# OpenDriveLab/ST-P3

Hardware: AMD Instinct MI355X
Metric: BEV samples/sec (6-cam x 3-frame fwd+bwd) (higher is better)
Workload: dtype bf16 convs / f32 voxel pool; 1 GPU; BASELINE configs[2]: batch=4/GPU, 6-cam 224x480, T=3, full STP3 fwd+bwd with segmentation + pedestrian + hdmap + depth CE + instance centerness/offset + flow losses, grad-clip 5, Adam; EfficientNet-B4, D=48, C=64, BEV 200x200; global_batch=4, parallelism=dp1, launch=hipgraph

## Files before the change

### include/stp3_hip.h

```cpp
#ifndef STP3_HIP_H
#define STP3_HIP_H

#include <stddef.h>
#include <stdint.h>

#ifdef __cplusplus
extern "C" {
#endif

#define STP3_OK          0
#define STP3_EINVAL   (-10001)
#define STP3_EUNSUP   (-10002)
#define STP3_ENOSPACE (-10003)

#define STP3_DTYPE_F32  0
#define STP3_DTYPE_BF16 1

typedef struct stp3_lift_dims {
    int32_t B, T, N;
    int32_t D, fH, fW;
    int32_t C;
    int32_t X, Y, Z;
} stp3_lift_dims;

// ... 135 lines not shown
                    void* stream);
int stp3_linear_bwd(int32_t M, int32_t K, int32_t N, const float* dy, const float* x, const float* w, int32_t ldw, float* dx,
                    float* dw, int32_t lddw, float* db, void* stream);

typedef struct stp3_conv_dims {
    int32_t N, H, W, Cin;
    int32_t Ho, Wo, Cout;
    int32_t KH, KW, stride;
    int32_t pad_h, pad_w, dil_h, dil_w;
    int32_t ldx, ldy;
    int32_t out_dtype, has_bias;
} stp3_conv_dims;

int stp3_conv2d_fwd_workspace(const stp3_conv_dims* dims, size_t* bytes);
int stp3_conv2d_fwd(const stp3_conv_dims* dims, const void* x, const void* w, const float* bias, void* y,
                    float* sums, void* workspace, size_t workspace_bytes, void* stream);

int stp3_conv2d_fwd_stats(const stp3_conv_dims* dims, const void* x, const void* w, float* sums, void* workspace,
                          size_t workspace_bytes, void* stream);
int stp3_conv2d_fwd_bnact(const stp3_conv_dims* dims, const void* x, const void* w, const float* coef, int32_t act, void* y,
                          void* stream);
int stp3_conv2d_bn_bwd_reduce(const stp3_conv_dims* dims, const void* x, const void* w, const void* dz, int32_t ldz,
                              const float* coef, int32_t act, float* sums, void* workspace, size_t workspace_bytes,
                              void* stream);
int stp3_conv2d_bn_bwd_apply(const stp3_conv_dims* dims, const void* x, const void* w, const void* dz, int32_t ldz,
                             const float* coef, int32_t act, const float* gsums, double count, void* dy, void* stream);
int stp3_conv2d_bn_bwd_apply_dx(const stp3_conv_dims* dims, const void* x, const void* w, const void* dz, int32_t ldz,
                                const float* coef, int32_t act, const float* gsums, double count, void* dy, void* dx,
                                int32_t lddx, const void* add, int32_t ldadd, void* stream);

int stp3_conv2d_fwd_add(const stp3_conv_dims* dims, const void* x, const void* w, const float* bias, const void* add,
                        int32_t ldadd, void* y, void* stream);

int stp3_conv2d_wgrad_workspace(const stp3_conv_dims* dims, size_t* bytes);
int stp3_conv2d_wgrad(const stp3_conv_dims* dims, const void* dy, const void* x, float* dw, void* workspace,
                      size_t workspace_bytes, void* stream);

#define STP3_WGRAD_BATCH_MAX 96
typedef struct stp3_wgrad_job {
    const void* partials;
    float* dw;
    int64_t numel;
    int32_t splits;
    int32_t reserved;
} stp3_wgrad_job;
int stp3_conv2d_wgrad_partials(const stp3_conv_dims* dims, const void* dy, const void* x, const float* pre_coef,
                               int32_t pre_act, void* partials, size_t partials_bytes, int32_t* splits, void* stream);
int stp3_conv2d_wgrad_reduce_batch(int32_t n, const stp3_wgrad_job* jobs, void* stream);

int stp3_conv2d_fwd_pre(const stp3_conv_dims* dims, const void* x, const void* w, const float* bias, const float* pre_coef,
                        int32_t pre_act, void* y, void* stream);
int stp3_conv2d_wgrad_pre(const stp3_conv_dims* dims, const void* dy, const void* x, const float* pre_coef, int32_t pre_act,
                          float* dw, void* workspace, size_t workspace_bytes, void* stream);

typedef struct stp3_se_dims {
    int32_t N, rows, C, ld;
    int32_t dtype;
} stp3_se_dims;

int stp3_se_workspace_bytes(const stp3_se_dims* dims, size_t* bytes);
int stp3_se_pool(const stp3_se_dims* dims, const void* x, const void* dy, void* workspace, size_t workspace_bytes,
                 float* out, void* stream);
int stp3_se_scale(const stp3_se_dims* dims, const void* x, const float* gate, const float* add, void* y, void* stream);

typedef struct stp3_se_mlp_dims {
    int32_t N, C, S;
    float inv_rows;
} stp3_se_mlp_dims;

int stp3_se_mlp_fwd(const stp3_se_mlp_dims* dims, const float* pooled_sum, const float* w1, const float* b1,
                    const float* w2, const float* b2, float* z1, float* gate, void* stream);
int stp3_se_mlp_bwd(const stp3_se_mlp_dims* dims, const float* dgate, const float* gate, const float* pooled_sum,
                    const float* z1, const float* w1, const float* w2, float* dz2, float* dz1, float* dpooled,
                    float* dw1, float* db1, float* dw2, float* db2, void* stream);

int stp3_dwconv2d_fwd_stats_workspace(const stp3_dwconv_dims* dims, size_t* bytes);
int stp3_dwconv2d_fwd_stats(const stp3_dwconv_dims* dims, const void* x, const float* w, void* y, float* sums,
                            void* workspace, size_t workspace_bytes, void* stream);
int stp3_bn_finalize(const float* sums, int32_t C, double count, const float* gamma, const float* beta, float eps,
                     float momentum, float* running_mean, float* running_var, float* coef, void* stream);
int stp3_mbconv_workspace_bytes(const stp3_se_dims* dims, size_t* bytes);
int stp3_se_pool_act(const stp3_se_dims* dims, const void* x, const float* scale, const float* shift, int32_t act,
                     void* workspace, size_t workspace_bytes, float* out, void* stream);
int stp3_mbconv_scale_act(const stp3_se_dims* dims, int32_t ldy, const void* x, const float* scale, const float* shift,
                          int32_t act, const float* gate, void* y, void* stream);
int stp3_mbconv_bwd_reduce(const stp3_se_dims* dims, int32_t ldg, const void* da, const void* x, const float* coef,
                           int32_t act, void* workspace, size_t workspace_bytes, float* sums5, void* stream);
int stp3_mbconv_bwd_coef(int32_t N, int32_t C, const float* sums5, const float* gate, const float* dpooled,
                         float* gsums, void* stream);
int stp3_mbconv_bwd_apply(const stp3_se_dims* dims, int32_t ldg, const void* da, const void* x, const float* coef,
                          int32_t act, const float* gate, const float* dpooled, const float* gsums, double count,
                          void* dx, void* stream);

int stp3_dwconv2d_fwd_stats_bn(const stp3_dwconv_dims* dims, const void* x, const float* w, void* y, float* sums, double count,
                               const float* gamma, const float* beta, float eps, float momentum, float* running_mean,
                               float* running_var, float* coef, void* workspace, size_t workspace_bytes, void* stream);

typedef struct stp3_ce_dims {
    int32_t rows, P, C, k;
    int32_t ignore_index, dtype;
    int64_t stride_row, stride_c, stride_p;
} stp3_ce_dims;

int stp3_ce_topk_workspace_bytes(const stp3_ce_dims* dims, size_t* bytes);
int stp3_ce_topk_fwd(const stp3_ce_dims* dims, const void* logits, const int64_t* labels, const float* class_weights,
                     const float* row_scale, float* loss_px, float* sel, double out_scale, int32_t accumulate, float* out,
// ... 332 lines not shown
```

### st-p3_amd/csrc/stp3_bnact.hip

```cpp
#include <hip/hip_runtime.h>
#include <stdint.h>
#include <stdlib.h>

#include <initializer_list>

#include "stp3_cdna.h"
#include "stp3_hip.h"

namespace {

struct BnDims {
    int N, rows, C, ldx, ldy, ldr;
    int act, res_mode, has_sbias, has_oscale;
    int CL;
};

constexpr int kThreads = 256;
constexpr int kUnroll = 4;

__device__ __forceinline__ float bf2f(uint16_t b) { return __uint_as_float((uint32_t)b << 16); }

template <typename T, int VEC> struct Io;
template <> struct Io<float, 4> {
    typedef float4 Raw;
    static __device__ Raw load_raw(const float* p) { return *reinterpret_cast<const float4*>(p); }
    static __device__ void unpack(const Raw& v, float* f) { f[0] = v.x; f[1] = v.y; f[2] = v.z; f[3] = v.w; }
    static __device__ void load(const float* p, float* f) {
        const float4 v = *reinterpret_cast<const float4*>(p);
        f[0] = v.x; f[1] = v.y; f[2] = v.z; f[3] = v.w;
    }
    static __device__ void store(float* p, const float* f) {
        *reinterpret_cast<float4*>(p) = make_float4(f[0], f[1], f[2], f[3]);
    }
};
template <> struct Io<float, 1> {
    typedef float Raw;
    static __device__ Raw load_raw(const float* p) { return p[0]; }
    static __device__ void unpack(const Raw& v, float* f) { f[0] = v; }
    static __device__ void load(const float* p, float* f) { f[0] = p[0]; }
    static __device__ void store(float* p, const float* f) { p[0] = f[0]; }
};
template <> struct Io<uint16_t, 8> {
    typedef uint4 Raw;
    static __device__ Raw load_raw(const uint16_t* p) { return *reinterpret_cast<const uint4*>(p); }
    static __device__ void unpack(const Raw& v, float* f) {
        const uint32_t w[4] = {v.x, v.y, v.z, v.w};
#pragma unroll
        for (int i = 0; i < 4; ++i) {
            f[2 * i] = __uint_as_float(w[i] << 16);
            f[2 * i + 1] = __uint_as_float(w[i] & 0xffff0000u);
        }
    }
    static __device__ void load(const uint16_t* p, float* f) {
        const uint4 v = *reinterpret_cast<const uint4*>(p);
        const uint32_t w[4] = {v.x, v.y, v.z, v.w};
#pragma unroll
        for (int i = 0; i < 4; ++i) {
            f[2 * i] = __uint_as_float(w[i] << 16);
            f[2 * i + 1] = __uint_as_float(w[i] & 0xffff0000u);
        }
// ... 345 lines not shown
#pragma unroll
                for (int u = 0; u < U; ++u) {
                    if (r + u * step < d.rows) {
                        float v[VEC], g[VEC], rv[VEC];
                        Io<T, VEC>::unpack(xr[u], v);
                        Io<T, VEC>::unpack(gr[u], g);
                        mask_tail<VEC, TAIL>(m, v);
                        mask_tail<VEC, TAIL>(m, g);
                        if (PRE_RES) {
                            Io<T, VEC>::unpack(rr[u], rv);
                            mask_tail<VEC, TAIL>(m, rv);
                        }
#pragma unroll
                        for (int j = 0; j < VEC; ++j) {
                            const float xh = (v[j] - mu[j]) * is[j];
                            float gg = g[j] * os;
                            if (ACT != STP3_ACT_NONE) {
                                float pre = fmaf(v[j], cs[j], ct[j]);
                                if (PRE_RES) pre += rv[j];
                                gg *= act_grad_c<ACT>(pre);
                            }
                            acc[0][j] += gg;
                            acc[1][j] = fmaf(gg, xh, acc[1][j]);
                            acc[2][j] += xh;
                        }
                    }
                }
            }
        });
    }
    block_reduce_store<VEC, 3, FULL>(d, m, acc, red, partial);
}

template <typename T, int VEC, bool TRAIN, bool FULL, bool TAIL>
__global__ __launch_bounds__(kThreads) void bn_apply_bwd_kernel(
    BnDims d, const T* __restrict__ dy, const T* __restrict__ x, const float* __restrict__ sbias,
    const T* __restrict__ res, const float* __restrict__ oscale, const float* __restrict__ mean_,
    const float* __restrict__ invstd_, const float* __restrict__ gamma, const float* __restrict__ beta,
    const float* __restrict__ gsums, float inv_count, T* __restrict__ dx, T* __restrict__ dres) {
    const Map m = make_map<VEC, FULL>(d);
    if (!m.live) return;
    const int n = blockIdx.y;
    const int c0 = m.cv * VEC;
    float cs[VEC], ct[VEC], a2[VEC], a3[VEC];
#pragma unroll
    for (int j = 0; j < VEC; ++j) {
        const int c = c0 + j;
        const bool ok = c < d.C;
        const float sb = (ok && d.has_sbias) ? sbias[(size_t)n * d.C + c] : 0.f;
        const float mu = ok ? mean_[c] - sb : 0.f;
        const float is = ok ? invstd_[c] : 0.f;
        const float ga = ok ? (gamma ? gamma[c] : 1.f) : 0.f;
        const float be = ok ? (beta ? beta[c] : 0.f) : 0.f;
        const float k0 = (TRAIN && ok) ? gsums[c] * inv_count : 0.f;
        const float k1 = (TRAIN && ok) ? gsums[d.C + c] * inv_count : 0.f;
        cs[j] = ga * is;
        ct[j] = be - mu * cs[j];
        a2[j] = -(cs[j] * is) * k1;
        a3[j] = -cs[j] * k0 - a2[j] * mu;
    }
    const float os = d.has_oscale ? oscale[n] : 1.f;
    const T* xs = x + (size_t)n * d.rows * d.ldx + c0;
    const T* gs = dy + (size_t)n * d.rows * d.ldy + c0;
    const bool pre_res = d.res_mode == STP3_RES_BEFORE_ACT;
    const T* rs = pre_res ? res + (size_t)n * d.rows * d.ldr + c0 : nullptr;
    T* dxs = dx + (size_t)n * d.rows * d.ldx + c0;
    T* drs = (pre_res && dres) ? dres + (size_t)n * d.rows * d.ldr + c0 : nullptr;
    const int step = gridDim.x * m.RL;
    constexpr int U = 4;
    typedef typename Io<T, VEC>::Raw Raw;
    dispatch_act_res(d.act, rs ? STP3_RES_BEFORE_ACT : STP3_RES_NONE, [&](auto act_c, auto res_c) {
        constexpr int ACT = decltype(act_c)::value;
        constexpr bool PRE_RES = decltype(res_c)::value == STP3_RES_BEFORE_ACT;
        for (int r = blockIdx.x * m.RL + m.rl; r < d.rows; r += U * step) {
            Raw xr[U], gr[U], rr[U];
#pragma unroll
            for (int u = 0; u < U; ++u) {
                if (r + u * step < d.rows) {
                    xr[u] = Io<T, VEC>::load_raw(xs + (size_t)(r + u * step) * d.ldx);
                    gr[u] = Io<T, VEC>::load_raw(gs + (size_t)(r + u * step) * d.ldy);
                    if (PRE_RES) rr[u] = Io<T, VEC>::load_raw(rs + (size_t)(r + u * step) * d.ldr);
                }
            }
#pragma unroll
            for (int u = 0; u < U; ++u) {
                if (r + u * step < d.rows) {
                    float v[VEC], g[VEC], rv[VEC];
                    Io<T, VEC>::unpack(xr[u], v);
                    Io<T, VEC>::unpack(gr[u], g);
                    mask_tail<VEC, TAIL>(m, v);
                    mask_tail<VEC, TAIL>(m, g);
                    if (PRE_RES) {
                        Io<T, VEC>::unpack(rr[u], rv);
                        mask_tail<VEC, TAIL>(m, rv);
                    }
#pragma unroll
                    for (int j = 0; j < VEC; ++j) {
                        float gg = g[j] * os;
                        if (ACT != STP3_ACT_NONE) {
                            float pre = fmaf(v[j], cs[j], ct[j]);
                            if (PRE_RES) pre += rv[j];
                            gg *= act_grad_c<ACT>(pre);
                        }
                        g[j] = gg;
                        v[j] = fmaf(cs[j], gg, fmaf(a2[j], v[j], a3[j]));
                    }
                    Io<T, VEC>::store(dxs + (size_t)(r + u * step) * d.ldx, v);
                    if (drs) Io<T, VEC>::store(drs + (size_t)(r + u * step) * d.ldr, g);
                }
            }
        }
    });
}

__global__ __launch_bounds__(kThreads) void bn_dsbias_kernel(int N, int C, float rows, const float* __restrict__ sample_sums,
                                                             const float* __restrict__ gsums, float inv_count,
                                                             const float* __restrict__ gamma,
                                                             const float* __restrict__ invstd, float* __restrict__ out) {
    const int i = blockIdx.x * kThreads + threadIdx.x;
    if (i >= N * C) return;
    const int n = i / C, c = i - n * C;
    const float* s = sample_sums + (size_t)n * 3 * C;
    const float gi = (gamma ? gamma[c] : 1.f) * invstd[c];
    float v = s[c];
    if (gsums) {
        const float k0 = gsums[c] * inv_count, k1 = gsums[C + c] * inv_count;
        v = (v - rows * k0) - s[2 * C + c] * k1;
    }
    out[i] = gi * v;
}

struct SumPtrs {
    const void* p[8];
};
template <typename T, int VEC>
__global__ __launch_bounds__(kThreads) void sum_n_kernel(int n, size_t nvec, SumPtrs src, T* __restrict__ y,
                                                         const T* __restrict__ plane, unsigned vps, unsigned cvs) {
    typedef typename Io<T, VEC>::Raw Raw;
    const size_t stride = (size_t)gridDim.x * kThreads;
    for (size_t i = (size_t)blockIdx.x * kThreads + threadIdx.x; i < nvec; i += 2 * stride) {
        const bool two = i + stride < nvec;
        Raw a[8], b[8];
#pragma unroll
        for (int k = 0; k < 8; ++k) {
            if (k < n) {
                a[k] = Io<T, VEC>::load_raw((const T*)src.p[k] + i * VEC);
                if (two) b[k] = Io<T, VEC>::load_raw((const T*)src.p[k] + (i + stride) * VEC);
            }
        }
        float acc[VEC], acc2[VEC], v[VEC];
#pragma unroll
        for (int j = 0; j < VEC; ++j) acc[j] = acc2[j] = 0.f;
#pragma unroll
        for (int k = 0; k < 8; ++k) {
            if (k < n) {
                Io<T, VEC>::unpack(a[k], v);
#pragma unroll
                for (int j = 0; j < VEC; ++j) acc[j] += v[j];
// ... 322 lines not shown
```

### st-p3_amd/csrc/stp3_conv.hip

```cpp
#include <hip/hip_runtime.h>
#include <stdint.h>
#include <stdlib.h>
#include <string.h>

#include "stp3_cdna.h"
#include "stp3_hip.h"

namespace {

typedef __attribute__((ext_vector_type(8))) __bf16 bf16x8;
typedef __attribute__((ext_vector_type(4))) float f32x4;
typedef __attribute__((ext_vector_type(16))) float f32x16;

struct ConvDims {
    int N, H, W, Cin, Ho, Wo, Cout;
    int KH, KW, stride, pad_h, pad_w, dil_h, dil_w;
    int ldx, ldy;
    int out_f32, has_bias;
    int M;
    int kchunks;
    int Ktot;
};

union Frag {
    uint4 u;
    bf16x8 v;
};

__device__ __forceinline__ float bf2f(uint32_t b) { return __uint_as_float(b << 16); }

constexpr int kBM = 128;
constexpr int kBK = 64;

__device__ __attribute__((aligned(16))) uint4 g_zero16 = {0u, 0u, 0u, 0u};
typedef stp3_u32x4 u32x4;

__device__ __forceinline__ uint4 keep(uint4 v, bool ok) {
    return make_uint4(ok ? v.x : 0u, ok ? v.y : 0u, ok ? v.z : 0u, ok ? v.w : 0u);
}

__device__ __forceinline__ int xcd_order(int bid, int nwg) {
    const int q = nwg >> 3, r = nwg & 7, xcd = bid & 7;
    return (xcd < r ? xcd * (q + 1) : r * (q + 1) + (xcd - r) * q) + (bid >> 3);
}

__device__ __forceinline__ int lds_piece(int r, int j) { return (r * 8 + (j ^ ((r >> 1) & 7))) * 16; }

enum { kModePlain = 0, kModeStats = 1, kModeBnAct = 2, kModeBwdReduce = 3, kModeBwdApply = 4, kModeAffine = 5 };
constexpr bool mode_bwd(int m) { return m == kModeBwdReduce || m == kModeBwdApply; }

struct EpiArgs {
    const uint16_t* add;
    int ldadd;
    uint16_t* dx;
    int lddx;
    const float* coef;
    const uint16_t* dz;
    const float* gsums;
    float inv_count;
    int ldz, act;
    const uint16_t* res;
    int ldres, res_mode;
    int cvalid;
    const float* sbias;
    int hw;
    const float* pre;
    int pre_off;
};

enum { kPreNone = 0, kPreAffine = 1, kPreRelu = 2 };
template <int PRE>
__device__ __forceinline__ uint32_t pre_pair(uint32_t wd, stp3_f32x2 cs, stp3_f32x2 ct) {
    const stp3_f32x2 e0 = {__uint_as_float(wd << 16), __uint_as_float(wd & 0xffff0000u)};
    stp3_f32x2 out = pk_fma(e0, cs, ct);
    if (PRE == kPreRelu) out = stp3_f32x2{fmaxf(out.x, 0.f), fmaxf(out.y, 0.f)};
    return pack_bf16(out.x, out.y);
}
template <int PRE>
__device__ __forceinline__ u32x4 pre_piece(u32x4 v, const stp3_f32x2 (&cs)[4], const stp3_f32x2 (&ct)[4], uint32_t mask) {
    u32x4 o;
#pragma unroll
    for (int r = 0; r < 4; ++r) o[r] = pre_pair<PRE>(v[r], cs[r], ct[r]) & mask;
    return o;
}

template <int ACT>
__device__ __forceinline__ float epi_act(float v) {
    if (ACT == STP3_ACT_RELU) return fmaxf(v, 0.f);
    if (ACT == STP3_ACT_SWISH) return v * fast_sigmoid(v);
    return v;
}
template <int ACT>
__device__ __forceinline__ float epi_act_grad(float pre) {
    if (ACT == STP3_ACT_RELU) return pre > 0.f ? 1.f : 0.f;
    if (ACT == STP3_ACT_SWISH) {
        const float sg = fast_sigmoid(pre);
        return sg * (1.f + pre * (1.f - sg));
    }
    return 1.f;
}

template <int BN, int MODE = kModePlain, int ACT = STP3_ACT_NONE, bool BUF = false, int PRE = kPreNone>
__global__ __launch_bounds__(256) void conv2d_igemm_kernel(ConvDims d, int tiles_co, const uint16_t* __restrict__ x,
                                                           const uint16_t* __restrict__ w,
                                                           const float* __restrict__ bias, void* __restrict__ y,
                                                           float* __restrict__ stat_partial, EpiArgs ep = EpiArgs()) {
    constexpr int TP = BN == 128 ? 2 : 1;
    constexpr int TC = 2;
    constexpr int kStage = (kBM + BN) * kBK * 2;
    extern __shared__ __attribute__((aligned(16))) uint8_t smem[];
    const int tid = threadIdx.x;
    const int lane = tid & 63;
    const int wave = __builtin_amdgcn_readfirstlane(tid >> 6);
    const int wm = BN == 128 ? (wave >> 1) : wave;
    const int wn = BN == 128 ? (wave & 1) : 0;
    const int v = xcd_order(blockIdx.x, gridDim.x);
    const int tile_m = v / tiles_co, tile_co = v - tile_m * tiles_co;
    const int m0 = tile_m * kBM;
    const int co0 = tile_co * BN;

    const int j = tid & 7, rr = tid >> 3;
    const uint16_t* const zero = reinterpret_cast<const uint16_t*>(&g_zero16);
    const uint16_t* prow[4];
    uint32_t poff[4];
    int phi[4], pwi[4];
    uint32_t rmask[4];
#pragma unroll
    for (int i = 0; i < 4; ++i) {
        const int m = m0 + rr + 32 * i;
        if (PRE) rmask[i] = m < d.M ? 0xffffffffu : 0u;
        if (m < d.M) {
            const int wo = m % d.Wo;
            const int t = m / d.Wo;
            const int ho = t % d.Ho;
            const int n = t / d.Ho;
            phi[i] = ho * d.stride - d.pad_h;
            pwi[i] = wo * d.stride - d.pad_w;
            if (BUF) poff[i] = (uint32_t)(((n * d.H + phi[i]) * d.W + pwi[i]) * d.ldx) * 2u;
            else prow[i] = x + (ptrdiff_t)((n * d.H + phi[i]) * d.W + pwi[i]) * d.ldx;
        } else {
            phi[i] = -(1 << 28);
            pwi[i] = 0;
            if (BUF) poff[i] = kBufOob; else prow[i] = zero;
        }
    }
    const uint16_t* wrow[BN / 32];
    uint32_t woff[BN / 32];
#pragma unroll
    for (int i = 0; i < BN / 32; ++i) {
        const int co = co0 + rr + 32 * i;
        if (BUF) woff[i] = co < d.Cout ? (uint32_t)(co * d.Ktot) * 2u : kBufOob;
        else wrow[i] = co < d.Cout ? w + (size_t)co * d.Ktot : zero;
    }
    const stp3_buffer xbuf = make_buffer(x, BUF ? (uint32_t)((size_t)d.N * d.H * d.W * d.ldx * 2) : 0u);
    const stp3_buffer wbuf = make_buffer(w, BUF ? (uint32_t)((size_t)d.Cout * d.Ktot * 2) : 0u);
    int tap = 0, ci = j * 8;
    while (ci >= d.Cin) { ci -= d.Cin; ++tap; }
    int kh = tap / d.KW, kw = tap - kh * d.KW;
    const int taps = d.KH * d.KW;
    const bool pointwise = taps == 1 && d.pad_h == 0 && d.pad_w == 0 && (d.Ho - 1) * d.stride < d.H &&
                           (d.Wo - 1) * d.stride < d.W;

    const int steps = (d.Ktot + kBK - 1) / kBK;
    float* const ptab = reinterpret_cast<float*>(smem + ep.pre_off);
    const int kpad = steps * kBK;
    int prek = 0;
    if (PRE) {
        for (int e = tid; e < 2 * kpad; e += 256) {
            const int h = e >= kpad, c = e - h * kpad;
            ptab[e] = c < d.Cin ? ep.pre[h * d.Cin + c] : 0.f;
        }
        __syncthreads();
    }

    u32x4 ra[4], rb[BN / 32];
    auto load_step = [&]() {
        const bool kvalid = tap < taps;
        const int dh = kh * d.dil_h, dw = kw * d.dil_w;
        const int toff = (dh * d.W + dw) * d.ldx + ci;
#pragma unroll
        for (int i = 0; i < 4; ++i) {
            if (BUF) {
                bool ok = kvalid & (poff[i] != kBufOob);
                if (!pointwise) {
                    const int hi = phi[i] + dh, wi = pwi[i] + dw;
                    ok = ok & ((unsigned)hi < (unsigned)d.H) & ((unsigned)wi < (unsigned)d.W);
                }
                ra[i] = buffer_load16(xbuf, ok ? poff[i] + (uint32_t)toff * 2u : kBufOob);
            } else {
                bool ok = kvalid && prow[i] != zero;
                if (!pointwise) {
                    const int hi = phi[i] + dh, wi = pwi[i] + dw;
                    ok = ok && (unsigned)hi < (unsigned)d.H && (unsigned)wi < (unsigned)d.W;
                }
                ra[i] = *reinterpret_cast<const u32x4*>(ok ? prow[i] + toff : zero);
            }
        }
        const int kk = tap * d.Cin + ci;
        if (PRE) prek = kk;
#pragma unroll
        for (int i = 0; i < BN / 32; ++i) {
            if (BUF) rb[i] = buffer_load16(wbuf, (kvalid & (woff[i] != kBufOob)) ? woff[i] + (uint32_t)kk * 2u : kBufOob);
            else rb[i] = *reinterpret_cast<const u32x4*>((kvalid && wrow[i] != zero) ? wrow[i] + kk : zero);
        }
        ci += kBK;
        while (ci >= d.Cin && tap < taps) {
            ci -= d.Cin;
            ++tap;
            if (++kw == d.KW) { kw = 0; ++kh; }
        }
    };
    auto store_step = [&](uint8_t* buf) {
        if (PRE) {
            const f32x4 s0 = *reinterpret_cast<const f32x4*>(ptab + prek), s1 = *reinterpret_cast<const f32x4*>(ptab + prek + 4);
            const f32x4 t0 = *reinterpret_cast<const f32x4*>(ptab + kpad + prek);
            const f32x4 t1 = *reinterpret_cast<const f32x4*>(ptab + kpad + prek + 4);
            const stp3_f32x2 cs[4] = {{s0[0], s0[1]}, {s0[2], s0[3]}, {s1[0], s1[1]}, {s1[2], s1[3]}};
            const stp3_f32x2 ct[4] = {{t0[0], t0[1]}, {t0[2], t0[3]}, {t1[0], t1[1]}, {t1[2], t1[3]}};
#pragma unroll
            for (int i = 0; i < 4; ++i) ra[i] = pre_piece<PRE>(ra[i], cs, ct, rmask[i]);
        }
#pragma unroll
        for (int i = 0; i < 4; ++i) *reinterpret_cast<u32x4*>(buf + lds_piece(rr + 32 * i, j)) = ra[i];
#pragma unroll
        for (int i = 0; i < BN / 32; ++i) *reinterpret_cast<u32x4*>(buf + kBM * kBK * 2 + lds_piece(rr + 32 * i, j)) = rb[i];
    };

    f32x16 acc[TC][TP];
#pragma unroll
    for (int a = 0; a < TC; ++a)
#pragma unroll
        for (int b = 0; b < TP; ++b)
#pragma unroll
            for (int r = 0; r < 16; ++r) acc[a][b][r] = 0.f;

    load_step();
    store_step(smem);
    __syncthreads();
    const int frow = lane & 31, fk = lane >> 5;
    for (int s = 0; s < steps; ++s) {
        uint8_t* cur = smem + (s & 1) * kStage;
        if (s + 1 < steps) load_step();
#pragma unroll
        for (int ks = 0; ks < kBK / 16; ++ks) {
            Frag fa[TC], fb[TP];
#pragma unroll
            for (int a = 0; a < TC; ++a)
                fa[a].u = *reinterpret_cast<const uint4*>(cur + kBM * kBK * 2 + lds_piece(wn * 64 + a * 32 + frow, ks * 2 + fk));
#pragma unroll
            for (int b = 0; b < TP; ++b)
                fb[b].u = *reinterpret_cast<const uint4*>(cur + lds_piece(wm * (32 * TP) + b * 32 + frow, ks * 2 + fk));
#pragma unroll
            for (int a = 0; a < TC; ++a)
#pragma unroll
                for (int b = 0; b < TP; ++b)
                    acc[a][b] = __builtin_amdgcn_mfma_f32_32x32x16_bf16(fa[a].v, fb[b].v, acc[a][b], 0, 0, 0);
        }
        if (s + 1 < steps) store_step(smem + ((s + 1) & 1) * kStage);
        __syncthreads();
    }

    const int ldt = BN + 8;
    if (d.out_f32) {
        float* tile = reinterpret_cast<float*>(smem);
#pragma unroll
        for (int a = 0; a < TC; ++a)
// ... 240 lines not shown
                }
            }
        }
}

template <int MODE>
__device__ __forceinline__ void epi8(const uint32_t (&wds)[4], const uint32_t (&gds)[4], const Chan8& k, int act,
                                     stp3_f32x2 (&s1)[4], stp3_f32x2 (&s2)[4], uint32_t (&ow)[4], int res_mode = STP3_RES_NONE) {
#pragma unroll
    for (int r = 0; r < 4; ++r) {
        const uint32_t wd = MODE == kModeAffine ? wds[r] & k.keep[r] : wds[r];
        const stp3_f32x2 e0 = {__uint_as_float(wd << 16), __uint_as_float(wd & 0xffff0000u)};
        if (MODE == kModePlain || MODE == kModeStats) {
            s1[r] = s1[r] + e0;
            s2[r] = pk_fma(e0, e0, s2[r]);
        } else {
            const stp3_f32x2 pre = pk_fma(e0, k.cs[r], k.ct[r]);
            if (MODE == kModeBnAct) {
                stp3_f32x2 out = pre;
                if (act == STP3_ACT_SWISH) out = pre * pk_sigmoid(pre);
                else if (act == STP3_ACT_RELU) out = stp3_f32x2{fmaxf(pre.x, 0.f), fmaxf(pre.y, 0.f)};
                ow[r] = pack_bf16(out.x, out.y);
            } else if (MODE == kModeAffine) {
                const uint32_t gd = gds[r] & k.keep[r];
                const stp3_f32x2 rv = {__uint_as_float(gd << 16), __uint_as_float(gd & 0xffff0000u)};
                stp3_f32x2 out = pre;
                if (res_mode == STP3_RES_BEFORE_ACT) out = out + rv;
                if (act == STP3_ACT_SWISH) out = out * pk_sigmoid(out);
                else if (act == STP3_ACT_RELU) out = stp3_f32x2{fmaxf(out.x, 0.f), fmaxf(out.y, 0.f)};
                if (res_mode == STP3_RES_AFTER_ACT) out = out + rv;
                ow[r] = pack_bf16(out.x, out.y);
            } else {
                const stp3_f32x2 dz = {__uint_as_float(gds[r] << 16), __uint_as_float(gds[r] & 0xffff0000u)};
                stp3_f32x2 der = {1.f, 1.f};
                if (act == STP3_ACT_SWISH) {
                    const stp3_f32x2 sg = pk_sigmoid(pre);
                    der = sg * (1.f + pre * (1.f - sg));
                } else if (act == STP3_ACT_RELU) {
                    der = stp3_f32x2{pre.x > 0.f ? 1.f : 0.f, pre.y > 0.f ? 1.f : 0.f};
                }
                const stp3_f32x2 gg = dz * der;
                if (MODE == kModeBwdReduce) {
                    s1[r] = s1[r] + gg;
                    s2[r] = pk_fma(gg, (e0 - k.mu[r]) * k.is[r], s2[r]);
                } else {
                    const stp3_f32x2 out = pk_fma(k.cs[r], gg, pk_fma(k.a2[r], e0, k.a3[r]));
                    ow[r] = pack_bf16(out.x, out.y);
                }
            }
        }
    }
}

template <int PP, int KMAX, int MODE>
__global__ __launch_bounds__(256, 2) void pointwise_rows_kernel(ConvDims d, int ksteps, int tiles_co, const uint16_t* __restrict__ x,
                                                             const uint16_t* __restrict__ w, uint16_t* __restrict__ y,
                                                             float* __restrict__ stat_partial, EpiArgs ep) {
    constexpr int NT = (PP + 3) / 4;
    constexpr int RPI = 64 / PP;
    constexpr int NIT = (32 + RPI - 1) / RPI;
    constexpr int LDT = NT * 32 + 8;
    extern __shared__ __attribute__((aligned(16))) uint8_t smem[];
    const int tid = threadIdx.x, lane = tid & 63;
    const int wave = __builtin_amdgcn_readfirstlane(tid >> 6);
    const int v_order = xcd_order(blockIdx.x, gridDim.x);
    const int group = v_order / tiles_co, ngroups = gridDim.x / tiles_co;
    const int co0 = (v_order - group * tiles_co) * (PP * 8);
    const int LDW = ksteps * 16 + 8;
    uint16_t* wimg = reinterpret_cast<uint16_t*>(smem);
    uint16_t* tile = wimg + NT * 32 * LDW + wave * (32 * LDT);
    float* red = reinterpret_cast<float*>(wimg + NT * 32 * LDW);
    uint16_t* wtimg = wimg + NT * 32 * LDW + 4 * (32 * LDT);
    const bool with_dx = MODE == kModeBwdApply && ep.dx != nullptr;
    if (with_dx) {
        for (int e = tid; e < 32 * NT * 32; e += 256) {
            const int k = e / (NT * 32), c = e - k * (NT * 32);
            wtimg[k * LDT + c] = (c < PP * 8 && k < d.Cin) ? w[(size_t)(co0 + c) * d.Cin + k] : (uint16_t)0;
        }
    }
    for (int e = tid; e < NT * 32 * ksteps * 2; e += 256) {
        const int r = e / (ksteps * 2), k0 = (e - r * (ksteps * 2)) * 8;
        u32x4 v = {0u, 0u, 0u, 0u};
        if (r < PP * 8 && k0 < d.Cin) v = *reinterpret_cast<const u32x4*>(w + (size_t)(co0 + r) * d.Cin + k0);
        *reinterpret_cast<u32x4*>(wimg + r * LDW + k0) = v;
    }
    __syncthreads();
    const int px = lane & 31, half = lane >> 5;
    const int cp = lane % PP, prow = lane / PP;
    const bool lane_ok = prow < RPI;
    const int cl = cp * 8, cch = co0 + cl;
    Chan8 kc;
    load_chan8<MODE>(kc, ep, d.Cout, cch, true);
    stp3_f32x2 s1[4], s2[4];
#pragma unroll
    for (int r = 0; r < 4; ++r) s1[r] = s2[r] = stp3_f32x2{0.f, 0.f};
    const uint16_t* const zero = reinterpret_cast<const uint16_t*>(&g_zero16);
    u32x4 cur[KMAX], nxt[KMAX];
    const int ntiles = (d.M + 31) / 32;
    const int stride_t = ngroups * 4;
    auto load_tile = [&](int t, u32x4 (&f)[KMAX]) {
        const int m = t * 32 + px;
        const uint16_t* row = (t < ntiles && m < d.M) ? x + (size_t)m * d.ldx : nullptr;
#pragma unroll
        for (int ks = 0; ks < KMAX; ++ks) {
            const int k0 = ks * 16 + half * 8;
            if (ks < ksteps) f[ks] = *reinterpret_cast<const u32x4*>((row && k0 < d.Cin) ? row + k0 : zero);
        }
    };
    int t = group * 4 + wave;
    load_tile(t, cur);
    for (; t < ntiles; t += stride_t) {
        load_tile(t + stride_t, nxt);
        const int mbase = t * 32;
        f32x16 acc[NT];
#pragma unroll
        for (int a = 0; a < NT; ++a)
#pragma unroll
            for (int r = 0; r < 16; ++r) acc[a][r] = 0.f;
#pragma unroll
        for (int ks = 0; ks < KMAX; ++ks) {
            if (ks < ksteps) {
                Frag fb;
                fb.u = make_uint4(cur[ks][0], cur[ks][1], cur[ks][2], cur[ks][3]);
#pragma unroll
                for (int a = 0; a < NT; ++a) {
                    Frag fa;
                    fa.u = *reinterpret_cast<const uint4*>(wimg + (a * 32 + px) * LDW + ks * 16 + half * 8);
                    acc[a] = __builtin_amdgcn_mfma_f32_32x32x16_bf16(fa.v, fb.v, acc[a], 0, 0, 0);
                }
            }
        }
#pragma unroll
        for (int a = 0; a < NT; ++a)
#pragma unroll
            for (int q = 0; q < 4; ++q)
                *reinterpret_cast<uint2*>(tile + px * LDT + a * 32 + 8 * q + 4 * half) =
                    make_uint2(pack_bf16(acc[a][4 * q], acc[a][4 * q + 1]), pack_bf16(acc[a][4 * q + 2], acc[a][4 * q + 3]));
        __builtin_amdgcn_fence(__ATOMIC_RELEASE, "wavefront");
        __builtin_amdgcn_wave_barrier();
#pragma unroll
        for (int i = 0; i < NIT; ++i) {
            const int p = prow + i * RPI;
            const int m = mbase + p;
            if (lane_ok && p < 32 && m < d.M) {
                const uint4 v = *reinterpret_cast<const uint4*>(tile + p * LDT + cl);
                if (MODE == kModePlain) *reinterpret_cast<uint4*>(y + (size_t)m * d.ldy + cch) = v;
                if (MODE != kModePlain || stat_partial) {
                    const uint32_t wds[4] = {v.x, v.y, v.z, v.w};
                    uint32_t gds[4] = {0u, 0u, 0u, 0u}, ow[4];
                    if (mode_bwd(MODE)) {
                        const uint4 g = *reinterpret_cast<const uint4*>(ep.dz + (size_t)m * ep.ldz + cch);
                        gds[0] = g.x; gds[1] = g.y; gds[2] = g.z; gds[3] = g.w;
                    }
                    if (MODE == kModeAffine && ep.res) {
                        const uint4 g = *reinterpret_cast<const uint4*>(ep.res + (size_t)m * ep.ldres + cch);
                        gds[0] = g.x; gds[1] = g.y; gds[2] = g.z; gds[3] = g.w;
                    }
                    if (MODE == kModeAffine) epi8<MODE>(wds, gds, kc, ep.act, s1, s2, ow, ep.res ? ep.res_mode : STP3_RES_NONE);
                    else epi8<MODE>(wds, gds, kc, ep.act, s1, s2, ow);
                    if (MODE == kModeBnAct || MODE == kModeBwdApply || MODE == kModeAffine)
                        *reinterpret_cast<uint4*>(y + (size_t)m * d.ldy + cch) = make_uint4(ow[0], ow[1], ow[2], ow[3]);
                    if (with_dx)
                        *reinterpret_cast<uint4*>(tile + p * LDT + cl) = make_uint4(ow[0], ow[1], ow[2], ow[3]);
                }
            }
        }
        if (with_dx) {
            __builtin_amdgcn_fence(__ATOMIC_RELEASE, "wavefront");
            __builtin_amdgcn_wave_barrier();
            f32x16 dxa;
#pragma unroll
            for (int r = 0; r < 16; ++r) dxa[r] = 0.f;
#pragma unroll
            for (int ks = 0; ks < NT * 2; ++ks) {
                Frag fa, fb;
                fa.u = *reinterpret_cast<const uint4*>(wtimg + px * LDT + ks * 16 + half * 8);
                fb.u = *reinterpret_cast<const uint4*>(tile + px * LDT + ks * 16 + half * 8);
                dxa = __builtin_amdgcn_mfma_f32_32x32x16_bf16(fa.v, fb.v, dxa, 0, 0, 0);
            }
            const int m = mbase + px;
            if (m < d.M) {
#pragma unroll
                for (int q = 0; q < 4; ++q) {
                    const int ci = 8 * q + 4 * half;
                    if (ci < d.Cin) {
                        uint32_t lo = pack_bf16(dxa[4 * q], dxa[4 * q + 1]), hi = pack_bf16(dxa[4 * q + 2], dxa[4 * q + 3]);
                        if (ep.add) {
                            const uint2 a = *reinterpret_cast<const uint2*>(ep.add + (size_t)m * ep.ldadd + ci);
                            lo = pack_bf16(__uint_as_float(lo << 16) + __uint_as_float(a.x << 16),
                                           __uint_as_float(lo & 0xffff0000u) + __uint_as_float(a.x & 0xffff0000u));
                            hi = pack_bf16(__uint_as_float(hi << 16) + __uint_as_float(a.y << 16),
                                           __uint_as_float(hi & 0xffff0000u) + __uint_as_float(a.y & 0xffff0000u));
                        }
                        *reinterpret_cast<uint2*>(ep.dx + (size_t)m * ep.lddx + ci) = make_uint2(lo, hi);
                    }
                }
            }
        }
        __builtin_amdgcn_wave_barrier();
#pragma unroll
        for (int ks = 0; ks < KMAX; ++ks) cur[ks] = nxt[ks];
    }
    if (stat_partial && (MODE == kModePlain || MODE == kModeStats || MODE == kModeBwdReduce)) {
        __syncthreads();
#pragma unroll
        for (int r = 0; r < 8; ++r) {
            red[(wave * 64 + lane) * 16 + r] = s1[r >> 1][r & 1];
            red[(wave * 64 + lane) * 16 + 8 + r] = s2[r >> 1][r & 1];
        }
        __syncthreads();
        for (int e = tid; e < 2 * PP * 8; e += 256) {
            const int k = e / (PP * 8), c = e - k * (PP * 8);
            const int pc = c >> 3, r = c & 7;
            float tot = 0.f;
            for (int wv = 0; wv < 4; ++wv)
                for (int g = 0; g < RPI; ++g) tot += red[(wv * 64 + g * PP + pc) * 16 + k * 8 + r];
            stat_partial[((size_t)group * 2 + k) * d.Cout + co0 + c] = tot;
        }
    }
}

template <int KMAX, int MODE>
__global__ __launch_bounds__(256) void pointwise_direct_kernel(ConvDims d, int ksteps, int cblocks, int ngroups,
                                                               const uint16_t* __restrict__ x, const uint16_t* __restrict__ w,
                                                               uint16_t* __restrict__ y, float* __restrict__ stat_partial,
                                                               EpiArgs ep) {
    constexpr bool kSums = MODE == kModePlain || MODE == kModeStats || MODE == kModeBwdReduce;
    __shared__ float red[kSums ? 4 * 64 * 33 : 1];
    const int tid = threadIdx.x, lane = tid & 63;
    const int wave = __builtin_amdgcn_readfirstlane(tid >> 6);
    const int slot = xcd_order(blockIdx.x, gridDim.x) * 4 + wave;
    const int group = slot / cblocks, cb = slot - group * cblocks;
    const bool live = group < ngroups;
    const int px = lane & 31, h = lane >> 5;
    const uint16_t* const zero = reinterpret_cast<const uint16_t*>(&g_zero16);
    Frag wf[KMAX];
    {
        const int q = px >> 3, hh = (px >> 2) & 1, j = px & 3;
        const int co = cb * 32 + 16 * (q >> 1) + 8 * hh + 4 * (q & 1) + j;
#pragma unroll
        for (int ks = 0; ks < KMAX; ++ks) {
            const int k0 = ks * 16 + h * 8;
            wf[ks].u = *reinterpret_cast<const uint4*>((live && ks < ksteps && co < d.Cout && k0 < d.Cin) ? w + (size_t)co * d.Cin + k0 : zero);
        }
    }
    int ch[2];
    bool ok[2];
    Chan8 kc[2];
    stp3_f32x2 s1[2][4], s2[2][4];
#pragma unroll
    for (int s = 0; s < 2; ++s) {
        ch[s] = cb * 32 + 16 * s + 8 * h;
        ok[s] = live && ch[s] < d.Cout;
        load_chan8<MODE>(kc[s], ep, d.Cout, ch[s], ok[s]);
#pragma unroll
        for (int r = 0; r < 4; ++r) s1[s][r] = s2[s][r] = stp3_f32x2{0.f, 0.f};
    }
    const int ntiles = (d.M + 31) / 32;
    u32x4 cur[KMAX], nxt[KMAX];
    auto load_tile = [&](int t, u32x4 (&f)[KMAX]) {
        const int m = t * 32 + px;
        const uint16_t* row = (live && t < ntiles && m < d.M) ? x + (size_t)m * d.ldx : nullptr;
#pragma unroll
        for (int ks = 0; ks < KMAX; ++ks) {
            if (ks < ksteps) {
                const int k0 = ks * 16 + h * 8;
                f[ks] = *reinterpret_cast<const u32x4*>((row && k0 < d.Cin) ? row + k0 : zero);
            }
        }
    };
    int t = live ? group : ntiles;
    load_tile(t, cur);
    for (; t < ntiles; t += ngroups) {
        load_tile(t + ngroups, nxt);
        const int m = t * 32 + px;
        const bool row_ok = m < d.M;
        uint4 g[2] = {make_uint4(0u, 0u, 0u, 0u), make_uint4(0u, 0u, 0u, 0u)};
        if (mode_bwd(MODE)) {
#pragma unroll
            for (int s = 0; s < 2; ++s)
                if (row_ok && ok[s]) g[s] = *reinterpret_cast<const uint4*>(ep.dz + (size_t)m * ep.ldz + ch[s]);
        }
        if (MODE == kModeAffine && ep.res) {
#pragma unroll
            for (int s = 0; s < 2; ++s)
                if (row_ok && ok[s]) g[s] = *reinterpret_cast<const uint4*>(ep.res + (size_t)m * ep.ldres + ch[s]);
        }
        f32x16 acc;
#pragma unroll
        for (int r = 0; r < 16; ++r) acc[r] = 0.f;
#pragma unroll
        for (int ks = 0; ks < KMAX; ++ks) {
            if (ks < ksteps) {
                Frag fb;
                fb.u = make_uint4(cur[ks][0], cur[ks][1], cur[ks][2], cur[ks][3]);
                acc = __builtin_amdgcn_mfma_f32_32x32x16_bf16(wf[ks].v, fb.v, acc, 0, 0, 0);
            }
        }
#pragma unroll
        for (int s = 0; s < 2; ++s) {
            const uint32_t wds[4] = {pack_bf16(acc[8 * s], acc[8 * s + 1]), pack_bf16(acc[8 * s + 2], acc[8 * s + 3]),
                                     pack_bf16(acc[8 * s + 4], acc[8 * s + 5]), pack_bf16(acc[8 * s + 6], acc[8 * s + 7])};
            if (!(row_ok && ok[s])) continue;
            if (MODE == kModePlain) {
                *reinterpret_cast<uint4*>(y + (size_t)m * d.ldy + ch[s]) = make_uint4(wds[0], wds[1], wds[2], wds[3]);
                if (!stat_partial) continue;
            }
            const uint32_t gds[4] = {g[s].x, g[s].y, g[s].z, g[s].w};
            uint32_t ow[4];
            if (MODE == kModeAffine) epi8<MODE>(wds, gds, kc[s], ep.act, s1[s], s2[s], ow, ep.res ? ep.res_mode : STP3_RES_NONE);
            else epi8<MODE>(wds, gds, kc[s], ep.act, s1[s], s2[s], ow);
            if (MODE == kModeBnAct || MODE == kModeBwdApply || MODE == kModeAffine)
                *reinterpret_cast<uint4*>(y + (size_t)m * d.ldy + ch[s]) = make_uint4(ow[0], ow[1], ow[2], ow[3]);
        }
#pragma unroll
        for (int ks = 0; ks < KMAX; ++ks) cur[ks] = nxt[ks];
    }
    if (kSums) {
        if (!stat_partial) return;
        float* mine = red + (wave * 64 + lane) * 33;
#pragma unroll
        for (int s = 0; s < 2; ++s)
#pragma unroll
            for (int r = 0; r < 8; ++r) {
                mine[s * 8 + r] = s1[s][r >> 1][r & 1];
                mine[16 + s * 8 + r] = s2[s][r >> 1][r & 1];
            }
        __builtin_amdgcn_fence(__ATOMIC_RELEASE, "wavefront");
        __builtin_amdgcn_wave_barrier();
        const int idx = lane & 31;
        float tot = 0.f;
        for (int p = 0; p < 32; ++p) tot += red[(wave * 64 + h * 32 + p) * 33 + idx];
        const int k = idx >> 4, sp = (idx >> 3) & 1, r = idx & 7;
        const int c = cb * 32 + 16 * sp + 8 * h + r;
        if (live && c < d.Cout) stat_partial[((size_t)group * 2 + k) * d.Cout + c] = tot;
    }
}

__global__ __launch_bounds__(256) void colsum_kernel(int parts, int width, const float* __restrict__ partial,
                                                     float* __restrict__ out) {
    __shared__ double red[256];
    const int cl = threadIdx.x & 63, rl = threadIdx.x >> 6;
    const int col = blockIdx.x * 64 + cl;
    const int r0 = blockIdx.y * 256, r1 = min(r0 + 256, parts);
    double s0 = 0.0, s1 = 0.0, s2 = 0.0, s3 = 0.0;
    if (col < width) {
        int p = r0 + rl;
        for (; p + 12 < r1; p += 16) {
            const float a = partial[(size_t)p * width + col], b = partial[(size_t)(p + 4) * width + col];
            const float c = partial[(size_t)(p + 8) * width + col], e = partial[(size_t)(p + 12) * width + col];
            s0 += (double)a; s1 += (double)b; s2 += (double)c; s3 += (double)e;
        }
        for (; p < r1; p += 4) s0 += (double)partial[(size_t)p * width + col];
    }
    red[threadIdx.x] = (s0 + s1) + (s2 + s3);
    __syncthreads();
    if (rl == 0 && col < width)
        out[(size_t)blockIdx.y * width + col] = (float)(red[cl] + red[64 + cl] + red[128 + cl] + red[192 + cl]);
}

inline void launch_colsum(hipStream_t s, int parts, int width, float* partial, float* sums) {
    const int wx = (width + 63) / 64;
    if (parts <= 256) {
        hipLaunchKernelGGL(colsum_kernel, dim3(wx, 1), dim3(256), 0, s, parts, width, (const float*)partial, sums);
        return;
    }
    const int l1 = (parts + 255) / 256;
    float* mid = partial + (size_t)parts * width;
    hipLaunchKernelGGL(colsum_kernel, dim3(wx, l1), dim3(256), 0, s, parts, width, (const float*)partial, mid);
    hipLaunchKernelGGL(colsum_kernel, dim3(wx, 1), dim3(256), 0, s, l1 > 256 ? 256 : l1, width, (const float*)mid, sums);
}


template <int T>
__device__ __forceinline__ int wg_piece(int m, int p) {
    const int sw = T == 64 ? ((m >> 1) & 1) << 2 : (m & 3) << 2;
    return m * (T * 2) + ((p ^ sw) << 4);
}

union FragTr {
    stp3_s16x4 h[2];
    bf16x8 v;
};

template <int TCO, int TCI, bool BUF = false, int PRE = kPreNone>
__global__ __launch_bounds__(256) void conv2d_wgrad_kernel(ConvDims d, int tiles_ci, int ksteps_per_block, int tap_fold,
                                                           int xcd_chunks, const uint16_t* __restrict__ dy,
                                                           const uint16_t* __restrict__ x,
                                                           float* __restrict__ partial, const float* __restrict__ pre = nullptr) {
    constexpr int TA = TCO / 64, TB = TCI / 64;
    constexpr int kImgA = kBK * TCO * 2;
    constexpr int kStage = kBK * (TCO + TCI) * 2;
    constexpr int PA = TCO / 8, PB = TCI / 8;
    constexpr int NA = TCO / 32, NB = TCI / 32;
    constexpr int RA = 256 / PA, RB = 256 / PB;
    extern __shared__ __attribute__((aligned(16))) uint8_t smem[];
    const int tid = threadIdx.x;
    const int lane = tid & 63;
    const int wave = __builtin_amdgcn_readfirstlane(tid >> 6);
    const int wa = wave >> 1, wb = wave & 1;
    int bx = blockIdx.x, by = blockIdx.y, bz = blockIdx.z;
    if (xcd_chunks) {
        const int lin = xcd_order(bx + (int)gridDim.x * (by + (int)gridDim.y * bz), (int)(gridDim.x * gridDim.y * gridDim.z));
        bx = lin % (int)gridDim.x;
        by = (lin / (int)gridDim.x) % (int)gridDim.y;
        bz = lin / (int)(gridDim.x * gridDim.y);
    }
    const int tco = bx / tiles_ci, tci = bx - tco * tiles_ci;
    const int tap = by;
    const int split = bz;
    const int kh = tap / d.KW, kw = tap - kh * d.KW;
    const int co0 = tco * TCO, ci0 = tci * TCI;
    const int total_steps = (d.M + kBK - 1) / kBK;
    const int step0 = split * ksteps_per_block;
    const int step1 = min(step0 + ksteps_per_block, total_steps);
    const uint16_t* const zero = reinterpret_cast<const uint16_t*>(&g_zero16);

    const int pa = tid % PA, ra0 = tid / PA;
    const int pb = tid % PB, rb0 = tid / PB;
    const bool a_ok = co0 + pa * 8 < d.Cout;
    const uint16_t* const srca = a_ok ? dy + co0 + pa * 8 : zero;
    const unsigned lda = a_ok ? (unsigned)d.ldy : 0u;
    bool b_ok = ci0 + pb * 8 < d.Cin;
    int chb = ci0 + pb * 8, khb = kh, kwb = kw;
    if (tap_fold) {
        const int t = tap * tap_fold + pb;
        khb = t / d.KW;
        kwb = t - khb * d.KW;
        chb = 0;
        b_ok = t < d.KH * d.KW;
    }
    const uint16_t* const srcb = b_ok ? x + chb : zero;
    const unsigned ldb = b_ok ? (unsigned)d.ldx : 0u;
    const stp3_buffer abuf = make_buffer(dy, BUF ? (uint32_t)((size_t)d.M * d.ldy * 2) : 0u);
    const stp3_buffer bbuf = make_buffer(x, BUF ? (uint32_t)((size_t)d.N * d.H * d.W * d.ldx * 2) : 0u);
    const uint32_t cola = (uint32_t)(co0 + pa * 8) * 2u, colb = (uint32_t)chb * 2u;
    const uint32_t pitcha = (uint32_t)d.ldy * 2u, pitchb = (uint32_t)d.ldx * 2u;
    const int fold_dh = khb * d.dil_h, fold_dw = kwb * d.dil_w;
    stp3_f32x2 pcs[4], pct[4];
    uint32_t bmask[NB];
    if (PRE) {
#pragma unroll
        for (int r = 0; r < 4; ++r)
#pragma unroll
            for (int h = 0; h < 2; ++h) {
                pcs[r][h] = b_ok ? pre[chb + 2 * r + h] : 0.f;
                pct[r][h] = b_ok ? pre[d.Cin + chb + 2 * r + h] : 0.f;
            }
    }

    const int hw = d.Ho * d.Wo;
    const int qa = kBK / hw, qr = kBK - qa * hw, qb = qr / d.Wo, qc = qr - qb * d.Wo;
    int p_wo, p_ho, p_n;
    {
        const int m = step0 * kBK + lane;
        p_wo = m % d.Wo;
        const int t = m / d.Wo;
        p_ho = t % d.Ho;
        p_n = t / d.Ho;
    }
    const int tap_h = kh * d.dil_h - d.pad_h, tap_w = kw * d.dil_w - d.pad_w;

    u32x4 rawa[NA], rawb[NB];
    auto load_step = [&](int step) {
        const int mbase = step * kBK;
#pragma unroll
        for (int i = 0; i < NA; ++i) {
            const int m = mbase + ra0 + RA * i;
            if (BUF) rawa[i] = buffer_load16(abuf, (a_ok & (m < d.M)) ? (uint32_t)m * pitcha + cola : kBufOob);
            else rawa[i] = *reinterpret_cast<const u32x4*>(m < d.M ? srca + (size_t)(unsigned)m * lda : zero);
        }
        const bool inside = mbase + lane < d.M;
        if (!tap_fold) {
            const int hi = p_ho * d.stride + tap_h, wi = p_wo * d.stride + tap_w;
            const bool ok = inside && (unsigned)hi < (unsigned)d.H && (unsigned)wi < (unsigned)d.W;
            const int pix = ok ? (p_n * d.H + hi) * d.W + wi : -1;
#pragma unroll
            for (int i = 0; i < NB; ++i) {
                const int pv = __shfl(pix, rb0 + RB * i);
                if (PRE) bmask[i] = pv >= 0 ? 0xffffffffu : 0u;
                if (BUF) rawb[i] = buffer_load16(bbuf, (b_ok & (pv >= 0)) ? (uint32_t)pv * pitchb + colb : kBufOob);
                else rawb[i] = *reinterpret_cast<const u32x4*>(pv >= 0 ? srcb + (size_t)(unsigned)pv * ldb : zero);
            }
        } else {
            const int hs = p_ho * d.stride - d.pad_h, ws = p_wo * d.stride - d.pad_w;
            const int base = (p_n * d.H + hs) * d.W + ws;
            const int pack = inside ? ((hs + 32768) << 16) | (ws + 32768) : 0;
#pragma unroll
            for (int i = 0; i < NB; ++i) {
                const int bs = __shfl(base, rb0 + RB * i), pk = __shfl(pack, rb0 + RB * i);
                const int hi = (int)((unsigned)pk >> 16) - 32768 + fold_dh, wi = (pk & 0xffff) - 32768 + fold_dw;
                const bool ok = (unsigned)hi < (unsigned)d.H && (unsigned)wi < (unsigned)d.W;
                const int pv = bs + fold_dh * d.W + fold_dw;
                if (BUF) rawb[i] = buffer_load16(bbuf, (b_ok & ok) ? (uint32_t)pv * pitchb + colb : kBufOob);
                else rawb[i] = *reinterpret_cast<const u32x4*>(ok ? srcb + (size_t)(unsigned)pv * ldb : zero);
            }
        }
        p_wo += qc; p_ho += qb; p_n += qa;
        if (p_wo >= d.Wo) { p_wo -= d.Wo; ++p_ho; }
        if (p_ho >= d.Ho) { p_ho -= d.Ho; ++p_n; }
    };
    auto store_step = [&](uint8_t* buf) {
        if (PRE) {
#pragma unroll
            for (int i = 0; i < NB; ++i) rawb[i] = pre_piece<PRE>(rawb[i], pcs, pct, bmask[i]);
        }
#pragma unroll
        for (int i = 0; i < NA; ++i) *reinterpret_cast<u32x4*>(buf + wg_piece<TCO>(ra0 + RA * i, pa)) = rawa[i];
#pragma unroll
        for (int i = 0; i < NB; ++i) *reinterpret_cast<u32x4*>(buf + kImgA + wg_piece<TCI>(rb0 + RB * i, pb)) = rawb[i];
    };

    f32x16 acc[TA][TB];
#pragma unroll
    for (int a = 0; a < TA; ++a)
#pragma unroll
        for (int b = 0; b < TB; ++b)
#pragma unroll
            for (int r = 0; r < 16; ++r) acc[a][b][r] = 0.f;

    const int frow = lane & 31, fk = lane >> 5;
    const int fm = 8 * fk + ((lane & 15) >> 2), fc = 16 * ((lane >> 4) & 1) + 4 * (lane & 3);
    int offa[TA], offb[TB];
#pragma unroll
    for (int a = 0; a < TA; ++a) {
        const int c = wa * (32 * TA) + a * 32 + fc;
        offa[a] = wg_piece<TCO>(fm, c >> 3) + (c & 7) * 2;
    }
#pragma unroll
    for (int b = 0; b < TB; ++b) {
        const int c = wb * (32 * TB) + b * 32 + fc;
        offb[b] = kImgA + wg_piece<TCI>(fm, c >> 3) + (c & 7) * 2;
    }

    if (step0 < step1) {
        load_step(step0);
        store_step(smem);
    }
    __syncthreads();
    for (int s = step0; s < step1; ++s) {
        const uint8_t* cur = smem + ((s - step0) & 1) * kStage;
        if (s + 1 < step1) load_step(s + 1);
#pragma unroll
        for (int ks = 0; ks < kBK / 16; ++ks) {
            FragTr fa[TA], fb[TB];
#pragma unroll
            for (int a = 0; a < TA; ++a) {
                fa[a].h[0] = lds_read_tr16(cur + offa[a] + (ks * 16) * (TCO * 2));
                fa[a].h[1] = lds_read_tr16(cur + offa[a] + (ks * 16 + 4) * (TCO * 2));
            }
#pragma unroll
            for (int b = 0; b < TB; ++b) {
                fb[b].h[0] = lds_read_tr16(cur + offb[b] + (ks * 16) * (TCI * 2));
                fb[b].h[1] = lds_read_tr16(cur + offb[b] + (ks * 16 + 4) * (TCI * 2));
            }
#pragma unroll
            for (int a = 0; a < TA; ++a)
#pragma unroll
// ... 79 lines not shown
        for (; k < splits; k += 4) add(s0, *reinterpret_cast<const float4*>(partial + (size_t)k * n + i));
    } else if (i < n) {
        float* s0e = &s0.x; float* s1e = &s1.x; float* s2e = &s2.x; float* s3e = &s3.x;
        for (int e = 0; e < 4 && i + e < n; ++e) {
            int k = kl;
            for (; k + 12 < splits; k += 16) {
                s0e[e] += partial[(size_t)k * n + i + e];       s1e[e] += partial[(size_t)(k + 4) * n + i + e];
                s2e[e] += partial[(size_t)(k + 8) * n + i + e]; s3e[e] += partial[(size_t)(k + 12) * n + i + e];
            }
            for (; k < splits; k += 4) s0e[e] += partial[(size_t)k * n + i + e];
        }
    }
    float4 t;
    t.x = (s0.x + s1.x) + (s2.x + s3.x); t.y = (s0.y + s1.y) + (s2.y + s3.y);
    t.z = (s0.z + s1.z) + (s2.z + s3.z); t.w = (s0.w + s1.w) + (s2.w + s3.w);
    red[threadIdx.x] = t;
    __syncthreads();
    if (kl == 0 && i < n) {
        const float4 a = red[cg], bb = red[64 + cg], c = red[128 + cg], d = red[192 + cg];
        float4 o;
        o.x = (a.x + bb.x) + (c.x + d.x); o.y = (a.y + bb.y) + (c.y + d.y);
        o.z = (a.z + bb.z) + (c.z + d.z); o.w = (a.w + bb.w) + (c.w + d.w);
        if (i + 3 < n && ((uintptr_t)(dw + i) & 15) == 0) {
            *reinterpret_cast<float4*>(dw + i) = o;
        } else {
            const float* oe = &o.x;
            for (int e = 0; e < 4 && i + e < n; ++e) dw[i + e] = oe[e];
        }
    }
}

inline int status() {
    hipError_t e = hipGetLastError();
    return e == hipSuccess ? STP3_OK : -(int)e;
}

inline size_t igemm_lds(int bn, int steps, bool out_f32) {
    const size_t stage = (size_t)(steps > 1 ? 2 : 1) * (kBM + bn) * kBK * 2;
    const size_t tile = out_f32 ? (size_t)kBM * (bn + 8) * 4 : (size_t)kBM * (bn + 8) * 2 + 512 * sizeof(float);
    return stage > tile ? stage : tile;
}

template <int TCO, int TCI, int PRE>
int wgrad_launch_pre(const ConvDims& d, int tco, int tci, int taps, int splits, int ksteps, int xcd, size_t lds, const void* dy,
                     const void* x, void* workspace, const float* pre, hipStream_t s) {
    hipError_t e = hipFuncSetAttribute(reinterpret_cast<const void*>(&conv2d_wgrad_kernel<TCO, TCI, true, PRE>),
                                       hipFuncAttributeMaxDynamicSharedMemorySize, (int)lds);
    if (e != hipSuccess) return -(int)e;
    hipLaunchKernelGGL((conv2d_wgrad_kernel<TCO, TCI, true, PRE>), dim3(tco * tci, taps, splits), dim3(256), lds, s, d, tci,
                       ksteps, 0, xcd, (const uint16_t*)dy, (const uint16_t*)x, (float*)workspace, pre);
    return STP3_OK;
}

template <int TCO, int TCI>
int wgrad_launch(const ConvDims& d, int tco, int tci, int taps, int splits, int ksteps, int fold, const void* dy,
                 const void* x, void* workspace, hipStream_t s, const float* pre = nullptr, int pre_act = STP3_ACT_NONE) {
    const size_t lds = (size_t)2 * (TCO + TCI) * kBK * 2;
    const int xcd = taps <= 9 && (int64_t)tco * tci * taps * splits < (1LL << 31);
    const bool buf = (size_t)d.M * d.ldy * 2 < (1ull << 31) && (size_t)d.N * d.H * d.W * d.ldx * 2 < (1ull << 31);
    if (pre) {
        if (!buf || fold) return STP3_EUNSUP;
        constexpr int TCIP = (TCO == 64 && TCI == 64) ? 128 : TCI;
        const size_t ldsp = (size_t)2 * (TCO + TCIP) * kBK * 2;
        if (pre_act == STP3_ACT_RELU)
            return wgrad_launch_pre<TCO, TCIP, kPreRelu>(d, tco, tci, taps, splits, ksteps, xcd, ldsp, dy, x, workspace, pre, s);
        return wgrad_launch_pre<TCO, TCIP, kPreAffine>(d, tco, tci, taps, splits, ksteps, xcd, ldsp, dy, x, workspace, pre, s);
    }
    if (buf) {
        hipError_t e = hipFuncSetAttribute(reinterpret_cast<const void*>(&conv2d_wgrad_kernel<TCO, TCI, true>),
                                           hipFuncAttributeMaxDynamicSharedMemorySize, (int)lds);
        if (e != hipSuccess) return -(int)e;
        hipLaunchKernelGGL((conv2d_wgrad_kernel<TCO, TCI, true>), dim3(tco * tci, taps, splits), dim3(256), lds, s, d, tci,
                           ksteps, fold, xcd, (const uint16_t*)dy, (const uint16_t*)x, (float*)workspace);
        return STP3_OK;
    }
    hipError_t e = hipFuncSetAttribute(reinterpret_cast<const void*>(&conv2d_wgrad_kernel<TCO, TCI>),
                                       hipFuncAttributeMaxDynamicSharedMemorySize, (int)lds);
    if (e != hipSuccess) return -(int)e;
    hipLaunchKernelGGL((conv2d_wgrad_kernel<TCO, TCI>), dim3(tco * tci, taps, splits), dim3(256), lds, s, d, tci, ksteps,
                       fold, xcd, (const uint16_t*)dy, (const uint16_t*)x, (float*)workspace);
    return STP3_OK;
}

}

extern "C" {

int stp3_conv2d_fwd_workspace(const stp3_conv_dims* p, size_t* bytes) {
    if (!p || !bytes || p->N <= 0 || p->Ho <= 0 || p->Wo <= 0 || p->Cout <= 0) return STP3_EINVAL;
    const int64_t M = (int64_t)p->N * p->Ho * p->Wo;
    const size_t parts = (size_t)((M + kBM - 1) / kBM);
    if (parts > 65536) return STP3_EUNSUP;
    *bytes = (parts + (parts + 255) / 256) * 2 * p->Cout * sizeof(float);
    return STP3_OK;
}

}

namespace {

template <int BN, int MODE, int ACT>
int igemm_launch_one(const ConvDims& d, dim3 grid, size_t lds, int tiles_co, const void* x, const void* w, const float* bias,
                     void* y, float* partial, const EpiArgs& ep, hipStream_t s) {
    const bool buf = (size_t)d.N * d.H * d.W * d.ldx * 2 < (1ull << 31) && (size_t)d.Cout * d.Ktot * 2 < (1ull << 31);
    if (buf) {
        hipError_t e = hipFuncSetAttribute(reinterpret_cast<const void*>(&conv2d_igemm_kernel<BN, MODE, ACT, true>),
                                           hipFuncAttributeMaxDynamicSharedMemorySize, (int)lds);
        if (e != hipSuccess) return -(int)e;
        hipLaunchKernelGGL((conv2d_igemm_kernel<BN, MODE, ACT, true>), grid, dim3(256), lds, s, d, tiles_co, (const uint16_t*)x,
                           (const uint16_t*)w, bias, y, partial, ep);
        return STP3_OK;
    }
    hipError_t e = hipFuncSetAttribute(reinterpret_cast<const void*>(&conv2d_igemm_kernel<BN, MODE, ACT>),
                                       hipFuncAttributeMaxDynamicSharedMemorySize, (int)lds);
    if (e != hipSuccess) return -(int)e;
    hipLaunchKernelGGL((conv2d_igemm_kernel<BN, MODE, ACT>), grid, dim3(256), lds, s, d, tiles_co, (const uint16_t*)x,
                       (const uint16_t*)w, bias, y, partial, ep);
    return STP3_OK;
}

template <int BN, int PRE>
int igemm_launch_pre(const ConvDims& d, dim3 grid, size_t lds, int tiles_co, const void* x, const void* w, const float* bias, void* y,
                     const EpiArgs& ep, hipStream_t s) {
    hipError_t e = hipFuncSetAttribute(reinterpret_cast<const void*>(&conv2d_igemm_kernel<BN, kModePlain, STP3_ACT_NONE, true, PRE>),
                                       hipFuncAttributeMaxDynamicSharedMemorySize, (int)lds);
    if (e != hipSuccess) return -(int)e;
    hipLaunchKernelGGL((conv2d_igemm_kernel<BN, kModePlain, STP3_ACT_NONE, true, PRE>), grid, dim3(256), lds, s, d, tiles_co,
                       (const uint16_t*)x, (const uint16_t*)w, bias, y, (float*)nullptr, ep);
    return STP3_OK;
}

template <int BN, int MODE>
int igemm_launch_act(int act, const ConvDims& d, dim3 grid, size_t lds, int tiles_co, const void* x, const void* w,
                     const float* bias, void* y, float* partial, const EpiArgs& ep, hipStream_t s) {
    if (MODE == kModePlain || MODE == kModeStats || act == STP3_ACT_NONE)
        return igemm_launch_one<BN, MODE, STP3_ACT_NONE>(d, grid, lds, tiles_co, x, w, bias, y, partial, ep, s);
    if (act == STP3_ACT_RELU) return igemm_launch_one<BN, MODE, STP3_ACT_RELU>(d, grid, lds, tiles_co, x, w, bias, y, partial, ep, s);
    return igemm_launch_one<BN, MODE, STP3_ACT_SWISH>(d, grid, lds, tiles_co, x, w, bias, y, partial, ep, s);
}

template <int PP, int KMAX, int MODE>
int pointwise_rows_launch_one(const ConvDims& d, int ksteps, int tiles_co, unsigned nwg, size_t lds, const void* x, const void* w,
                              void* y, float* partial, const EpiArgs& ep, hipStream_t s) {
    hipError_t e = hipFuncSetAttribute(reinterpret_cast<const void*>(&pointwise_rows_kernel<PP, KMAX, MODE>),
                                       hipFuncAttributeMaxDynamicSharedMemorySize, (int)lds);
    if (e != hipSuccess) return -(int)e;
    hipLaunchKernelGGL((pointwise_rows_kernel<PP, KMAX, MODE>), dim3(nwg), dim3(256), lds, s, d, ksteps, tiles_co,
                       (const uint16_t*)x, (const uint16_t*)w, (uint16_t*)y, partial, ep);
    return STP3_OK;
}

template <int PP, int KMAX>
int pointwise_rows_launch_mode(int mode, const ConvDims& d, int ksteps, int tiles_co, unsigned nwg, size_t lds, const void* x,
                               const void* w, void* y, float* partial, const EpiArgs& ep, hipStream_t s) {
    switch (mode) {
        case kModePlain: return pointwise_rows_launch_one<PP, KMAX, kModePlain>(d, ksteps, tiles_co, nwg, lds, x, w, y, partial, ep, s);
        case kModeStats: return pointwise_rows_launch_one<PP, KMAX, kModeStats>(d, ksteps, tiles_co, nwg, lds, x, w, y, partial, ep, s);
        case kModeBnAct: return pointwise_rows_launch_one<PP, KMAX, kModeBnAct>(d, ksteps, tiles_co, nwg, lds, x, w, y, partial, ep, s);
        case kModeAffine: return pointwise_rows_launch_one<PP, KMAX, kModeAffine>(d, ksteps, tiles_co, nwg, lds, x, w, y, partial, ep, s);
        case kModeBwdReduce:
            return pointwise_rows_launch_one<PP, KMAX, kModeBwdReduce>(d, ksteps, tiles_co, nwg, lds, x, w, y, partial, ep, s);
        default: return pointwise_rows_launch_one<PP, KMAX, kModeBwdApply>(d, ksteps, tiles_co, nwg, lds, x, w, y, partial, ep, s);
    }
}

template <int KMAX, int MODE>
int pointwise_direct_launch_one(const ConvDims& d, int ksteps, unsigned gx, int* parts, const void* x, const void* w, void* y,
                                float* partial, const EpiArgs& ep, hipStream_t s) {
    static const int resident = [] {
        int per_cu = 0;
        if (hipOccupancyMaxActiveBlocksPerMultiprocessor(&per_cu, pointwise_direct_kernel<KMAX, MODE>, 256, 0) != hipSuccess || per_cu < 1)
            per_cu = 1;
        return per_cu * 256;
    }();
    const int cblocks = (d.Cout + 31) / 32;
    const int ntiles = (d.M + 31) / 32;
    int ngroups = resident * 4 / cblocks;
    if (ngroups > (int)gx) ngroups = (int)gx;
    if (ngroups > ntiles) ngroups = ntiles;
    if (ngroups < 1) ngroups = 1;
    *parts = ngroups;
    const unsigned nwg = (unsigned)(((int64_t)ngroups * cblocks + 3) / 4);
    hipLaunchKernelGGL((pointwise_direct_kernel<KMAX, MODE>), dim3(nwg), dim3(256), 0, s, d, ksteps, cblocks, ngroups,
                       (const uint16_t*)x, (const uint16_t*)w, (uint16_t*)y, partial, ep);
    return STP3_OK;
}

template <int KMAX>
int pointwise_direct_launch_mode(int mode, const ConvDims& d, int ksteps, unsigned gx, int* parts, const void* x, const void* w,
                                 void* y, float* partial, const EpiArgs& ep, hipStream_t s) {
    switch (mode) {
        case kModePlain: return pointwise_direct_launch_one<KMAX, kModePlain>(d, ksteps, gx, parts, x, w, y, partial, ep, s);
        case kModeStats: return pointwise_direct_launch_one<KMAX, kModeStats>(d, ksteps, gx, parts, x, w, y, partial, ep, s);
        case kModeBnAct: return pointwise_direct_launch_one<KMAX, kModeBnAct>(d, ksteps, gx, parts, x, w, y, partial, ep, s);
        case kModeAffine: return pointwise_direct_launch_one<KMAX, kModeAffine>(d, ksteps, gx, parts, x, w, y, partial, ep, s);
        case kModeBwdReduce: return pointwise_direct_launch_one<KMAX, kModeBwdReduce>(d, ksteps, gx, parts, x, w, y, partial, ep, s);
        default: return pointwise_direct_launch_one<KMAX, kModeBwdApply>(d, ksteps, gx, parts, x, w, y, partial, ep, s);
    }
}

constexpr int kPointwiseMaxCin = 128;

bool pointwise_applies(const stp3_conv_dims* p, const void* y) {
    return p->KH == 1 && p->KW == 1 && p->stride == 1 && p->pad_h == 0 && p->pad_w == 0 && p->H == p->Ho && p->W == p->Wo &&
           p->Cin <= kPointwiseMaxCin && p->Cout >= 64 && !p->has_bias && p->out_dtype == STP3_DTYPE_BF16 &&
           p->Cout % 8 == 0 && p->ldy % 8 == 0 && !((uintptr_t)y & 15);
}

int pointwise_run(const ConvDims& d, const void* x, const void* w, void* y, float* sums, float* partial, unsigned gx,
                  hipStream_t s, int mode, const EpiArgs& ep) {
    const int ksteps = (d.Cin + 15) / 16;
    int rc, parts;
    const bool rows_small = (d.Cout == 144 || d.Cout == 192) && ksteps <= 2;
    const bool rows_lines = d.Cout % 64 == 0;
    if ((rows_small || rows_lines) && d.ldy % 8 == 0 && (!mode_bwd(mode) || ep.ldz % 8 == 0)) {
        const int pp = rows_small ? d.Cout / 8 : (d.Cout % 128 == 0 ? 16 : 8), nt = (pp + 3) / 4;
        const int tiles_co = d.Cout / (pp * 8);
        if (ep.dx && !(rows_small && mode == kModeBwdApply && d.Cin <= 32)) return STP3_EUNSUP;
        const size_t lds = (size_t)nt * 32 * (ksteps * 16 + 8) * 2 + (size_t)4 * 32 * (nt * 32 + 8) * 2 +
                           (ep.dx ? (size_t)32 * (nt * 32 + 8) * 2 : 0);
        unsigned per_cu = (unsigned)((160 * 1024) / lds);
        if (per_cu > 3) per_cu = 3;
        unsigned groups = (256 * per_cu + tiles_co - 1) / tiles_co;
        if (groups > gx) groups = gx;
        parts = (int)groups;
        const unsigned nwg = groups * (unsigned)tiles_co;
        if (pp == 18) rc = pointwise_rows_launch_mode<18, 2>(mode, d, ksteps, tiles_co, nwg, lds, x, w, y, partial, ep, s);
        else if (pp == 24) rc = pointwise_rows_launch_mode<24, 2>(mode, d, ksteps, tiles_co, nwg, lds, x, w, y, partial, ep, s);
        else if (pp == 8) rc = pointwise_rows_launch_mode<8, 8>(mode, d, ksteps, tiles_co, nwg, lds, x, w, y, partial, ep, s);
        else if (ksteps <= 4) rc = pointwise_rows_launch_mode<16, 4>(mode, d, ksteps, tiles_co, nwg, lds, x, w, y, partial, ep, s);
        else rc = pointwise_rows_launch_mode<16, 8>(mode, d, ksteps, tiles_co, nwg, lds, x, w, y, partial, ep, s);
    } else {
        if (ep.dx) return STP3_EUNSUP;
        if (ksteps <= 2) rc = pointwise_direct_launch_mode<2>(mode, d, ksteps, gx, &parts, x, w, y, partial, ep, s);
        else if (ksteps <= 4) rc = pointwise_direct_launch_mode<4>(mode, d, ksteps, gx, &parts, x, w, y, partial, ep, s);
        else rc = pointwise_direct_launch_mode<8>(mode, d, ksteps, gx, &parts, x, w, y, partial, ep, s);
    }
    if (rc) return rc;
    if (sums) launch_colsum(s, parts, 2 * d.Cout, partial, sums);
    return status();
}

int igemm_run(const stp3_conv_dims* p, const void* x, const void* w, const float* bias, void* y, float* sums, void* workspace,
              size_t workspace_bytes, void* stream, int mode, int act, EpiArgs ep) {
    if (!p || !x || !w || (mode != kModeStats && mode != kModeBwdReduce && !y)) return STP3_EINVAL;
    if (p->N <= 0 || p->H <= 0 || p->W <= 0 || p->Cin <= 0 || p->Cout <= 0 || p->Ho <= 0 || p->Wo <= 0 || p->KH <= 0 ||
        p->KW <= 0 || p->stride <= 0 || p->dil_h <= 0 || p->dil_w <= 0 || p->pad_h < 0 || p->pad_w < 0)
        return STP3_EINVAL;
    if (p->has_bias && !bias) return STP3_EINVAL;
    if (p->Cin % 8 || p->ldx % 8 || p->ldx < p->Cin || p->ldy < p->Cout) return STP3_EUNSUP;
    if (((uintptr_t)x & 15) || ((uintptr_t)w & 15)) return STP3_EUNSUP;
    if (p->out_dtype != STP3_DTYPE_BF16 && p->out_dtype != STP3_DTYPE_F32) return STP3_EUNSUP;
    if (y && ((uintptr_t)y & (p->out_dtype == STP3_DTYPE_F32 ? 3 : 1))) return STP3_EUNSUP;
    if ((sums || mode != kModePlain) && p->out_dtype != STP3_DTYPE_BF16) return STP3_EUNSUP;
    if (mode != kModePlain) {
        if ((p->has_bias && mode != kModeAffine) || p->Cout % 8 || p->ldy % 8 || (y && ((uintptr_t)y & 15))) return STP3_EUNSUP;
        if (mode >= kModeBnAct && !ep.coef) return STP3_EINVAL;
        if (mode == kModeAffine && ep.res && (ep.ldres % 8 || ep.ldres < p->Cout || ((uintptr_t)ep.res & 15))) return STP3_EUNSUP;
        if (mode_bwd(mode) && (!ep.dz || ep.ldz % 8 || ep.ldz < p->Cout || ((uintptr_t)ep.dz & 15))) return STP3_EUNSUP;
        if (mode == kModeBwdApply && !ep.gsums) return STP3_EINVAL;
        if ((mode == kModeStats || mode == kModeBwdReduce) && !sums) return STP3_EINVAL;
    }
    const int64_t M = (int64_t)p->N * p->Ho * p->Wo;
    if (M >= (1LL << 31) || (int64_t)p->N * p->H * p->W >= (1LL << 31)) return STP3_EUNSUP;
    ConvDims d;
    d.N = p->N; d.H = p->H; d.W = p->W; d.Cin = p->Cin; d.Ho = p->Ho; d.Wo = p->Wo; d.Cout = p->Cout;
    d.KH = p->KH; d.KW = p->KW; d.stride = p->stride; d.pad_h = p->pad_h; d.pad_w = p->pad_w;
    d.dil_h = p->dil_h; d.dil_w = p->dil_w; d.ldx = p->ldx; d.ldy = p->ldy;
    d.out_f32 = p->out_dtype == STP3_DTYPE_F32; d.has_bias = p->has_bias;
    d.M = (int)M; d.kchunks = (p->Cin + 31) / 32; d.Ktot = p->KH * p->KW * p->Cin;
    const unsigned gx = (unsigned)((M + kBM - 1) / kBM);
    hipStream_t s = (hipStream_t)stream;
    float* partial = nullptr;
    if (sums) {
        if (gx > 65536) return STP3_EUNSUP;
        if (!workspace || workspace_bytes < ((size_t)gx + (gx + 255) / 256) * 2 * p->Cout * sizeof(float)) return STP3_ENOSPACE;
        partial = (float*)workspace;
    }
    if (y && ((uintptr_t)y & 15)) return STP3_EUNSUP;
    if (ep.dx) {
        if (!pointwise_applies(p, y) || ep.lddx % 4 || ep.lddx < p->Cin || ((uintptr_t)ep.dx & 7) ||
            (ep.add && (ep.ldadd % 4 || ep.ldadd < p->Cin || ((uintptr_t)ep.add & 7))))
            return STP3_EUNSUP;
        ep.act = act;
        return pointwise_run(d, x, w, y, sums, partial, gx, s, mode, ep);
    }
    if (ep.pre) {
        if (mode != kModePlain || sums || ep.add || p->KH != 1 || p->KW != 1 || p->stride != 1 || p->pad_h || p->pad_w ||
            p->H != p->Ho || p->W != p->Wo || p->Cin > 4096)
            return STP3_EUNSUP;
        if (!((size_t)d.N * d.H * d.W * d.ldx * 2 < (1ull << 31) && (size_t)d.Cout * d.Ktot * 2 < (1ull << 31))) return STP3_EUNSUP;
    } else if (ep.add) {
        if (mode != kModePlain || d.out_f32 || p->Cout % 8 || p->ldy % 8 || ep.ldadd % 8 || ep.ldadd < p->Cout ||
            ((uintptr_t)ep.add & 15) || ((uintptr_t)y & 15))
            return STP3_EUNSUP;
    } else if (pointwise_applies(p, y)) {
        if (ep.sbias) return STP3_EUNSUP;
        ep.act = act;
        return pointwise_run(d, x, w, y, sums, partial, gx, s, mode, ep);
    }
    const int steps = (d.Ktot + kBK - 1) / kBK;
    const bool wide = p->Cout > 64 && steps > 2 && (int64_t)gx * ((p->Cout + 127) / 128) >= 512;
    const int bn = wide ? 128 : 64;
    size_t lds = igemm_lds(bn, steps, d.out_f32 != 0);
    if (mode == kModeBwdReduce) {
        const size_t need = (size_t)2 * kBM * (bn + 8) * 2 + 512 * sizeof(float);
        if (need > lds) lds = need;
    }
    const int tiles_co = (p->Cout + bn - 1) / bn;
    if ((int64_t)gx * tiles_co >= (1LL << 31)) return STP3_EUNSUP;
    const dim3 grid(gx * (unsigned)tiles_co);
    int rc;
    if (ep.pre) {
        ep.pre_off = (int)((lds + 15) / 16 * 16);
        lds = (size_t)ep.pre_off + (size_t)2 * steps * kBK * sizeof(float);
        if (act == STP3_ACT_RELU)
            rc = wide ? igemm_launch_pre<128, kPreRelu>(d, grid, lds, tiles_co, x, w, bias, y, ep, s)
                      : igemm_launch_pre<64, kPreRelu>(d, grid, lds, tiles_co, x, w, bias, y, ep, s);
        else
            rc = wide ? igemm_launch_pre<128, kPreAffine>(d, grid, lds, tiles_co, x, w, bias, y, ep, s)
                      : igemm_launch_pre<64, kPreAffine>(d, grid, lds, tiles_co, x, w, bias, y, ep, s);
        return rc ? rc : status();
    }
#define STP3_IGEMM_MODE(MODE)                                                                                                \
    rc = wide ? igemm_launch_act<128, MODE>(act, d, grid, lds, tiles_co, x, w, bias, y, partial, ep, s)                       \
              : igemm_launch_act<64, MODE>(act, d, grid, lds, tiles_co, x, w, bias, y, partial, ep, s)
    switch (mode) {
        case kModePlain: STP3_IGEMM_MODE(kModePlain); break;
        case kModeStats: STP3_IGEMM_MODE(kModeStats); break;
        case kModeBnAct: STP3_IGEMM_MODE(kModeBnAct); break;
        case kModeAffine: STP3_IGEMM_MODE(kModeAffine); break;
        case kModeBwdReduce: STP3_IGEMM_MODE(kModeBwdReduce); break;
        default: STP3_IGEMM_MODE(kModeBwdApply); break;
    }
#undef STP3_IGEMM_MODE
    if (rc) return rc;
    if (sums) launch_colsum(s, (int)gx, 2 * p->Cout, partial, sums);
    return status();
}

}

extern "C" {

int stp3_conv2d_fwd(const stp3_conv_dims* p, const void* x, const void* w, const float* bias, void* y, float* sums,
                    void* workspace, size_t workspace_bytes, void* stream) {
    return igemm_run(p, x, w, bias, y, sums, workspace, workspace_bytes, stream, kModePlain, STP3_ACT_NONE, EpiArgs());
}

int stp3_conv2d_fwd_pre(const stp3_conv_dims* p, const void* x, const void* w, const float* bias, const float* pre_coef,
                        int32_t pre_act, void* y, void* stream) {
    if (!pre_coef || (pre_act != STP3_ACT_NONE && pre_act != STP3_ACT_RELU)) return STP3_EINVAL;
    EpiArgs ep = EpiArgs();
    ep.pre = pre_coef;
    return igemm_run(p, x, w, bias, y, nullptr, nullptr, 0, stream, kModePlain, pre_act, ep);
}

int stp3_conv2d_fwd_add(const stp3_conv_dims* p, const void* x, const void* w, const float* bias, const void* add, int32_t ldadd,
                        void* y, void* stream) {
    if (!add) return STP3_EINVAL;
    EpiArgs ep = EpiArgs();
    ep.add = (const uint16_t*)add;
    ep.ldadd = ldadd;
    return igemm_run(p, x, w, bias, y, nullptr, nullptr, 0, stream, kModePlain, STP3_ACT_NONE, ep);
}
// ... 40 lines not shown
    ep.coef = coef; ep.dz = (const uint16_t*)dz; ep.ldz = ldz; ep.gsums = gsums; ep.inv_count = (float)(1.0 / count);
    return igemm_run(p, x, w, nullptr, dy, nullptr, nullptr, 0, stream, kModeBwdApply, act, ep);
}

int stp3_conv2d_bn_bwd_apply_dx(const stp3_conv_dims* p, const void* x, const void* w, const void* dz, int32_t ldz,
                                const float* coef, int32_t act, const float* gsums, double count, void* dy, void* dx,
                                int32_t lddx, const void* add, int32_t ldadd, void* stream) {
    if (!(count >= 1.0) || !dx) return STP3_EINVAL;
    EpiArgs ep = EpiArgs();
    ep.coef = coef; ep.dz = (const uint16_t*)dz; ep.ldz = ldz; ep.gsums = gsums; ep.inv_count = (float)(1.0 / count);
    ep.dx = (uint16_t*)dx; ep.lddx = lddx; ep.add = (const uint16_t*)add; ep.ldadd = ldadd;
    return igemm_run(p, x, w, nullptr, dy, nullptr, nullptr, 0, stream, kModeBwdApply, act, ep);
}


static int wgrad_plan(const stp3_conv_dims* p, int* tco_sz, int* tci_sz, int* tiles_co, int* tiles_ci, int* splits, int* ksteps,
                      int* fold, int* grid_y) {
    const int64_t M = (int64_t)p->N * p->Ho * p->Wo;
    const int taps = p->KH * p->KW;
    *tco_sz = p->Cout > 64 ? 128 : 64;
    *tci_sz = p->Cin > 64 ? 128 : 64;
    *fold = 0;
    *grid_y = taps;
    if (p->Cin == 8 && taps > 1) {
        *tci_sz = taps > 8 ? 128 : 64;
        *fold = *tci_sz / 8;
        *grid_y = (taps + *fold - 1) / *fold;
    }
    *tiles_co = (p->Cout + *tco_sz - 1) / *tco_sz;
    *tiles_ci = *fold ? 1 : (p->Cin + *tci_sz - 1) / *tci_sz;
    const int64_t total_steps = (M + kBK - 1) / kBK;
    const int64_t base = (int64_t)(*tiles_co) * (*tiles_ci) * (*grid_y);
    const int per_cu = (*tco_sz == 128 && *tci_sz == 128) ? 2 : (*tco_sz == 128 || *tci_sz == 128) ? 3 : 5;
    int64_t want = (256 * per_cu) / base;
    const int64_t max_splits = (total_steps + 7) / 8;
    if (want > max_splits) want = max_splits;
    if (want < 1) want = 1;
    if (want > 512) want = 512;
    *ksteps = (int)((total_steps + want - 1) / want);
    *splits = (int)((total_steps + *ksteps - 1) / *ksteps);
    return STP3_OK;
}

int stp3_conv2d_wgrad_workspace(const stp3_conv_dims* p, size_t* bytes) {
    if (!p || !bytes || p->N <= 0 || p->Cout <= 0 || p->Cin <= 0 || p->KH <= 0 || p->KW <= 0 || p->Ho <= 0 || p->Wo <= 0)
        return STP3_EINVAL;
    int a, b, tco, tci, splits, ksteps, fold, gy;
    wgrad_plan(p, &a, &b, &tco, &tci, &splits, &ksteps, &fold, &gy);
    *bytes = (size_t)splits * p->Cout * p->KH * p->KW * p->Cin * sizeof(float);
    return STP3_OK;
}

static int wgrad_partials(const stp3_conv_dims* p, const void* dy, const void* x, void* workspace, size_t workspace_bytes,
                          int* splits_out, hipStream_t s, const float* pre_coef = nullptr, int pre_act = STP3_ACT_NONE) {
    if (!p || !dy || !x || !workspace) return STP3_EINVAL;
    if (pre_coef) {
        if (pre_act != STP3_ACT_NONE && pre_act != STP3_ACT_RELU) return STP3_EINVAL;
        if (p->KH != 1 || p->KW != 1 || p->stride != 1 || p->pad_h || p->pad_w || p->H != p->Ho || p->W != p->Wo) return STP3_EUNSUP;
    }
    if (p->N <= 0 || p->H <= 0 || p->W <= 0 || p->Cin <= 0 || p->Cout <= 0 || p->Ho <= 0 || p->Wo <= 0 || p->KH <= 0 ||
        p->KW <= 0 || p->stride <= 0 || p->dil_h <= 0 || p->dil_w <= 0 || p->pad_h < 0 || p->pad_w < 0)
        return STP3_EINVAL;
    if (p->Cin % 8 || p->Cout % 8 || p->ldx % 8 || p->ldy % 8 || p->ldx < p->Cin || p->ldy < p->Cout) return STP3_EUNSUP;
    if (((uintptr_t)x & 15) || ((uintptr_t)dy & 15)) return STP3_EUNSUP;
    const int64_t M = (int64_t)p->N * p->Ho * p->Wo;
    if (M >= (1LL << 31) - 64 || ((int64_t)p->N + 2) * p->H * p->W >= (1LL << 31)) return STP3_EUNSUP;
    if ((int64_t)p->Ho * p->stride >= 32768 || (int64_t)p->Wo * p->stride >= 32768 || p->pad_h >= 32768 || p->pad_w >= 32768)
        return STP3_EUNSUP;
    if (p->KH * p->KW > 65535) return STP3_EUNSUP;
    int tco_sz, tci_sz, tco, tci, splits, ksteps, fold, taps;
    wgrad_plan(p, &tco_sz, &tci_sz, &tco, &tci, &splits, &ksteps, &fold, &taps);
    const size_t wsize = (size_t)p->Cout * p->KH * p->KW * p->Cin;
    if (workspace_bytes < (size_t)splits * wsize * sizeof(float)) return STP3_ENOSPACE;
    ConvDims d;
    d.N = p->N; d.H = p->H; d.W = p->W; d.Cin = p->Cin; d.Ho = p->Ho; d.Wo = p->Wo; d.Cout = p->Cout;
    d.KH = p->KH; d.KW = p->KW; d.stride = p->stride; d.pad_h = p->pad_h; d.pad_w = p->pad_w;
    d.dil_h = p->dil_h; d.dil_w = p->dil_w; d.ldx = p->ldx; d.ldy = p->ldy;
    d.out_f32 = 1; d.has_bias = 0; d.M = (int)M; d.kchunks = 0; d.Ktot = p->KH * p->KW * p->Cin;
    int rc;
    if (tco_sz == 128 && tci_sz == 128)
        rc = wgrad_launch<128, 128>(d, tco, tci, taps, splits, ksteps, fold, dy, x, workspace, s, pre_coef, pre_act);
    else if (tco_sz == 128) rc = wgrad_launch<128, 64>(d, tco, tci, taps, splits, ksteps, fold, dy, x, workspace, s, pre_coef, pre_act);
    else if (tci_sz == 128) rc = wgrad_launch<64, 128>(d, tco, tci, taps, splits, ksteps, fold, dy, x, workspace, s, pre_coef, pre_act);
    else rc = wgrad_launch<64, 64>(d, tco, tci, taps, splits, ksteps, fold, dy, x, workspace, s, pre_coef, pre_act);
    if (rc) return rc;
    *splits_out = splits;
    return status();
}

int stp3_conv2d_wgrad(const stp3_conv_dims* p, const void* dy, const void* x, float* dw, void* workspace,
                      size_t workspace_bytes, void* stream) {
    if (!dw) return STP3_EINVAL;
    hipStream_t s = (hipStream_t)stream;
    int splits = 0;
    int rc = wgrad_partials(p, dy, x, workspace, workspace_bytes, &splits, s);
    if (rc) return rc;
    const size_t wsize = (size_t)p->Cout * p->KH * p->KW * p->Cin;
    hipLaunchKernelGGL(conv2d_wgrad_reduce_kernel, dim3((unsigned)((wsize + 63) / 64)), dim3(256), 0, s, splits, wsize,
                       (const float*)workspace, dw);
    return status();
}

int stp3_conv2d_wgrad_pre(const stp3_conv_dims* p, const void* dy, const void* x, const float* pre_coef, int32_t pre_act, float* dw,
                          void* workspace, size_t workspace_bytes, void* stream) {
    if (!dw || !pre_coef) return STP3_EINVAL;
    hipStream_t s = (hipStream_t)stream;
    int splits = 0;
    int rc = wgrad_partials(p, dy, x, workspace, workspace_bytes, &splits, s, pre_coef, pre_act);
    if (rc) return rc;
    const size_t wsize = (size_t)p->Cout * p->KH * p->KW * p->Cin;
    hipLaunchKernelGGL(conv2d_wgrad_reduce_kernel, dim3((unsigned)((wsize + 63) / 64)), dim3(256), 0, s, splits, wsize,
                       (const float*)workspace, dw);
    return status();
}

int stp3_conv2d_wgrad_partials(const stp3_conv_dims* p, const void* dy, const void* x, const float* pre_coef, int32_t pre_act,
                               void* partials, size_t partials_bytes, int32_t* splits, void* stream) {
    if (!splits) return STP3_EINVAL;
    int n = 0;
    int rc = wgrad_partials(p, dy, x, partials, partials_bytes, &n, (hipStream_t)stream, pre_coef, pre_act);
    if (rc) return rc;
    *splits = n;
    return STP3_OK;
}

int stp3_conv2d_wgrad_reduce_batch(int32_t n, const stp3_wgrad_job* jobs, void* stream) {
    if (n < 0 || (n > 0 && !jobs)) return STP3_EINVAL;
    for (int j = 0; j < n; ++j)
        if (!jobs[j].partials || !jobs[j].dw || jobs[j].splits <= 0 || jobs[j].numel <= 0 || jobs[j].numel >= (1LL << 32))
            return STP3_EINVAL;
    hipStream_t s = (hipStream_t)stream;
    for (int j0 = 0; j0 < n; j0 += kWgradBatch) {
        WgradJobs t;
        t.count = n - j0 < kWgradBatch ? n - j0 : kWgradBatch;
        int64_t blocks = 0;
        for (int j = 0; j < t.count; ++j) {
            const stp3_wgrad_job& q = jobs[j0 + j];
            t.partial[j] = (const float*)q.partials;
            t.dw[j] = q.dw;
            t.n[j] = (unsigned)q.numel;
            t.splits[j] = q.splits;
            t.first[j] = (int)blocks;
            blocks += (q.numel + kWgradBatchCols - 1) / kWgradBatchCols;
            if (blocks >= (1LL << 31)) return STP3_EUNSUP;
        }
        for (int j = t.count; j <= kWgradBatch; ++j) t.first[j] = (int)blocks;
        for (int j = t.count; j < kWgradBatch; ++j) { t.partial[j] = nullptr; t.dw[j] = nullptr; t.n[j] = 0; t.splits[j] = 0; }
        hipLaunchKernelGGL(conv2d_wgrad_reduce_batch_kernel, dim3((unsigned)blocks), dim3(256), 0, s, t);
    }
    return status();
}

}
```

### st-p3_amd/stp3_amd/_lib.py

```python
import ctypes
import os

from . import profiling

_HERE = os.path.dirname(os.path.abspath(__file__))
LIB_PATH = os.path.join(_HERE, 'libstp3hip.so')

c_void_p = ctypes.c_void_p
c_int = ctypes.c_int
c_int32 = ctypes.c_int32
c_float = ctypes.c_float
c_size_t = ctypes.c_size_t


class LiftDims(ctypes.Structure):
    _fields_ = [(k, ctypes.c_int32) for k in ('B', 'T', 'N', 'D', 'fH', 'fW', 'C', 'X', 'Y', 'Z')]

    @property
    def BT(self):
        return self.B * self.T

    @property
    def NPIX(self):
        return self.N * self.fH * self.fW

    @property
    def P(self):
        return self.NPIX * self.D

    @property
    def V(self):
        return self.X * self.Y * self.Z


class DwConvDims(ctypes.Structure):
    _fields_ = [(k, ctypes.c_int32) for k in ('N', 'H', 'W', 'C', 'Ho', 'Wo', 'K', 'stride', 'pad_top', 'pad_left',
                                              'dtype')]


class WgradJob(ctypes.Structure):
    _fields_ = [('partials', ctypes.c_void_p), ('dw', ctypes.c_void_p), ('numel', ctypes.c_int64), ('splits', ctypes.c_int32),
                ('reserved', ctypes.c_int32)]


class LayerNormDims(ctypes.Structure):
    _fields_ = [('rows', ctypes.c_int64), ('C', ctypes.c_int32), ('ldx', ctypes.c_int32), ('ldy', ctypes.c_int32),
                ('dtype', ctypes.c_int32), ('act', ctypes.c_int32), ('eps', ctypes.c_float)]


class GruDims(ctypes.Structure):
    _fields_ = [('rows', ctypes.c_int64), ('Cx', ctypes.c_int32), ('C', ctypes.c_int32), ('dtype', ctypes.c_int32),
                ('bias_init', ctypes.c_float)]


class BnDims(ctypes.Structure):
    _fields_ = [(k, ctypes.c_int32) for k in ('N', 'rows', 'C', 'ldx', 'ldy', 'ldr', 'dtype', 'act', 'res_mode',
                                              'has_sbias', 'has_oscale', 'cpad')]


class ConvDims(ctypes.Structure):
    _fields_ = [(k, ctypes.c_int32) for k in ('N', 'H', 'W', 'Cin', 'Ho', 'Wo', 'Cout', 'KH', 'KW', 'stride', 'pad_h',
                                              'pad_w', 'dil_h', 'dil_w', 'ldx', 'ldy', 'out_dtype', 'has_bias')]


class SeDims(ctypes.Structure):
    _fields_ = [(k, ctypes.c_int32) for k in ('N', 'rows', 'C', 'ld', 'dtype')]


class WprepEntry(ctypes.Structure):
    _fields_ = [('src', ctypes.c_void_p), ('fwd', ctypes.c_void_p), ('flip', ctypes.c_void_p),
                ('stride_co', ctypes.c_int64), ('stride_ci', ctypes.c_int64), ('stride_kh', ctypes.c_int64),
                ('stride_kw', ctypes.c_int64), ('first_block', ctypes.c_int64),
                ('cout', ctypes.c_int32), ('cin', ctypes.c_int32), ('kh', ctypes.c_int32), ('kw', ctypes.c_int32),
                ('dst_cout', ctypes.c_int32), ('dst_cin', ctypes.c_int32), ('co_off', ctypes.c_int32),
                ('ci_off', ctypes.c_int32), ('fwd_f32', ctypes.c_int32), ('reserved', ctypes.c_int32)]


class BnCoefEntry(ctypes.Structure):
    _fields_ = [('running_mean', ctypes.c_void_p), ('running_var', ctypes.c_void_p), ('gamma', ctypes.c_void_p),
                ('beta', ctypes.c_void_p), ('out', ctypes.c_void_p), ('first_block', ctypes.c_int64),
                ('channels', ctypes.c_int32), ('lanes', ctypes.c_int32), ('eps', ctypes.c_float), ('reserved', ctypes.c_int32)]


class SeMlpDims(ctypes.Structure):
    _fields_ = [('N', ctypes.c_int32), ('C', ctypes.c_int32), ('S', ctypes.c_int32), ('inv_rows', ctypes.c_float)]


class PairDims(ctypes.Structure):
    _fields_ = [(k, ctypes.c_int32) for k in ('frames', 'T', 'rows', 'C', 'ldx', 'dtype')]


class UpsampleDims(ctypes.Structure):
    _fields_ = [(k, ctypes.c_int32) for k in ('N', 'H', 'W', 'C', 'scale', 'ldx', 'ldy', 'dtype')]


# ... 144 lines not shown
                                    c_void_p, c_void_p, c_void_p]),
    'stp3_lift_bwd_needs_prob': (c_int, [_DIMS_P, ctypes.POINTER(c_int)]),
    'stp3_lift_splat_bwd': (c_int, [_DIMS_P, c_void_p, c_int, c_int, c_void_p, c_void_p, c_void_p, c_void_p, c_void_p,
                                    c_float, c_void_p, c_size_t, c_void_p, c_void_p, c_void_p]),
    'stp3_gru_reset_cat_fwd': (c_int, [_GRU_P, c_void_p, c_void_p, c_void_p, c_void_p]),
    'stp3_gru_output_fwd': (c_int, [_GRU_P, c_void_p, c_void_p, c_void_p, c_void_p, c_void_p]),
    'stp3_gru_output_bwd': (c_int, [_GRU_P, c_void_p, ctypes.c_int32, c_void_p, c_void_p, c_void_p, c_void_p, c_void_p, c_void_p]),
    'stp3_gru_reset_cat_bwd': (c_int, [_GRU_P, c_void_p, ctypes.c_int32, c_void_p, c_void_p, c_void_p, c_void_p, c_void_p, c_void_p]),
    'stp3_layernorm_fwd': (c_int, [_LN_P, c_void_p, c_void_p, c_void_p, c_void_p, c_void_p]),
    'stp3_layernorm_bwd_workspace': (c_int, [_LN_P, ctypes.POINTER(c_size_t)]),
    'stp3_layernorm_bwd': (c_int, [_LN_P] + [c_void_p] * 8 + [c_size_t, c_void_p]),
    'stp3_dwconv2d_fwd': (c_int, [_DW_P, c_void_p, c_void_p, c_void_p, c_void_p]),
    'stp3_dwconv2d_fwd_bias': (c_int, [_DW_P, c_void_p, c_void_p, c_void_p, c_void_p, c_void_p]),
    'stp3_dwconv2d_bwd_data': (c_int, [_DW_P, c_void_p, c_void_p, c_void_p, c_void_p]),
    'stp3_dwconv2d_bwd_weight_workspace': (c_int, [_DW_P, ctypes.POINTER(c_size_t)]),
    'stp3_dwconv2d_bwd_weight': (c_int, [_DW_P, c_void_p, c_void_p, c_void_p, c_void_p, c_size_t, c_void_p]),
    'stp3_dwconv2d_bwd_weight_oihw': (c_int, [_DW_P, c_void_p, c_void_p, c_void_p, c_void_p, c_size_t, c_void_p]),
    'stp3_bn_workspace_bytes': (c_int, [_BN_P, ctypes.POINTER(c_size_t)]),
    'stp3_bn_stats': (c_int, [_BN_P, c_void_p, c_void_p, c_void_p, c_size_t, c_void_p, c_void_p]),
    'stp3_bn_apply_fwd': (c_int, [_BN_P] + [c_void_p] * 5 + [c_double, c_void_p, c_void_p, c_float, c_float]
                          + [c_void_p] * 6),
    'stp3_bn_bwd_reduce': (c_int, [_BN_P] + [c_void_p] * 10 + [c_size_t, c_void_p, c_void_p, c_void_p]),
    'stp3_bn_apply_bwd': (c_int, [_BN_P] + [c_void_p] * 10 + [c_double, c_void_p, c_void_p, c_void_p]),
    'stp3_bn_fwd_train': (c_int, [_BN_P] + [c_void_p] * 6 + [c_float, c_float] + [c_void_p] * 4 + [c_size_t, c_void_p,
                                                                                                 c_void_p]),
    'stp3_bn_bwd_train': (c_int, [_BN_P] + [c_void_p] * 10 + [c_size_t] + [c_void_p] * 4),
    'stp3_bn_dsbias': (c_int, [c_int32, c_int32, c_int32, c_void_p, c_void_p, c_double, c_void_p, c_void_p, c_void_p, c_void_p]),
    'stp3_sum_n': (c_int, [c_int32, ctypes.c_int64, c_int32, c_void_p, c_void_p, c_void_p]),
    'stp3_linear_fwd': (c_int, [c_int32, c_int32, c_int32, c_void_p, c_void_p, c_int32, c_void_p, c_void_p, c_void_p]),
    'stp3_linear_bwd': (c_int, [c_int32, c_int32, c_int32, c_void_p, c_void_p, c_void_p, c_int32, c_void_p, c_void_p, c_int32, c_void_p,
                                c_void_p]),
    'stp3_sum_n_plane': (c_int, [c_int32, ctypes.c_int64, c_int32, c_void_p, c_void_p, ctypes.c_int64, c_int32, c_void_p, c_void_p]),
    'stp3_conv2d_fwd_workspace': (c_int, [ctypes.POINTER(ConvDims), ctypes.POINTER(c_size_t)]),
    'stp3_conv2d_fwd': (c_int, [ctypes.POINTER(ConvDims)] + [c_void_p] * 6 + [c_size_t, c_void_p]),
    'stp3_conv2d_fwd_add': (c_int, [ctypes.POINTER(ConvDims), c_void_p, c_void_p, c_void_p, c_void_p, c_int32, c_void_p, c_void_p]),
    'stp3_conv2d_fwd_stats': (c_int, [ctypes.POINTER(ConvDims), c_void_p, c_void_p, c_void_p, c_void_p, c_size_t, c_void_p]),
    'stp3_conv2d_fwd_bnact': (c_int, [ctypes.POINTER(ConvDims), c_void_p, c_void_p, c_void_p, c_int32, c_void_p, c_void_p]),
    'stp3_conv2d_bn_bwd_reduce': (c_int, [ctypes.POINTER(ConvDims), c_void_p, c_void_p, c_void_p, c_int32, c_void_p, c_int32,
                                          c_void_p, c_void_p, c_size_t, c_void_p]),
    'stp3_conv2d_bn_bwd_apply': (c_int, [ctypes.POINTER(ConvDims), c_void_p, c_void_p, c_void_p, c_int32, c_void_p, c_int32,
                                         c_void_p, c_double, c_void_p, c_void_p]),
    'stp3_se_workspace_bytes': (c_int, [ctypes.POINTER(SeDims), ctypes.POINTER(c_size_t)]),
    'stp3_se_pool': (c_int, [ctypes.POINTER(SeDims), c_void_p, c_void_p, c_void_p, c_size_t, c_void_p, c_void_p]),
    'stp3_se_scale': (c_int, [ctypes.POINTER(SeDims), c_void_p, c_void_p, c_void_p, c_void_p, c_void_p]),
    'stp3_conv2d_bn_bwd_apply_dx': (c_int, [ctypes.POINTER(ConvDims), c_void_p, c_void_p, c_void_p, c_int32, c_void_p, c_int32, c_void_p,
                                            ctypes.c_double, c_void_p, c_void_p, c_int32, c_void_p, c_int32, c_void_p]),
    'stp3_conv2d_wgrad_workspace': (c_int, [ctypes.POINTER(ConvDims), ctypes.POINTER(c_size_t)]),
    'stp3_conv2d_wgrad': (c_int, [ctypes.POINTER(ConvDims), c_void_p, c_void_p, c_void_p, c_void_p, c_size_t, c_void_p]),
    'stp3_conv2d_wgrad_partials': (c_int, [ctypes.POINTER(ConvDims), c_void_p, c_void_p, c_void_p, c_int32, c_void_p, c_size_t,
                                           ctypes.POINTER(c_int32), c_void_p]),
    'stp3_conv2d_fwd_pre': (c_int, [ctypes.POINTER(ConvDims), c_void_p, c_void_p, c_void_p, c_void_p, c_int32, c_void_p, c_void_p]),
    'stp3_conv2d_wgrad_pre': (c_int, [ctypes.POINTER(ConvDims), c_void_p, c_void_p, c_void_p, c_int32, c_void_p, c_void_p, c_size_t,
                                      c_void_p]),
    'stp3_conv2d_wgrad_reduce_batch': (c_int, [c_int32, ctypes.POINTER(WgradJob), c_void_p]),
    'stp3_conv2d_prep_weights': (c_int, [c_void_p, c_int32, ctypes.c_int64, c_void_p]),
    'stp3_conv2d_scatter_weight_grads': (c_int, [c_void_p, c_int32, ctypes.c_int64, c_void_p]),
    'stp3_se_mlp_fwd': (c_int, [c_void_p] * 9),
    'stp3_se_mlp_bwd': (c_int, [c_void_p] * 15),
    'stp3_optim_workspace_bytes': (c_int, [ctypes.c_int64, ctypes.POINTER(c_size_t)]),
    'stp3_optim_clip_adam': (c_int, [c_void_p, c_int32, ctypes.c_int64] + [c_float] * 6 + [c_void_p, c_void_p, c_size_t,
                                                                                          c_void_p]),
    'stp3_causal_pair_fwd': (c_int, [ctypes.POINTER(PairDims), c_void_p, c_void_p, c_void_p]),
    'stp3_causal_pair_bwd': (c_int, [ctypes.POINTER(PairDims), c_void_p, c_void_p, c_void_p]),
    'stp3_upsample_bilinear_fwd': (c_int, [ctypes.POINTER(UpsampleDims), c_void_p, c_void_p, c_void_p]),
    'stp3_upsample_bilinear_bwd': (c_int, [ctypes.POINTER(UpsampleDims), c_void_p, c_void_p, c_void_p]),
    'stp3_dwconv2d_fwd_stats_workspace': (c_int, [_DW_P, ctypes.POINTER(c_size_t)]),
    'stp3_dwconv2d_fwd_stats': (c_int, [_DW_P, c_void_p, c_void_p, c_void_p, c_void_p, c_void_p, c_size_t, c_void_p]),
    'stp3_bn_finalize': (c_int, [c_void_p, c_int32, c_double, c_void_p, c_void_p, c_float, c_float, c_void_p, c_void_p,
                                 c_void_p, c_void_p]),
    'stp3_mbconv_workspace_bytes': (c_int, [ctypes.POINTER(SeDims), ctypes.POINTER(c_size_t)]),
    'stp3_se_pool_act': (c_int, [ctypes.POINTER(SeDims), c_void_p, c_void_p, c_void_p, c_int32, c_void_p, c_size_t, c_void_p,
                                 c_void_p]),
    'stp3_mbconv_scale_act': (c_int, [ctypes.POINTER(SeDims), c_int32, c_void_p, c_void_p, c_void_p, c_int32, c_void_p,
                                      c_void_p, c_void_p]),
    'stp3_mbconv_bwd_reduce': (c_int, [ctypes.POINTER(SeDims), c_int32, c_void_p, c_void_p, c_void_p, c_int32, c_void_p,
                                       c_size_t, c_void_p, c_void_p]),
    'stp3_mbconv_bwd_coef': (c_int, [c_int32, c_int32, c_void_p, c_void_p, c_void_p, c_void_p, c_void_p]),
    'stp3_mbconv_bwd_apply': (c_int, [ctypes.POINTER(SeDims), c_int32, c_void_p, c_void_p, c_void_p, c_int32, c_void_p,
                                      c_void_p, c_void_p, c_double, c_void_p, c_void_p]),
    'stp3_dwconv2d_fwd_stats_bn': (c_int, [_DW_P, c_void_p, c_void_p, c_void_p, c_void_p, c_double, c_void_p, c_void_p, c_float,
                                           c_float, c_void_p, c_void_p, c_void_p, c_void_p, c_size_t, c_void_p]),
    'stp3_ce_topk_workspace_bytes': (c_int, [ctypes.POINTER(CeDims), ctypes.POINTER(c_size_t)]),
    'stp3_ce_topk_fwd': (c_int, [ctypes.POINTER(CeDims)] + [c_void_p] * 6 + [c_double, c_int32, c_void_p, c_void_p, c_size_t,
                                                                           c_void_p]),
    'stp3_ce_topk_bwd': (c_int, [ctypes.POINTER(CeDims)] + [c_void_p] * 7 + [c_double, c_void_p, c_void_p]),
    'stp3_reg_loss_workspace_bytes': (c_int, [ctypes.POINTER(c_size_t)]),
    'stp3_reg_loss_fwd': (c_int, [c_int32] * 4 + [c_float, c_int32] + [c_void_p] * 5 + [c_size_t, c_void_p]),
    'stp3_reg_loss_bwd': (c_int, [c_int32] * 4 + [c_float, c_int32] + [c_void_p] * 7),
    'stp3_warp_nearest': (c_int, [c_int32] * 4 + [c_void_p] * 5),
    'stp3_traj_cost_fwd': (c_int, [ctypes.POINTER(PlanDims)] + [c_void_p] * 14),
    'stp3_traj_cost_bwd': (c_int, [ctypes.POINTER(PlanDims)] + [c_void_p] * 5),
    'stp3_plan_scene': (c_int, [ctypes.POINTER(SceneDims)] + [c_void_p] * 7),
    'stp3_plan_drive': (c_int, [ctypes.POINTER(PlanDims), ctypes.POINTER(DriveDims)] + [c_void_p] * 14),
    'stp3_traj_sample': (c_int, [ctypes.POINTER(SamplerDims)] + [c_void_p] * 6),
    'stp3_instance_segment': (c_int, [c_int32] * 3 + [c_float] + [c_void_p] * 7),
    'stp3_instance_track': (c_int, [c_int32] * 4 + [c_float] + [c_void_p] * 5),
    'stp3_eval_semantic': (c_int, [ctypes.POINTER(EvalDims)] + [c_void_p] * 8),
    'stp3_eval_planning': (c_int, [ctypes.POINTER(EvalPlanDims)] + [c_void_p] * 10),
    'stp3_eval_panoptic_workspace_bytes': (c_int, [c_int32] * 3 + [ctypes.POINTER(c_size_t)]),
    'stp3_eval_panoptic': (c_int, [c_int32] * 7 + [c_void_p] * 3 + [c_size_t] + [c_void_p] * 3),
    'stp3_image_prep_rows_per_workgroup': (c_int, []),
    'stp3_image_prep_lds_bytes': (c_int, [ctypes.POINTER(ImageDims), c_int32, ctypes.POINTER(c_size_t)]),
    'stp3_image_prep': (c_int, [ctypes.POINTER(ImageDims)] + [c_void_p] * 5 + [c_int32, c_void_p, c_void_p]),
    'stp3_image_augment_workspace_bytes': (c_int, [ctypes.POINTER(AugmentDims), ctypes.POINTER(c_size_t)]),
    'stp3_image_augment': (c_int, [ctypes.POINTER(AugmentDims)] + [c_void_p] * 4 + [c_size_t, c_void_p, c_void_p]),
    'stp3_fill_polygons': (c_int, [c_void_p, c_int32, c_int32, c_int32, c_int32, c_void_p, c_void_p]),
# ... 74 lines not shown
```

### st-p3_amd/stp3_amd/ops.py

```python
import ctypes
import os
import types
import weakref

import torch

from . import _lib, scratch
from ._lib import LiftDims, VOX_PIXELMAJOR, VOX_REFERENCE, check


def _ptr(t):
    return ctypes.c_void_p(t.data_ptr())


def _stream():
    return ctypes.c_void_p(torch.cuda.current_stream().cuda_stream)


def _stream_handle():
    return torch.cuda.current_stream().cuda_stream


PROFILE_ENABLED = False
PROFILE = []
# ... 1006 lines not shown
    def forward(ctx, x, frames_per_sample):
        _need_gpu(x)
        n, c, h, w = x.shape
        x, ldx = _rows_view(x)
        dt = _lib.DTYPE_BF16 if x.dtype == torch.bfloat16 else _lib.DTYPE_F32
        dims = _lib.PairDims(n, int(frames_per_sample), h * w, c, ldx, dt)
        y = torch.empty((n, 2 * c, h, w), dtype=x.dtype, device=x.device, memory_format=torch.channels_last)
        check(_lib.lib().stp3_causal_pair_fwd(ctypes.byref(dims), x.data_ptr(), y.data_ptr(), _stream_handle()),
              'stp3_causal_pair_fwd')
        ctx.dims = dims
        return y

    @staticmethod
    def backward(ctx, dy):
        d = ctx.dims
        dy = dy.contiguous(memory_format=torch.channels_last)
        n, c2, h, w = dy.shape
        dx = torch.empty((n, c2 // 2, h, w), dtype=dy.dtype, device=dy.device, memory_format=torch.channels_last)
        dims = _lib.PairDims(d.frames, d.T, d.rows, d.C, d.C,
                             _lib.DTYPE_BF16 if dy.dtype == torch.bfloat16 else _lib.DTYPE_F32)
        check(_lib.lib().stp3_causal_pair_bwd(ctypes.byref(dims), dy.data_ptr(), dx.data_ptr(), _stream_handle()),
              'stp3_causal_pair_bwd')
        return dx, None


def causal_pair_supported(x):
    per = 8 if x.dtype == torch.bfloat16 else 4
    return x.is_cuda and x.dim() == 4 and x.dtype in (torch.bfloat16, torch.float32) and x.shape[1] % per == 0


def causal_pair(x, frames_per_sample):
    return _CausalPair.apply(x, frames_per_sample)


def _pair(v):
    return (int(v), int(v)) if not isinstance(v, (tuple, list)) else (int(v[0]), int(v[1]))


def _conv_out(size, k, stride, pad, dil):
    return (size + 2 * pad - dil * (k - 1) - 1) // stride + 1


class SkipCarrier:
    __slots__ = ('grad',)

    def __init__(self):
        self.grad = None

    def take(self):
        g, self.grad = self.grad, None
        return g


def _conv2d_launch(x, wb, bias, stride, pad, dil, out_dtype, sums_ptr=None, out_hw=None, add=None, out_slot=None):
    n, cin, h, w = x.shape
    cout, _, kh, kw = wb.shape
    x, ldx = _rows_view(x)
    if out_hw is None:
        ho, wo = _conv_out(h, kh, stride, pad[0], dil[0]), _conv_out(w, kw, stride, pad[1], dil[1])
    else:
        ho, wo = out_hw
    ldy = cout
    if out_slot is None:
        y = torch.empty((n, cout, ho, wo), dtype=out_dtype, device=x.device, memory_format=torch.channels_last)
    else:
        assert add is None
        y, ldy = slot_view(out_slot, types.SimpleNamespace(shape=(n, cout, ho, wo), dtype=out_dtype))
    dims = _lib.ConvDims(n, h, w, cin, ho, wo, cout, kh, kw, stride, pad[0], pad[1], dil[0], dil[1], ldx, ldy,
                         _lib.DTYPE_F32 if out_dtype == torch.float32 else _lib.DTYPE_BF16, int(bias is not None))
    lib = _lib.lib()
    ws_ptr, ws_bytes = None, 0
    if sums_ptr is not None:
        nbytes = ctypes.c_size_t()
        check(lib.stp3_conv2d_fwd_workspace(ctypes.byref(dims), ctypes.byref(nbytes)), 'stp3_conv2d_fwd_workspace')
        ws_ptr, ws_bytes = scratch.get('conv_stat', nbytes.value, x.device, floor=8 << 20).data_ptr(), nbytes.value
    if add is not None:
        assert sums_ptr is None
        add, ldadd = _rows_view(add)
        if (out_dtype == torch.bfloat16 and add.dtype == torch.bfloat16 and tuple(add.shape) == tuple(y.shape) and cout % 8 == 0
                and ldadd % 8 == 0 and add.data_ptr() % 16 == 0):
            check(lib.stp3_conv2d_fwd_add(ctypes.byref(dims), _ptr(x), _ptr(wb), _opt_ptr(bias), _ptr(add), ldadd, _ptr(y),
                                          _stream()), 'stp3_conv2d_fwd_add')
            return y
        check(lib.stp3_conv2d_fwd(ctypes.byref(dims), _ptr(x), _ptr(wb), _opt_ptr(bias), _ptr(y), None, None, 0, _stream()),
              'stp3_conv2d_fwd')
        return y + add.to(y.dtype)
    check(lib.stp3_conv2d_fwd(ctypes.byref(dims), _ptr(x), _ptr(wb), _opt_ptr(bias), _ptr(y), sums_ptr, ws_ptr, ws_bytes,
                              _stream()), 'stp3_conv2d_fwd')
    return y


DIRECT_BUCKET_GRADS = True


def _conv2d_wgrad(dy, x, wshape, stride, pad, dil, leaf=None, pre=None):
    cout, cin, kh, kw = wshape
    pre_ptr, pre_act = (None, 0) if pre is None else (pre[0].data_ptr(), int(pre[1]))
    n, _, h, w = x.shape
    x, ldx = _rows_view(x)
    dy, ldy = _rows_view(dy)
    ho, wo = dy.shape[2], dy.shape[3]
    dims = _lib.ConvDims(n, h, w, cin, ho, wo, cout, kh, kw, stride, pad[0], pad[1], dil[0], dil[1], ldx, ldy,
                         _lib.DTYPE_F32, 0)
    lib = _lib.lib()
    nbytes = ctypes.c_size_t()
    check(lib.stp3_conv2d_wgrad_workspace(ctypes.byref(dims), ctypes.byref(nbytes)), 'stp3_conv2d_wgrad_workspace')
    dw = torch.empty((cout, cin, kh, kw), dtype=torch.float32, device=x.device, memory_format=torch.channels_last)
    direct = False
    plain_leaf = (leaf is not None and x.is_cuda and leaf.is_leaf and leaf.grad is None and leaf.dtype == torch.float32
                  and tuple(leaf.shape) == tuple(dw.shape) and _same_memory_order(leaf, dw))
    if plain_leaf:
        view = getattr(leaf, '_stp3_grad_view', None)
        task = _graph_task_id()
        if (DIRECT_BUCKET_GRADS and view is not None and task != -1 and getattr(leaf, '_stp3_grad_claim', None) != task and view.device == dw.device
                and view.dtype == torch.float32 and _same_memory_order(view, dw)):
            leaf._stp3_grad_claim = task
            dw = view.detach()
            direct = True
    asm = getattr(leaf, '_stp3_assembled', None) if leaf is not None else None
    if (asm is not None and ASSEMBLED_WEIGHTS and DIRECT_BUCKET_GRADS and x.is_cuda and leaf._stp3_assembled_direct
            and _assembled_claim(asm, dw, leaf._stp3_assembled_direct == 'shared')):
        dw = asm['dw'].detach()
        direct = True
    if direct and DEFER_WGRAD_REDUCE and getattr(leaf, '_stp3_uses', 0) == 1 and _single_process():
        key = scratch.key(x.device)
        arena = _WGRAD_ARENAS.get(key)
        if arena is None:
            arena = _WGRAD_ARENAS[key] = _WgradArena(x.device)
        slot = arena.take(nbytes.value)
        if slot is not None:
            splits = ctypes.c_int32()
            check(lib.stp3_conv2d_wgrad_partials(ctypes.byref(dims), _ptr(dy), _ptr(x), pre_ptr, pre_act, slot,
                                                 ctypes.c_size_t(nbytes.value), ctypes.byref(splits), _stream()),
                  'stp3_conv2d_wgrad_partials')
            arena.jobs.append((slot, dw.data_ptr(), cout * cin * kh * kw, splits.value))
            return dw
    ws = scratch.get('conv_wgrad', nbytes.value, x.device, floor=64 << 20)
    if pre is not None:
        check(lib.stp3_conv2d_wgrad_pre(ctypes.byref(dims), _ptr(dy), _ptr(x), pre_ptr, pre_act, _ptr(dw), _ptr(ws),
                                        ctypes.c_size_t(nbytes.value), _stream()), 'stp3_conv2d_wgrad_pre')
        return dw
    check(lib.stp3_conv2d_wgrad(ctypes.byref(dims), _ptr(dy), _ptr(x), _ptr(dw), _ptr(ws), ctypes.c_size_t(nbytes.value),
                                _stream()), 'stp3_conv2d_wgrad')
    return dw


DEFER_WGRAD_REDUCE = True
_WGRAD_ARENAS = {}


def note_weight_use(weight):
    if weight is not None:
        weight._stp3_uses = getattr(weight, '_stp3_uses', 0) + 1
    return weight


def _single_process():
    return not replicas(None)[1]


class _WgradArena:

    def __init__(self, device):
        self.device = device
        self.buf = None
        self.size = 0
        self.used = 0
        self.wanted = 0
        self.jobs = []

    def take(self, nbytes):
        nbytes = (nbytes + 255) // 256 * 256
        self.wanted += nbytes
        if self.used == 0:
            self.buf = scratch.get('wgrad_arena', 0 if scratch.capturing() else self.size, self.device, floor=64 << 20)
        if self.used + nbytes > self.buf.numel():
            return None
        ptr = self.buf.data_ptr() + self.used
        self.used += nbytes
        return ptr

    def flush(self):
        if self.jobs:
            arr = (_lib.WgradJob * len(self.jobs))()
            for rec, (partials, dw, numel, splits) in zip(arr, self.jobs):
                rec.partials, rec.dw, rec.numel, rec.splits = partials, dw, numel, splits
            check(_lib.lib().stp3_conv2d_wgrad_reduce_batch(len(self.jobs), arr, _stream()), 'stp3_conv2d_wgrad_reduce_batch')
        if self.wanted > self.buf.numel() and not scratch.capturing():
            self.size = self.wanted + (self.wanted >> 3)
        self.jobs, self.used, self.wanted = [], 0, 0
# ... 432 lines not shown
            g = torch.zeros_like(p)
            for pc in ent['pieces']:
                if pc['param']() is p:
                    co, ci = pc['dims'][:2]
                    g.as_strided(pc['dims'], pc['strides'], pc['offset']).copy_(
                        dw[pc['co_off']:pc['co_off'] + co, pc['ci_off']:pc['ci_off'] + ci])
            grads.append(g)
        return (None, None) + tuple(grads)


def _evict_weight(key, ent):
    if _WEIGHT_CACHE.get(key) is ent:
        del _WEIGHT_CACHE[key]


def _phase_taps(k, pad, stride, phase):
    khs = [kh for kh in range(k) if (phase + pad - kh) % stride == 0]
    if not khs:
        return None
    top = -((phase + pad - khs[-1]) // stride)
    return k - 1 - khs[-1], len(khs), top


def _strided_dgrad(dy, wt, x_shape, stride, pad, cache, out_dtype=torch.bfloat16):
    n, cin, h, w = x_shape
    kh, kw = wt.shape[2], wt.shape[3]
    plans = []
    for ph in range(stride):
        th = _phase_taps(kh, pad[0], stride, ph)
        for pw in range(stride):
            tw = _phase_taps(kw, pad[1], stride, pw)
            if th is not None and tw is not None and (th[2] < 0 or tw[2] < 0):
                return None
            plans.append((ph, pw, th, tw))
    dx = torch.empty((n, cin, h, w), dtype=out_dtype, device=dy.device, memory_format=torch.channels_last)
    for ph, pw, th, tw in plans:
        rows, cols = (h - ph + stride - 1) // stride, (w - pw + stride - 1) // stride
        if rows <= 0 or cols <= 0:
            continue
        if th is None or tw is None:
            dx[:, :, ph::stride, pw::stride] = 0
            continue
        key = (ph, pw)
        sub = None if cache is None else cache.get(key)
        if sub is None:
            sub = wt[:, :, th[0]::stride, tw[0]::stride].contiguous(memory_format=torch.channels_last)
            if cache is not None:
                cache[key] = sub
        part = _conv2d_launch(dy, sub, None, 1, (th[2], tw[2]), (1, 1), out_dtype, out_hw=(rows, cols))
        dx[:, :, ph::stride, pw::stride] = part
    return dx


def conv2d_data_grad(dy, wb, weight_ref, x_shape, stride, pad, dil, out_dtype=torch.bfloat16, add=None):
    cout, cin, kh, kw = wb.shape
    bpad = (dil[0] * (kh - 1) - pad[0], dil[1] * (kw - 1) - pad[1])
    phase_cache = None
    asm = getattr(weight_ref, '_stp3_assembled', None) if weight_ref is not None else None
    if asm is not None:
        wt = asm['wt']
        phase_cache = asm.setdefault('phases', {})
    elif weight_ref is not None and weight_ref.is_leaf and weight_ref.requires_grad:
        wt = _bf16_weights(weight_ref, need_flipped=True)[1]
        ent = _shadows(weight_ref.device).lookup(weight_ref) if isinstance(weight_ref, torch.nn.Parameter) else None
        if ent is not None and ent['wt'] is wt:
            phase_cache = ent.setdefault('phases', {})
    else:
        wt = wb if kh == kw == 1 else wb.flip(2, 3)
        wt = wt.transpose(0, 1).contiguous(memory_format=torch.channels_last)
    dx = None
    if stride > 1 and tuple(dil) == (1, 1):
        stuffed_flops = 2.0 * x_shape[0] * x_shape[2] * x_shape[3] * cout * cin * kh * kw
        if stuffed_flops >= 5e10:
            dx = _strided_dgrad(dy, wt, x_shape, stride, pad, phase_cache, out_dtype)
    if dx is None:
        g = dy
        if stride > 1:
            n, _, h, w = x_shape
            ho, wo = dy.shape[2], dy.shape[3]
            uh = h + 2 * pad[0] - dil[0] * (kh - 1)
            uw = w + 2 * pad[1] - dil[1] * (kw - 1)
            g = torch.empty((n, cout, uh, uw), dtype=dy.dtype, device=dy.device, memory_format=torch.channels_last).zero_()
            g[:, :, ::stride, ::stride][:, :, :ho, :wo] = dy
        return _conv2d_launch(g, wt, None, 1, bpad, dil, out_dtype, add=add)
    return dx if add is None else dx + add.to(dx.dtype)


def channel_sums(t):
    t, ld = _rows_view(t)
    n, c, h, w = t.shape
    per = 8 if t.dtype == torch.bfloat16 else 4
    if t.dtype not in (torch.bfloat16, torch.float32) or ld % per or c % per or t.data_ptr() % 16:
        return t.float().sum(dim=(0, 2, 3))
    dims = _lib.BnDims(n, h * w, c, ld, ld, ld, _lib.DTYPE_BF16 if t.dtype == torch.bfloat16 else _lib.DTYPE_F32, ACT_NONE,
                       RES_NONE, 0, 0, 0)
    ws, ws_bytes = _bn_workspace(n, c, t.device)
    sums = torch.empty(2 * c, dtype=torch.float32, device=t.device)
    check(_lib.lib().stp3_bn_stats(ctypes.byref(dims), t.data_ptr(), None, ws.data_ptr(), ws_bytes, sums.data_ptr(),
                                   _stream_handle()), 'stp3_bn_stats')
    return sums[:c]


class _Conv2dMfma(torch.autograd.Function):
    @staticmethod
    def forward(ctx, x, weight, bias, stride, pad, dil, out_dtype):
        _need_gpu(x, weight)
        if x.dtype != torch.bfloat16:
            x = x.to(torch.bfloat16)
        wb, _ = _bf16_weights(weight)
        fb = _f32(bias)
        y = _conv2d_launch(x, wb, fb, stride, pad, dil, out_dtype)
        ctx.weight_ref = note_weight_use(weight)
        ctx.weight_stamp = weight_stamp(weight)
        ctx.save_for_backward(x, wb)
        ctx.cfg = (stride, pad, dil, bias is not None, weight.dtype, None if bias is None else bias.dtype)
        return y

    @staticmethod
    def backward(ctx, dy):
        x, wb = ctx.saved_tensors
        check_weight_stamp(ctx.weight_ref, ctx.weight_stamp, 'conv2d backward')
        stride, pad, dil, has_bias, wdtype, bdtype = ctx.cfg
        cout_true, cin, kh, kw = wb.shape
        dy = dy.to(torch.bfloat16).contiguous(memory_format=torch.channels_last)
        cpad = (-cout_true) % 8
        if cpad:
            dy = torch.nn.functional.pad(dy, (0, 0, 0, 0, 0, cpad)).contiguous(memory_format=torch.channels_last)
            wb = torch.nn.functional.pad(wb, (0, 0, 0, 0, 0, 0, 0, cpad)).contiguous(memory_format=torch.channels_last)
        db = None
        if has_bias and ctx.needs_input_grad[2]:
            db = channel_sums(dy)[:cout_true].to(bdtype)
        cout = cout_true + cpad
        dx = dw = None
        bpad = (dil[0] * (kh - 1) - pad[0], dil[1] * (kw - 1) - pad[1])
        need_dx = ctx.needs_input_grad[0]
        hip_dx = need_dx and cout % 8 == 0 and bpad[0] >= 0 and bpad[1] >= 0
        if hip_dx:
# ... 187 lines not shown
```

### st-p3_amd/stp3_amd/ops_fused.py

```python
import ctypes
import os

import torch

from . import _lib, ops, scratch
from ._lib import check

_SE_MLP = True


def conv2d_v2(x, wb, bias, stride, pad, dil, sums_ptr=None):
    return ops._conv2d_launch(x, wb, bias, stride, pad, dil, torch.bfloat16, sums_ptr=sums_ptr)


class _ConvBnAct(torch.autograd.Function):
    @staticmethod
    def forward(ctx, x, weight, cbias, gamma, beta, res, running_mean, running_var, momentum, eps, act, res_mode,
                stride, pad, dil, group, oscale=None, out_slot=None, res_carrier=None, skip_carrier=None):
        return ops.drive_exchange(_ConvBnAct.forward_steps(ctx, x, weight, cbias, gamma, beta, res, running_mean,
                                                           running_var, momentum, eps, act, res_mode, stride, pad, dil,
                                                           group, oscale, out_slot, res_carrier, skip_carrier), group)

    @staticmethod
    def backward(ctx, dy):
        return ops.drive_exchange(_ConvBnAct.backward_steps(ctx, dy), ctx.cfg[3])

    @staticmethod
    def forward_steps(ctx, x, weight, cbias, gamma, beta, res, running_mean, running_var, momentum, eps, act, res_mode,
                      stride, pad, dil, group, oscale=None, out_slot=None, res_carrier=None, skip_carrier=None):
        ops._need_gpu(x, weight)
        if x.dtype != torch.bfloat16:
            x = x.to(torch.bfloat16)
        wb, _ = ops._bf16_weights(weight)
        cout = wb.shape[0]
        dev = x.device
        stat = torch.empty(4 * cout, dtype=torch.float32, device=dev)
        base = stat.data_ptr()
        yc = conv2d_v2(x, wb, ops._f32(cbias), stride, pad, dil, sums_ptr=base)
        n, _, ho, wo = yc.shape
        count = float(n * ho * wo)
        world, exchange = ops.replicas(group)
        if exchange:
            yield stat[:2 * cout]
            count *= world
        ldr = cout
        if res is not None:
            res, ldr = ops._rows_view(res if res.dtype == torch.bfloat16 else res.to(torch.bfloat16))
        else:
            res_mode = ops.RES_NONE
        ldo = cout
        if out_slot is None:
            out = torch.empty_like(yc)
        else:
            out, ldo = slot_view(out_slot, yc)
        osc = ops._f32(oscale)
        dims = _lib.BnDims(n, ho * wo, cout, cout, ldo, ldr, _lib.DTYPE_BF16, act, res_mode, 0, int(osc is not None))
        g32, b32 = ops._f32(gamma), ops._f32(beta)
        check(_lib.lib().stp3_bn_apply_fwd(ctypes.byref(dims), yc.data_ptr(), None, ops._opt_ptr(res), ops._opt_ptr(osc), base, count,
                                           ops._opt_ptr(g32), ops._opt_ptr(b32), eps, momentum, ops._opt_ptr(running_mean),
                                           ops._opt_ptr(running_var), base + 8 * cout, base + 12 * cout, out.data_ptr(),
                                           ops._stream_handle()), 'stp3_bn_apply_fwd')
        ctx.save_for_backward(x, wb, yc, res if res_mode == ops.RES_BEFORE_ACT else None, g32, b32, stat, osc)
        if ldo != cout:
            dims = _lib.BnDims(n, ho * wo, cout, cout, cout, ldr, _lib.DTYPE_BF16, act, res_mode, 0, int(osc is not None))
        ctx.cfg = (dims, count, exchange, group, stride, pad, dil, cbias is not None)
        ctx.carriers = (res_carrier if (res is not None and res_mode == ops.RES_AFTER_ACT) else None, skip_carrier)
        ctx.weight_ref = ops.note_weight_use(weight)
        ctx.weight_stamp = ops.weight_stamp(weight)
        ctx.dtypes = (weight.dtype, None if cbias is None else cbias.dtype, None if gamma is None else gamma.dtype,
                      None if beta is None else beta.dtype, None if res is None else res.dtype)
        return out

    @staticmethod
    def backward_steps(ctx, dy):
        x, wb, yc, res, g32, b32, stat, osc = ctx.saved_tensors
        ops.check_weight_stamp(ctx.weight_ref, ctx.weight_stamp, 'conv_bn_act backward')
        dims, count, exchange, group, stride, pad, dil, has_cbias = ctx.cfg
        wdt, cbdt, gdt, bdt, rdt = ctx.dtypes
        res_carrier, skip_carrier = ctx.carriers
        n, rows, c = dims.N, dims.rows, dims.C
        dev = x.device
        lib = _lib.lib()
        if dy.dtype != torch.bfloat16:
            dy = dy.to(torch.bfloat16)
        dy, ldy = ops._rows_view(dy)
        if ldy != c:
            if ldy % 8 == 0 and dy.data_ptr() % 16 == 0:
                dims = _lib.BnDims(dims.N, dims.rows, dims.C, dims.ldx, ldy, dims.ldr, dims.dtype, dims.act, dims.res_mode, 0,
                                   dims.has_oscale)
            else:
                dy = dy.contiguous(memory_format=torch.channels_last)
        ws, ws_bytes = ops._bn_workspace(n, c, dev)
        sumbuf = torch.empty((n + 1) * 3 * c, dtype=torch.float32, device=dev)
        sums_off = n * 3 * c
        mean_p, invstd_p = stat.data_ptr() + 8 * c, stat.data_ptr() + 12 * c
        dconv = torch.empty_like(yc)
        dres = None
        if dims.res_mode == ops.RES_BEFORE_ACT and ctx.needs_input_grad[5]:
            dres = torch.empty_like(yc)
            if dims.ldr != c:
                res = res.contiguous(memory_format=torch.channels_last)
                dims = _lib.BnDims(dims.N, dims.rows, dims.C, dims.ldx, dims.ldy, c, dims.dtype, dims.act, dims.res_mode, 0,
                                   dims.has_oscale)
        if dims.res_mode == ops.RES_AFTER_ACT and dims.ldy != c:
            dy = dy.contiguous(memory_format=torch.channels_last)
            dims = _lib.BnDims(dims.N, dims.rows, dims.C, dims.ldx, c, dims.ldr, dims.dtype, dims.act, dims.res_mode, 0,
                               dims.has_oscale)
        stream = ops._stream_handle()
        check(lib.stp3_bn_bwd_reduce(ctypes.byref(dims), dy.data_ptr(), yc.data_ptr(), None, ops._opt_ptr(res), ops._opt_ptr(osc), mean_p,
                                     invstd_p, ops._opt_ptr(g32), ops._opt_ptr(b32), ws.data_ptr(), ws_bytes,
                                     sumbuf.data_ptr(), sumbuf.data_ptr() + 4 * sums_off, stream), 'stp3_bn_bwd_reduce')
        lsums = sumbuf[sums_off:].view(3, c)
        gsums = lsums
        if exchange:
            gsums = lsums.clone()
            yield gsums
        check(lib.stp3_bn_apply_bwd(ctypes.byref(dims), dy.data_ptr(), yc.data_ptr(), None, ops._opt_ptr(res), ops._opt_ptr(osc), mean_p,
                                    invstd_p, ops._opt_ptr(g32), ops._opt_ptr(b32), gsums.data_ptr(), count,
                                    dconv.data_ptr(), ops._opt_ptr(dres), stream), 'stp3_bn_apply_bwd')
        dgamma = lsums[1].to(gdt) if gdt is not None and ctx.needs_input_grad[3] else None
        dbeta = lsums[0].to(bdt) if bdt is not None and ctx.needs_input_grad[4] else None
        if dims.res_mode == ops.RES_AFTER_ACT and ctx.needs_input_grad[5]:
            dres = dy
        if dres is not None and rdt is not None and dres.dtype != rdt:
            dres = dres.to(rdt)
        if res_carrier is not None and dres is not None:
            res_carrier.grad, dres = dres, None
        skip_grad = None if skip_carrier is None else skip_carrier.take()
        cout, cin, kh, kw = wb.shape
        dx = dw = dcb = None
        bpad = (dil[0] * (kh - 1) - pad[0], dil[1] * (kw - 1) - pad[1])
        need_dx = ctx.needs_input_grad[0]
        hip_dx = need_dx and cout % 8 == 0 and bpad[0] >= 0 and bpad[1] >= 0
        if hip_dx:
            dx = ops.conv2d_data_grad(dconv, wb, ctx.weight_ref, x.shape, stride, pad, dil, add=skip_grad)
            skip_grad = None
        need_dw = ctx.needs_input_grad[1]
        need_db = has_cbias and ctx.needs_input_grad[2]
        hip_dw = need_dw and cin % 8 == 0 and cout % 8 == 0
        if hip_dw:
            dw = ops._conv2d_wgrad(dconv, x, (cout, cin, kh, kw), stride, pad, dil, leaf=ctx.weight_ref).to(wdt)
            if need_db:
                dcb = ops.channel_sums(dconv).to(cbdt)
        mask = [need_dx and not hip_dx, need_dw and not hip_dw, need_db and not hip_dw]
        if any(mask):
            xd = x if x.is_contiguous(memory_format=torch.channels_last) else x.contiguous(memory_format=torch.channels_last)
            gx, gw, gb = torch.ops.aten.convolution_backward(dconv, xd, wb, [cout] if has_cbias else None, [stride, stride],
                                                             list(pad), list(dil), False, [0, 0], 1, mask)
            if mask[0]:
                dx = gx
            if mask[1]:
                dw = gw.to(wdt)
            if mask[2]:
                dcb = gb.to(cbdt)
        if skip_grad is not None:
            dx = skip_grad if dx is None else dx + skip_grad.to(dx.dtype)
        return (dx, dw, dcb, dgamma, dbeta, dres) + (None,) * 14


EXPAND_DGRAD_IN_APPLY = True


class _PointwiseBnAct(torch.autograd.Function):

    @staticmethod
    def forward(ctx, x, weight, gamma, beta, running_mean, running_var, momentum, eps, act, group, skip_carrier=None):
        return ops.drive_exchange(_PointwiseBnAct.forward_steps(ctx, x, weight, gamma, beta, running_mean, running_var,
                                                                momentum, eps, act, group, skip_carrier), group)

    @staticmethod
    def backward(ctx, dz):
        return ops.drive_exchange(_PointwiseBnAct.backward_steps(ctx, dz), ctx.cfg[3])

    @staticmethod
    def forward_steps(ctx, x, weight, gamma, beta, running_mean, running_var, momentum, eps, act, group, skip_carrier=None):
        ops._need_gpu(x, weight)
        ctx.skip_carrier = skip_carrier
        if x.dtype != torch.bfloat16:
            x = x.to(torch.bfloat16)
        wb, _ = ops._bf16_weights(weight)
        cout, cin = wb.shape[:2]
        n, _, h, w = x.shape
        x, ldx = ops._rows_view(x)
        dev = x.device
        lib = _lib.lib()
        dims = _lib.ConvDims(n, h, w, cin, h, w, cout, 1, 1, 1, 0, 0, 1, 1, ldx, cout, _lib.DTYPE_BF16, 0)
        need = ctypes.c_size_t()
        check(lib.stp3_conv2d_fwd_workspace(ctypes.byref(dims), ctypes.byref(need)), 'stp3_conv2d_fwd_workspace')
        ws = scratch.get('fused', need.value, dev, floor=32 << 20)
        stat = torch.empty(6 * cout, dtype=torch.float32, device=dev)
        stream = ops._stream_handle()
        check(lib.stp3_conv2d_fwd_stats(ctypes.byref(dims), x.data_ptr(), wb.data_ptr(), stat.data_ptr(), ws.data_ptr(),
                                        need.value, stream), 'stp3_conv2d_fwd_stats')
        count = float(n * h * w)
# ... 129 lines not shown
            check(lib.stp3_bn_finalize(stat.data_ptr(), c, count, ops._opt_ptr(g32), ops._opt_ptr(b32), eps, momentum,
                                       ops._opt_ptr(rmean), ops._opt_ptr(rvar), stat.data_ptr() + 8 * c, stream), 'stp3_bn_finalize')
            stats.append(stat)
            params.append((g32, b32))
            cfgs.append((c0, c, stride, pad, dil, cbias is not None, weight.dtype, None if cbias is None else cbias.dtype,
                         None if gamma is None else gamma.dtype, None if beta is None else beta.dtype))
            c0 += c
        if n_prod == 1:
            table = stats[0][2 * ctot:4 * ctot]
        else:
            table = torch.cat([st[2 * c:3 * c] for st, c in zip(stats, couts)] + [st[3 * c:4 * c] for st, c in zip(stats, couts)])
        w2b, _ = ops._bf16_weights(w2)
        cout2 = w2b.shape[0]
        fb2 = ops._f32(b2)
        y = torch.empty((n, cout2, ho, wo), dtype=torch.bfloat16, device=dev, memory_format=torch.channels_last)
        dims2 = _lib.ConvDims(n, ho, wo, ctot, ho, wo, cout2, 1, 1, 1, 0, 0, 1, 1, ctot, cout2, _lib.DTYPE_BF16, int(fb2 is not None))
        check(lib.stp3_conv2d_fwd_pre(ctypes.byref(dims2), zbuf.data_ptr(), w2b.data_ptr(), ops._opt_ptr(fb2), table.data_ptr(),
                                      int(act), y.data_ptr(), stream), 'stp3_conv2d_fwd_pre')
        saved = [zbuf, table, w2b]
        for x, wb, st, (g32, b32) in zip(xs, wbs, stats, params):
            saved += [x, wb, st, g32, b32]
        ctx.save_for_backward(*saved)
        ctx.cfg = (int(act), n_prod, cfgs, count, w2.dtype, None if b2 is None else b2.dtype)
        ctx.weight_refs = [ops.note_weight_use(w2)] + [ops.note_weight_use(p[1]) for p in prods]
        ctx.weight_stamps = [ops.weight_stamp(w2)] + [ops.weight_stamp(p[1]) for p in prods]
        return y

    @staticmethod
    def backward(ctx, dy):
        saved = ctx.saved_tensors
        zbuf, table, w2b = saved[:3]
        act, n_prod, cfgs, count, w2dt, b2dt = ctx.cfg
        for ref, stamp in zip(ctx.weight_refs, ctx.weight_stamps):
            ops.check_weight_stamp(ref, stamp, 'conv_bn_act_conv1x1 backward')
        lib = _lib.lib()
        stream = ops._stream_handle()
        dev = zbuf.device
        n, ctot, ho, wo = zbuf.shape
        cout_true = w2b.shape[0]
        dy = dy.to(torch.bfloat16).contiguous(memory_format=torch.channels_last)
        cpad = (-cout_true) % 8
        if cpad:
            dy = torch.nn.functional.pad(dy, (0, 0, 0, 0, 0, cpad)).contiguous(memory_format=torch.channels_last)
            w2b = torch.nn.functional.pad(w2b, (0, 0, 0, 0, 0, 0, 0, cpad)).contiguous(memory_format=torch.channels_last)
        ref2 = None if cpad else ctx.weight_refs[0]
        db2 = None
        if b2dt is not None and ctx.needs_input_grad[2]:
            db2 = ops.channel_sums(dy)[:cout_true].to(b2dt)
        da = ops.conv2d_data_grad(dy, w2b, ref2, (n, ctot, ho, wo), 1, (0, 0), (1, 1))
        dw2 = None
        if ctx.needs_input_grad[1]:
            dw2 = ops._conv2d_wgrad(dy, zbuf, (cout_true + cpad, ctot, 1, 1), 1, (0, 0), (1, 1), leaf=ref2,
                                    pre=(table, act))[:cout_true].to(w2dt)
        dzbuf = torch.empty_like(zbuf)
        grads = []
        for k, (c0, c, stride, pad, dil, has_cbias, wdt, cbdt, gdt, bdt) in enumerate(cfgs):
            x, wb, stat, g32, b32 = saved[3 + 5 * k:8 + 5 * k]
            base = 4 + _N_PRODUCER_ARGS * k
            need = ctx.needs_input_grad[base:base + 5]
            dak, zk, dconv = da[:, c0:c0 + c], zbuf[:, c0:c0 + c], dzbuf[:, c0:c0 + c]
            dims = _lib.BnDims(n, ho * wo, c, ctot, ctot, c, _lib.DTYPE_BF16, act, ops.RES_NONE, 0, 0)
            ws, ws_bytes = ops._bn_workspace(n, c, dev)
            sumbuf = torch.empty((n + 1) * 3 * c, dtype=torch.float32, device=dev)
            sums_off = n * 3 * c
            mean_p, invstd_p = stat.data_ptr() + 16 * c, stat.data_ptr() + 20 * c
            check(lib.stp3_bn_bwd_reduce(ctypes.byref(dims), dak.data_ptr(), zk.data_ptr(), None, None, None, mean_p, invstd_p,
                                         ops._opt_ptr(g32), ops._opt_ptr(b32), ws.data_ptr(), ws_bytes, sumbuf.data_ptr(),
                                         sumbuf.data_ptr() + 4 * sums_off, stream), 'stp3_bn_bwd_reduce')
            lsums = sumbuf[sums_off:].view(3, c)
            check(lib.stp3_bn_apply_bwd(ctypes.byref(dims), dak.data_ptr(), zk.data_ptr(), None, None, None, mean_p, invstd_p,
                                        ops._opt_ptr(g32), ops._opt_ptr(b32), lsums.data_ptr(), count, dconv.data_ptr(), None,
                                        stream), 'stp3_bn_apply_bwd')
            dgamma = lsums[1].to(gdt) if gdt is not None and need[3] else None
            dbeta = lsums[0].to(bdt) if bdt is not None and need[4] else None
            cout, cin, kh, kw = wb.shape
            ref = ctx.weight_refs[1 + k]
            dx = dw = dcb = None
            if need[0]:
                dx = ops.conv2d_data_grad(dconv, wb, ref, x.shape, stride, pad, dil)
            if need[1]:
                dw = ops._conv2d_wgrad(dconv, x, (cout, cin, kh, kw), stride, pad, dil, leaf=ref).to(wdt)
            if has_cbias and need[2]:
                dcb = ops.channel_sums(dconv).to(cbdt)
            grads += [dx, dw, dcb, dgamma, dbeta] + [None] * (_N_PRODUCER_ARGS - 5)
        return (None, dw2, db2, None) + tuple(grads)


def pre_fold_pays(n, h, w, channels):
    return n * h * w * channels >= PRE_FOLD_MIN_ELEMENTS


def pre_fold_supported(x, weight, stride, padding, dilation, w2):
    if not PRE_FOLD or ops.replicas(None)[1]:
        return False
    cout, cin, kh, kw = weight.shape
    p, d = ops._pair(padding), ops._pair(dilation)
    if cout % 8 or cin % 8 or w2.shape[1] % 8 or tuple(w2.shape[2:]) != (1, 1) or cout > 4096:
        return False
    if d[0] * (kh - 1) - p[0] < 0 or d[1] * (kw - 1) - p[1] < 0:
        return False
    n, _, h, w = x.shape
    return n * h * w * max(cin, w2.shape[1]) * 2 < (1 << 31)


def conv_bn_act_conv1x1(producers, act, w2, b2):
    flat = []
    for x, weight, cbias, bn, stride, padding, dilation in producers:
        if bn.num_batches_tracked is not None:
            ops.bump_batch_counter(bn)
        flat += [x, weight, cbias, bn.weight, bn.bias, bn.running_mean, bn.running_var, ops.bn_momentum(bn), float(bn.eps),
                 ops._pair(stride)[0], ops._pair(padding), ops._pair(dilation)]
    return _ConvBnActConv1x1.apply(int(act), w2, b2, len(producers), *flat)


slot_view = ops.slot_view


class _JoinSlices(torch.autograd.Function):

    @staticmethod
    def forward(ctx, holder, *parts):
        buf = holder[0]
        c0 = 0
        for p in parts:
            if p.data_ptr() != buf.data_ptr() + c0 * buf.element_size() or p.shape[1] + c0 > buf.shape[1]:
                raise _lib.Stp3HipError('join_slices: a part does not lie in its slot')
            c0 += p.shape[1]
        if c0 != buf.shape[1]:
            raise _lib.Stp3HipError('join_slices: the parts do not fill the buffer')
        ctx.sizes = [p.shape[1] for p in parts]
        return buf.view_as(buf)

    @staticmethod
    def backward(ctx, g):
# ... 356 lines not shown
```

### st-p3_amd/stp3_amd/profiling.py

```python
import torch

ENABLED = False
RECORDS = []


def _obj(arg):
    return getattr(arg, '_obj', arg)


def _esize(dtype_code):
    return 2 if dtype_code == 1 else 4


def _conv_flops(args):
    d = _obj(args[0])
    return 2.0 * d.N * d.Ho * d.Wo * d.Cout * d.KH * d.KW * d.Cin


def _conv_bytes(args):
    d = _obj(args[0])
    return (2.0 * d.N * d.H * d.W * d.Cin + float(_esize(1 if d.out_dtype == 1 else 0)) * d.N * d.Ho * d.Wo * d.Cout
            + 2.0 * d.Cout * d.KH * d.KW * d.Cin)


def _wgrad_bytes(args):
    d = _obj(args[0])
    return 2.0 * d.N * d.H * d.W * d.Cin + 2.0 * d.N * d.Ho * d.Wo * d.Cout + 4.0 * d.Cout * d.KH * d.KW * d.Cin


def _conv_label(args):
    d = _obj(args[0])
    return (f'{d.KH}x{d.KW}' + (f'/{d.stride}' if d.stride != 1 else '') + (f' d{d.dil_h}' if d.dil_h != 1 else '') +
            f' {d.Cin}->{d.Cout} @{d.Ho}x{d.Wo} x{d.N}')


LABEL = {'stp3_conv2d_fwd': _conv_label, 'stp3_conv2d_fwd_add': _conv_label, 'stp3_conv2d_wgrad': _conv_label, 'stp3_conv2d_wgrad_partials': _conv_label,
         'stp3_conv2d_fwd_pre': _conv_label, 'stp3_conv2d_wgrad_pre': _conv_label}


def _bn_bytes(tensors):
    def f(args):
        d = _obj(args[0])
        n = tensors + (1 if d.res_mode else 0)
        return float(n) * d.N * d.rows * d.C * _esize(d.dtype)
    return f


def _dw_bytes(args):
    d = _obj(args[0])
    return float(d.N * d.C * (d.H * d.W + d.Ho * d.Wo)) * _esize(d.dtype)


def _se_bytes(tensors):
    def f(args):
        d = _obj(args[0])
        return float(tensors) * d.N * d.rows * d.C * _esize(d.dtype)
    return f


def _se_pool_bytes(args):
    d = _obj(args[0])
    return float(2 if args[2] else 1) * d.N * d.rows * d.C * _esize(d.dtype)


WORK = {
    'stp3_conv2d_fwd': ('conv_fwd_dgrad', _conv_flops),
    'stp3_conv2d_fwd_add': ('conv_fwd_dgrad', _conv_flops),
    'stp3_conv2d_bn_bwd_apply_dx': ('conv_fwd_dgrad', _conv_flops),
    'stp3_conv2d_fwd_pre': ('conv_fwd_dgrad', _conv_flops),
    'stp3_conv2d_wgrad': ('conv_wgrad', _conv_flops),
    'stp3_conv2d_wgrad_pre': ('conv_wgrad', _conv_flops),
    'stp3_conv2d_wgrad_partials': ('conv_wgrad', _conv_flops),
    'stp3_conv2d_wgrad_reduce_batch': ('conv_wgrad', lambda args: 0.0),
    'stp3_bn_stats': ('batchnorm', _bn_bytes(1)),
    'stp3_bn_apply_fwd': ('batchnorm', _bn_bytes(2)),
    'stp3_bn_fwd_train': ('batchnorm', _bn_bytes(2)),
    'stp3_bn_bwd_reduce': ('batchnorm', _bn_bytes(0)),
    'stp3_bn_apply_bwd': ('batchnorm', _bn_bytes(3)),
    'stp3_bn_bwd_train': ('batchnorm', _bn_bytes(3)),
    'stp3_dwconv2d_fwd': ('depthwise', _dw_bytes),
    'stp3_dwconv2d_fwd_stats': ('depthwise', _dw_bytes),
    'stp3_dwconv2d_fwd_stats_bn': ('depthwise', _dw_bytes),
    'stp3_dwconv2d_bwd_data': ('depthwise', _dw_bytes),
    'stp3_dwconv2d_bwd_weight': ('depthwise', _dw_bytes),
    'stp3_dwconv2d_bwd_weight_oihw': ('depthwise', _dw_bytes),
    'stp3_se_pool': ('squeeze_excite', _se_pool_bytes),
    'stp3_se_scale': ('squeeze_excite', _se_bytes(2)),
    'stp3_se_pool_act': ('mbconv', _se_bytes(1)),
    'stp3_mbconv_scale_act': ('mbconv', _se_bytes(2)),
    'stp3_mbconv_bwd_reduce': ('mbconv', _se_bytes(2)),
    'stp3_mbconv_bwd_apply': ('mbconv', _se_bytes(3)),
}


class TimedLib:
    def __init__(self, handle):
        self._handle = handle

    def __getattr__(self, name):
        fn = getattr(self._handle, name)
        spec = WORK.get(name)
        if spec is None:
            wrapped = fn
        else:
            family, work = spec
            label = LABEL.get(name)

            def wrapped(*args):
                start = torch.cuda.Event(enable_timing=True)
                end = torch.cuda.Event(enable_timing=True)
                start.record()
                rc = fn(*args)
                end.record()
                RECORDS.append((family, work(args), start, end, label(args) if label else None,
                                (_wgrad_bytes if 'wgrad' in name else _conv_bytes)(args) if label else None))
                return rc
        self.__dict__[name] = wrapped
        return wrapped


def enable(on=True):
    global ENABLED
    ENABLED = bool(on)
    if on:
        RECORDS.clear()
# ... 26 lines not shown
```

Baseline: 113.8 samples/s.

## Fold BN-activation backward apply into 1x1 conv dgrad and wgrad operand loads

For large 1x1 stride-1 conv+BN(+ReLU) layers, the backward no longer materialises dconv with a separate bn_apply_bwd pass. The dgrad and wgrad GEMM kernels instead load dy and the saved pre-BN activation z, then apply the per-channel BN/activation gradient from an LDS table while staging the operand. This removes one full-tensor write and two reads per folded layer. In exchange, each of the two consumer GEMMs now reads z and recomputes the gradient, which adds register pressure and ALU work inside the GEMM load path.

Result: no change. 113.9 samples/s (median of 2 runs) (+0.2%).

```diff
diff --git a/include/stp3_hip.h b/include/stp3_hip.h
--- a/include/stp3_hip.h
+++ b/include/stp3_hip.h
@@ -211,6 +211,24 @@
                         int32_t pre_act, void* y, void* stream);
 int stp3_conv2d_wgrad_pre(const stp3_conv_dims* dims, const void* dy, const void* x, const float* pre_coef, int32_t pre_act,
                           float* dw, void* workspace, size_t workspace_bytes, void* stream);
+
+typedef struct stp3_bn_grad_operand {
+    const void* z;
+    const float* mean;
+    const float* invstd;
+    const float* gamma;
+    const float* beta;
+    const float* gsums;
+    double count;
+    int32_t ldz;
+    int32_t act;
+} stp3_bn_grad_operand;
+int stp3_conv2d_fwd_bngrad(const stp3_conv_dims* dims, const void* dy, const void* w, const stp3_bn_grad_operand* g,
+                           const void* add, int32_t ldadd, void* dx, void* stream);
+int stp3_conv2d_wgrad_bngrad(const stp3_conv_dims* dims, const void* dy, const void* x, const stp3_bn_grad_operand* g, float* dw,
+                             void* workspace, size_t workspace_bytes, void* stream);
+int stp3_conv2d_wgrad_bngrad_partials(const stp3_conv_dims* dims, const void* dy, const void* x, const stp3_bn_grad_operand* g,
+                                      void* partials, size_t partials_bytes, int32_t* splits, void* stream);
 
 typedef struct stp3_se_dims {
     int32_t N, rows, C, ld;
diff --git a/st-p3_amd/csrc/stp3_bn_grad.h b/st-p3_amd/csrc/stp3_bn_grad.h
--- /dev/null
+++ b/st-p3_amd/csrc/stp3_bn_grad.h
@@ -0,0 +1,85 @@
+#pragma once
+#include <stdint.h>
+
+struct BnGradConsts {
+    float cs, ct, a2, a3;
+};
+
+template <bool TRAIN>
+__device__ __forceinline__ BnGradConsts bn_grad_consts(float mu, float is, float ga, float be, float g0, float g1, float inv_count) {
+    const float k0 = TRAIN ? g0 * inv_count : 0.f;
+    const float k1 = TRAIN ? g1 * inv_count : 0.f;
+    BnGradConsts k;
+    k.cs = ga * is;
+    k.ct = be - mu * k.cs;
+    k.a2 = -(k.cs * is) * k1;
+    k.a3 = -k.cs * k0 - k.a2 * mu;
+    return k;
+}
+
+__device__ __forceinline__ float bn_grad_fma(float a, float b, float c) { return fmaf(a, b, c); }
+__device__ __forceinline__ stp3_f32x2 bn_grad_fma(stp3_f32x2 a, stp3_f32x2 b, stp3_f32x2 c) { return pk_fma(a, b, c); }
+
+template <int ACT>
+__device__ __forceinline__ float bn_grad_act(float pre) {
+    if (ACT == STP3_ACT_RELU) return pre > 0.f ? 1.f : 0.f;
+    if (ACT == STP3_ACT_SWISH) {
+        const float s = fast_sigmoid(pre);
+        return s * (1.f + pre * (1.f - s));
+    }
+    return 1.f;
+}
+template <int ACT>
+__device__ __forceinline__ stp3_f32x2 bn_grad_act(stp3_f32x2 pre) {
+    return stp3_f32x2{bn_grad_act<ACT>(pre.x), bn_grad_act<ACT>(pre.y)};
+}
+
+template <int ACT, bool PRE_RES, typename V>
+__device__ __forceinline__ V bn_grad_apply(V& g, V x, V res, V cs, V ct, V a2, V a3) {
+    if (ACT != STP3_ACT_NONE) {
+        V pre = bn_grad_fma(x, cs, ct);
+        if (PRE_RES) pre += res;
+        g *= bn_grad_act<ACT>(pre);
+    }
+    return bn_grad_fma(cs, g, bn_grad_fma(a2, x, a3));
+}
+
+template <int ACT>
+__device__ __forceinline__ uint32_t bn_grad_pair(uint32_t dy, uint32_t z, stp3_f32x2 cs, stp3_f32x2 ct, stp3_f32x2 a2, stp3_f32x2 a3) {
+    stp3_f32x2 g = {__uint_as_float(dy << 16), __uint_as_float(dy & 0xffff0000u)};
+    const stp3_f32x2 x = {__uint_as_float(z << 16), __uint_as_float(z & 0xffff0000u)};
+    const stp3_f32x2 out = bn_grad_apply<ACT, false>(g, x, x, cs, ct, a2, a3);
+    return pack_bf16(out.x, out.y);
+}
+
+typedef float stp3_f32x4 __attribute__((ext_vector_type(4)));
+template <int ACT>
+__device__ __forceinline__ stp3_u32x4 bn_grad_piece(stp3_u32x4 dy, stp3_u32x4 z, const float* k, uint32_t mask) {
+    stp3_u32x4 o;
+#pragma unroll
+    for (int r = 0; r < 4; ++r) {
+        const stp3_f32x4 lo = *reinterpret_cast<const stp3_f32x4*>(k + 8 * r), hi = *reinterpret_cast<const stp3_f32x4*>(k + 8 * r + 4);
+        o[r] = bn_grad_pair<ACT>(dy[r], z[r], stp3_f32x2{lo[0], lo[1]}, stp3_f32x2{lo[2], lo[3]}, stp3_f32x2{hi[0], hi[1]},
+                                 stp3_f32x2{hi[2], hi[3]}) & mask;
+    }
+    return o;
+}
+
+struct BnGradOperand {
+    const uint16_t* z;
+    const float *mean, *invstd, *gamma, *beta, *gsums;
+    float inv_count;
+    int ldz, C;
+};
+
+__device__ __forceinline__ void bn_grad_table(float* tab, const BnGradOperand& g, int c0, int n, int tid, int nthreads) {
+    for (int e = tid; e < n; e += nthreads) {
+        const int c = c0 + e;
+        BnGradConsts k = {0.f, 0.f, 0.f, 0.f};
+        if (c < g.C)
+            k = bn_grad_consts<true>(g.mean[c], g.invstd[c], g.gamma ? g.gamma[c] : 1.f, g.beta ? g.beta[c] : 0.f, g.gsums[c],
+                                     g.gsums[g.C + c], g.inv_count);
+        float* p = tab + (e >> 1) * 8 + (e & 1);
+        p[0] = k.cs; p[2] = k.ct; p[4] = k.a2; p[6] = k.a3;
+    }
+}
diff --git a/st-p3_amd/csrc/stp3_bnact.hip b/st-p3_amd/csrc/stp3_bnact.hip
--- a/st-p3_amd/csrc/stp3_bnact.hip
+++ b/st-p3_amd/csrc/stp3_bnact.hip
@@ -6,6 +6,8 @@
 
 #include "stp3_cdna.h"
 #include "stp3_hip.h"
+
+#include "stp3_bn_grad.h"
 
 namespace {
 
@@ -457,12 +459,9 @@
         const float is = ok ? invstd_[c] : 0.f;
         const float ga = ok ? (gamma ? gamma[c] : 1.f) : 0.f;
         const float be = ok ? (beta ? beta[c] : 0.f) : 0.f;
-        const float k0 = (TRAIN && ok) ? gsums[c] * inv_count : 0.f;
-        const float k1 = (TRAIN && ok) ? gsums[d.C + c] * inv_count : 0.f;
-        cs[j] = ga * is;
-        ct[j] = be - mu * cs[j];
-        a2[j] = -(cs[j] * is) * k1;
-        a3[j] = -cs[j] * k0 - a2[j] * mu;
+        const BnGradConsts k = bn_grad_consts<TRAIN>(mu, is, ga, be, (TRAIN && ok) ? gsums[c] : 0.f,
+                                                     (TRAIN && ok) ? gsums[d.C + c] : 0.f, inv_count);
+        cs[j] = k.cs; ct[j] = k.ct; a2[j] = k.a2; a3[j] = k.a3;
     }
     const float os = d.has_oscale ? oscale[n] : 1.f;
     const T* xs = x + (size_t)n * d.rows * d.ldx + c0;
@@ -502,13 +501,8 @@
 #pragma unroll
                     for (int j = 0; j < VEC; ++j) {
                         float gg = g[j] * os;
-                        if (ACT != STP3_ACT_NONE) {
-                            float pre = fmaf(v[j], cs[j], ct[j]);
-                            if (PRE_RES) pre += rv[j];
-                            gg *= act_grad_c<ACT>(pre);
-                        }
+                        v[j] = bn_grad_apply<ACT, PRE_RES>(gg, v[j], PRE_RES ? rv[j] : 0.f, cs[j], ct[j], a2[j], a3[j]);
                         g[j] = gg;
-                        v[j] = fmaf(cs[j], gg, fmaf(a2[j], v[j], a3[j]));
                     }
                     Io<T, VEC>::store(dxs + (size_t)(r + u * step) * d.ldx, v);
                     if (drs) Io<T, VEC>::store(drs + (size_t)(r + u * step) * d.ldr, g);
diff --git a/st-p3_amd/csrc/stp3_conv.hip b/st-p3_amd/csrc/stp3_conv.hip
--- a/st-p3_amd/csrc/stp3_conv.hip
+++ b/st-p3_amd/csrc/stp3_conv.hip
@@ -5,6 +5,8 @@
 
 #include "stp3_cdna.h"
 #include "stp3_hip.h"
+
+#include "stp3_bn_grad.h"
 
 namespace {
 
@@ -46,7 +48,8 @@
 
 __device__ __forceinline__ int lds_piece(int r, int j) { return (r * 8 + (j ^ ((r >> 1) & 7))) * 16; }
 
-enum { kModePlain = 0, kModeStats = 1, kModeBnAct = 2, kModeBwdReduce = 3, kModeBwdApply = 4, kModeAffine = 5 };
+enum { kModePlain = 0, kModeStats = 1, kModeBnAct = 2, kModeBwdReduce = 3, kModeBwdApply = 4, kModeAffine = 5,
+       kModePlainGrad = 6, kModePlainGradRelu = 7 };
 constexpr bool mode_bwd(int m) { return m == kModeBwdReduce || m == kModeBwdApply; }
 
 struct EpiArgs {
@@ -66,9 +69,11 @@
     int hw;
     const float* pre;
     int pre_off;
+    BnGradOperand grad;
 };
 
-enum { kPreNone = 0, kPreAffine = 1, kPreRelu = 2 };
+enum { kPreNone = 0, kPreAffine = 1, kPreRelu = 2, kPreGrad = 3, kPreGradRelu = 4 };
+constexpr bool pre_is_grad(int pre) { return pre == kPreGrad || pre == kPreGradRelu; }
 template <int PRE>
 __device__ __forceinline__ uint32_t pre_pair(uint32_t wd, stp3_f32x2 cs, stp3_f32x2 ct) {
     const stp3_f32x2 e0 = {__uint_as_float(wd << 16), __uint_as_float(wd & 0xffff0000u)};
@@ -83,6 +88,15 @@
     for (int r = 0; r < 4; ++r) o[r] = pre_pair<PRE>(v[r], cs[r], ct[r]) & mask;
     return o;
 }
+
+enum { kGradNone = 0, kGradAffine = 1, kGradRelu = 2 };
+constexpr int grad_act(int g) { return g == kGradRelu ? STP3_ACT_RELU : STP3_ACT_NONE; }
+constexpr int mode_grad(int mode) { return mode == kModePlainGrad ? kGradAffine : mode == kModePlainGradRelu ? kGradRelu : kGradNone; }
+#if defined(__AMDGCN__)
+#define STP3_SCHED_FENCE() __builtin_amdgcn_sched_barrier(0)
+#else
+#define STP3_SCHED_FENCE()
+#endif
 
 template <int ACT>
 __device__ __forceinline__ float epi_act(float v) {
@@ -165,15 +179,26 @@
     float* const ptab = reinterpret_cast<float*>(smem + ep.pre_off);
     const int kpad = steps * kBK;
     int prek = 0;
-    if (PRE) {
+    constexpr bool GRAD = pre_is_grad(PRE);
+    if (GRAD) {
+        bn_grad_table(ptab, ep.grad, 0, kpad, tid, 256);
+        __syncthreads();
+    } else if (PRE) {
         for (int e = tid; e < 2 * kpad; e += 256) {
             const int h = e >= kpad, c = e - h * kpad;
             ptab[e] = c < d.Cin ? ep.pre[h * d.Cin + c] : 0.f;
         }
         __syncthreads();
     }
-
-    u32x4 ra[4], rb[BN / 32];
+    const stp3_buffer zbuf = make_buffer(ep.grad.z, GRAD ? (uint32_t)((size_t)d.M * ep.grad.ldz * 2) : 0u);
+    uint32_t zoff[4];
+#pragma unroll
+    for (int i = 0; i < 4; ++i) {
+        const int m = m0 + rr + 32 * i;
+        zoff[i] = (GRAD && m < d.M) ? (uint32_t)m * (uint32_t)ep.grad.ldz * 2u : kBufOob;
+    }
+
+    u32x4 ra[4], rb[BN / 32], rz[GRAD ? 4 : 1];
     auto load_step = [&]() {
         const bool kvalid = tap < taps;
         const int dh = kh * d.dil_h, dw = kw * d.dil_w;
@@ -187,6 +212,7 @@
                     ok = ok & ((unsigned)hi < (unsigned)d.H) & ((unsigned)wi < (unsigned)d.W);
                 }
                 ra[i] = buffer_load16(xbuf, ok ? poff[i] + (uint32_t)toff * 2u : kBufOob);
+                if (GRAD) rz[GRAD ? i : 0] = buffer_load16(zbuf, ok ? zoff[i] + (uint32_t)ci * 2u : kBufOob);
             } else {
                 bool ok = kvalid && prow[i] != zero;
                 if (!pointwise) {
@@ -211,7 +237,15 @@
         }
     };
     auto store_step = [&](uint8_t* buf) {
-        if (PRE) {
+        if (GRAD) {
+#pragma unroll
+            for (int i = 0; i < 4; ++i) {
+                STP3_SCHED_FENCE();
+                ra[i] = bn_grad_piece<grad_act(PRE == kPreGradRelu ? kGradRelu : kGradAffine)>(ra[i], rz[GRAD ? i : 0], ptab + prek * 4,
+                                                                                                rmask[i]);
+            }
+            STP3_SCHED_FENCE();
+        } else if (PRE) {
             const f32x4 s0 = *reinterpret_cast<const f32x4*>(ptab + prek), s1 = *reinterpret_cast<const f32x4*>(ptab + prek + 4);
             const f32x4 t0 = *reinterpret_cast<const f32x4*>(ptab + kpad + prek);
             const f32x4 t1 = *reinterpret_cast<const f32x4*>(ptab + kpad + prek + 4);
@@ -558,10 +592,11 @@
     }
 }
 
-template <int PP, int KMAX, int MODE>
+template <int PP, int KMAX, int MODE_>
 __global__ __launch_bounds__(256, 2) void pointwise_rows_kernel(ConvDims d, int ksteps, int tiles_co, const uint16_t* __restrict__ x,
                                                              const uint16_t* __restrict__ w, uint16_t* __restrict__ y,
                                                              float* __restrict__ stat_partial, EpiArgs ep) {
+    constexpr int GRAD = mode_grad(MODE_), MODE = GRAD ? kModePlain : MODE_;
     constexpr int NT = (PP + 3) / 4;
     constexpr int RPI = 64 / PP;
     constexpr int NIT = (32 + RPI - 1) / RPI;
@@ -590,6 +625,8 @@
         if (r < PP * 8 && k0 < d.Cin) v = *reinterpret_cast<const u32x4*>(w + (size_t)(co0 + r) * d.Cin + k0);
         *reinterpret_cast<u32x4*>(wimg + r * LDW + k0) = v;
     }
+    const float* const gtab = reinterpret_cast<const float*>(smem + ep.pre_off);
+    if (GRAD) bn_grad_table(reinterpret_cast<float*>(smem + ep.pre_off), ep.grad, 0, ksteps * 16, tid, 256);
     __syncthreads();
     const int px = lane & 31, half = lane >> 5;
     const int cp = lane % PP, prow = lane / PP;
@@ -601,20 +638,32 @@
 #pragma unroll
     for (int r = 0; r < 4; ++r) s1[r] = s2[r] = stp3_f32x2{0.f, 0.f};
     const uint16_t* const zero = reinterpret_cast<const uint16_t*>(&g_zero16);
-    u32x4 cur[KMAX], nxt[KMAX];
+    u32x4 cur[KMAX], nxt[KMAX], nxtz[GRAD ? KMAX : 1];
     const int ntiles = (d.M + 31) / 32;
     const int stride_t = ngroups * 4;
     auto load_tile = [&](int t, u32x4 (&f)[KMAX]) {
         const int m = t * 32 + px;
         const uint16_t* row = (t < ntiles && m < d.M) ? x + (size_t)m * d.ldx : nullptr;
+        const uint16_t* zrow = (GRAD && row) ? ep.grad.z + (size_t)m * ep.grad.ldz : nullptr;
 #pragma unroll
         for (int ks = 0; ks < KMAX; ++ks) {
             const int k0 = ks * 16 + half * 8;
             if (ks < ksteps) f[ks] = *reinterpret_cast<const u32x4*>((row && k0 < d.Cin) ? row + k0 : zero);
-        }
+            if (GRAD && ks < ksteps) nxtz[GRAD ? ks : 0] = *reinterpret_cast<const u32x4*>((zrow && k0 < d.Cin) ? zrow + k0 : zero);
+        }
+    };
+    auto grad_tile = [&](int t, u32x4 (&f)[KMAX]) {
+        const uint32_t mask = (t < ntiles && t * 32 + px < d.M) ? 0xffffffffu : 0u;
+#pragma unroll
+        for (int ks = 0; ks < KMAX; ++ks) {
+            STP3_SCHED_FENCE();
+            if (ks < ksteps) f[ks] = bn_grad_piece<grad_act(GRAD)>(f[ks], nxtz[GRAD ? ks : 0], gtab + (ks * 16 + half * 8) * 4, mask);
+        }
+        STP3_SCHED_FENCE();
     };
     int t = group * 4 + wave;
     load_tile(t, cur);
+    if (GRAD) grad_tile(t, cur);
     for (; t < ntiles; t += stride_t) {
         load_tile(t + stride_t, nxt);
         const int mbase = t * 32;
@@ -704,6 +753,7 @@
             }
         }
         __builtin_amdgcn_wave_barrier();
+        if (GRAD) grad_tile(t + stride_t, nxt);
 #pragma unroll
         for (int ks = 0; ks < KMAX; ++ks) cur[ks] = nxt[ks];
     }
@@ -726,14 +776,20 @@
     }
 }
 
-template <int KMAX, int MODE>
+template <int KMAX, int MODE_>
 __global__ __launch_bounds__(256) void pointwise_direct_kernel(ConvDims d, int ksteps, int cblocks, int ngroups,
                                                                const uint16_t* __restrict__ x, const uint16_t* __restrict__ w,
                                                                uint16_t* __restrict__ y, float* __restrict__ stat_partial,
                                                                EpiArgs ep) {
+    constexpr int GRAD = mode_grad(MODE_), MODE = GRAD ? kModePlain : MODE_;
     constexpr bool kSums = MODE == kModePlain || MODE == kModeStats || MODE == kModeBwdReduce;
     __shared__ float red[kSums ? 4 * 64 * 33 : 1];
+    __shared__ __attribute__((aligned(16))) float gtab[GRAD ? KMAX * 16 * 4 : 4];
     const int tid = threadIdx.x, lane = tid & 63;
+    if (GRAD) {
+        bn_grad_table(gtab, ep.grad, 0, ksteps * 16, tid, 256);
+        __syncthreads();
+    }
     const int wave = __builtin_amdgcn_readfirstlane(tid >> 6);
     const int slot = xcd_order(blockIdx.x, gridDim.x) * 4 + wave;
     const int group = slot / cblocks, cb = slot - group * cblocks;
@@ -763,20 +819,32 @@
         for (int r = 0; r < 4; ++r) s1[s][r] = s2[s][r] = stp3_f32x2{0.f, 0.f};
     }
     const int ntiles = (d.M + 31) / 32;
-    u32x4 cur[KMAX], nxt[KMAX];
+    u32x4 cur[KMAX], nxt[KMAX], nxtz[GRAD ? KMAX : 1];
     auto load_tile = [&](int t, u32x4 (&f)[KMAX]) {
         const int m = t * 32 + px;
         const uint16_t* row = (live && t < ntiles && m < d.M) ? x + (size_t)m * d.ldx : nullptr;
+        const uint16_t* zrow = (GRAD && row) ? ep.grad.z + (size_t)m * ep.grad.ldz : nullptr;
 #pragma unroll
         for (int ks = 0; ks < KMAX; ++ks) {
             if (ks < ksteps) {
                 const int k0 = ks * 16 + h * 8;
                 f[ks] = *reinterpret_cast<const u32x4*>((row && k0 < d.Cin) ? row + k0 : zero);
-            }
-        }
+                if (GRAD) nxtz[GRAD ? ks : 0] = *reinterpret_cast<const u32x4*>((zrow && k0 < d.Cin) ? zrow + k0 : zero);
+            }
+        }
+    };
+    auto grad_tile = [&](int t, u32x4 (&f)[KMAX]) {
+        const uint32_t mask = (live && t < ntiles && t * 32 + px < d.M) ? 0xffffffffu : 0u;
+#pragma unroll
+        for (int ks = 0; ks < KMAX; ++ks) {
+            STP3_SCHED_FENCE();
+            if (ks < ksteps) f[ks] = bn_grad_piece<grad_act(GRAD)>(f[ks], nxtz[GRAD ? ks : 0], gtab + (ks * 16 + h * 8) * 4, mask);
+        }
+        STP3_SCHED_FENCE();
     };
     int t = live ? group : ntiles;
     load_tile(t, cur);
+    if (GRAD) grad_tile(t, cur);
     for (; t < ntiles; t += ngroups) {
         load_tile(t + ngroups, nxt);
         const int m = t * 32 + px;
@@ -819,6 +887,7 @@
             if (MODE == kModeBnAct || MODE == kModeBwdApply || MODE == kModeAffine)
                 *reinterpret_cast<uint4*>(y + (size_t)m * d.ldy + ch[s]) = make_uint4(ow[0], ow[1], ow[2], ow[3]);
         }
+        if (GRAD) grad_tile(t + ngroups, nxt);
 #pragma unroll
         for (int ks = 0; ks < KMAX; ++ks) cur[ks] = nxt[ks];
     }
@@ -889,11 +958,13 @@
     bf16x8 v;
 };
 
-template <int TCO, int TCI, bool BUF = false, int PRE = kPreNone>
+template <int TCO, int TCI, bool BUF = false, int PRE = kPreNone, int GRAD = kGradNone>
 __global__ __launch_bounds__(256) void conv2d_wgrad_kernel(ConvDims d, int tiles_ci, int ksteps_per_block, int tap_fold,
                                                            int xcd_chunks, const uint16_t* __restrict__ dy,
                                                            const uint16_t* __restrict__ x,
-                                                           float* __restrict__ partial, const float* __restrict__ pre = nullptr) {
+                                                           float* __restrict__ partial, const float* __restrict__ pre = nullptr,
+                                                           BnGradOperand gop = BnGradOperand()) {
+    static_assert(!GRAD || BUF, "GRAD stages through buffer resources");
     constexpr int TA = TCO / 64, TB = TCI / 64;
     constexpr int kImgA = kBK * TCO * 2;
     constexpr int kStage = kBK * (TCO + TCI) * 2;
@@ -954,6 +1025,14 @@
                 pct[r][h] = b_ok ? pre[d.Cin + chb + 2 * r + h] : 0.f;
             }
     }
+    float* const gtab = reinterpret_cast<float*>(smem + 2 * kStage);
+    const stp3_buffer zbuf = make_buffer(gop.z, GRAD ? (uint32_t)((size_t)d.M * gop.ldz * 2) : 0u);
+    const uint32_t pitchz = (uint32_t)gop.ldz * 2u;
+    uint32_t abits = 0;
+    if (GRAD) {
+        bn_grad_table(gtab, gop, co0, TCO, tid, 256);
+        __syncthreads();
+    }
 
     const int hw = d.Ho * d.Wo;
     const int qa = kBK / hw, qr = kBK - qa * hw, qb = qr / d.Wo, qc = qr - qb * d.Wo;
@@ -967,7 +1046,7 @@
     }
     const int tap_h = kh * d.dil_h - d.pad_h, tap_w = kw * d.dil_w - d.pad_w;
 
-    u32x4 rawa[NA], rawb[NB];
+    u32x4 rawa[NA], rawb[NB], rawz[GRAD ? NA : 1];
     auto load_step = [&](int step) {
         const int mbase = step * kBK;
 #pragma unroll
@@ -975,6 +1054,10 @@
             const int m = mbase + ra0 + RA * i;
             if (BUF) rawa[i] = buffer_load16(abuf, (a_ok & (m < d.M)) ? (uint32_t)m * pitcha + cola : kBufOob);
             else rawa[i] = *reinterpret_cast<const u32x4*>(m < d.M ? srca + (size_t)(unsigned)m * lda : zero);
+            if (GRAD) {
+                rawz[GRAD ? i : 0] = buffer_load16(zbuf, (a_ok & (m < d.M)) ? (uint32_t)m * pitchz + cola : kBufOob);
+                abits = (i ? abits : 0u) | ((a_ok & (m < d.M)) ? 1u << i : 0u);
+            }
         }
         const bool inside = mbase + lane < d.M;
         if (!tap_fold) {
@@ -1010,6 +1093,14 @@
         if (PRE) {
 #pragma unroll
             for (int i = 0; i < NB; ++i) rawb[i] = pre_piece<PRE>(rawb[i], pcs, pct, bmask[i]);
+        }
+        if (GRAD) {
+#pragma unroll
+            for (int i = 0; i < NA; ++i) {
+                STP3_SCHED_FENCE();
+                rawa[i] = bn_grad_piece<grad_act(GRAD)>(rawa[i], rawz[GRAD ? i : 0], gtab + pa * 32, 0u - ((abits >> i) & 1u));
+            }
+            STP3_SCHED_FENCE();
         }
 #pragma unroll
         for (int i = 0; i < NA; ++i) *reinterpret_cast<u32x4*>(buf + wg_piece<TCO>(ra0 + RA * i, pa)) = rawa[i];
@@ -1195,12 +1286,32 @@
     return STP3_OK;
 }
 
+template <int TCO, int TCI, int GRAD>
+int wgrad_launch_grad(const ConvDims& d, int tco, int tci, int taps, int splits, int ksteps, int xcd, const void* dy, const void* x,
+                      void* workspace, const BnGradOperand& gop, hipStream_t s) {
+    const size_t lds = (size_t)2 * (TCO + TCI) * kBK * 2 + (size_t)TCO * 16;
+    hipError_t e = hipFuncSetAttribute(reinterpret_cast<const void*>(&conv2d_wgrad_kernel<TCO, TCI, true, kPreNone, GRAD>),
+                                       hipFuncAttributeMaxDynamicSharedMemorySize, (int)lds);
+    if (e != hipSuccess) return -(int)e;
+    hipLaunchKernelGGL((conv2d_wgrad_kernel<TCO, TCI, true, kPreNone, GRAD>), dim3(tco * tci, taps, splits), dim3(256), lds, s, d,
+                       tci, ksteps, 0, xcd, (const uint16_t*)dy, (const uint16_t*)x, (float*)workspace, (const float*)nullptr, gop);
+    return STP3_OK;
+}
+
 template <int TCO, int TCI>
 int wgrad_launch(const ConvDims& d, int tco, int tci, int taps, int splits, int ksteps, int fold, const void* dy,
-                 const void* x, void* workspace, hipStream_t s, const float* pre = nullptr, int pre_act = STP3_ACT_NONE) {
+                 const void* x, void* workspace, hipStream_t s, const float* pre = nullptr, int pre_act = STP3_ACT_NONE,
+                 const BnGradOperand* gop = nullptr, int gact = STP3_ACT_NONE) {
     const size_t lds = (size_t)2 * (TCO + TCI) * kBK * 2;
     const int xcd = taps <= 9 && (int64_t)tco * tci * taps * splits < (1LL << 31);
     const bool buf = (size_t)d.M * d.ldy * 2 < (1ull << 31) && (size_t)d.N * d.H * d.W * d.ldx * 2 < (1ull << 31);
+    if (gop) {
+        if (!buf || fold || pre || taps != 1 || !((size_t)d.M * gop->ldz * 2 < (1ull << 31))) return STP3_EUNSUP;
+        constexpr int TCIG = (TCO == 64 && TCI == 64) ? 128 : TCI;
+        if (gact == STP3_ACT_RELU)
+            return wgrad_launch_grad<TCO, TCIG, kGradRelu>(d, tco, tci, taps, splits, ksteps, xcd, dy, x, workspace, *gop, s);
+        return wgrad_launch_grad<TCO, TCIG, kGradAffine>(d, tco, tci, taps, splits, ksteps, xcd, dy, x, workspace, *gop, s);
+    }
     if (pre) {
         if (!buf || fold) return STP3_EUNSUP;
         constexpr int TCIP = (TCO == 64 && TCI == 64) ? 128 : TCI;
@@ -1296,6 +1407,11 @@
 template <int PP, int KMAX>
 int pointwise_rows_launch_mode(int mode, const ConvDims& d, int ksteps, int tiles_co, unsigned nwg, size_t lds, const void* x,
                                const void* w, void* y, float* partial, const EpiArgs& ep, hipStream_t s) {
+    if (ep.grad.z) {
+        if (ep.act == STP3_ACT_RELU)
+            return pointwise_rows_launch_one<PP, KMAX, kModePlainGradRelu>(d, ksteps, tiles_co, nwg, lds, x, w, y, partial, ep, s);
+        return pointwise_rows_launch_one<PP, KMAX, kModePlainGrad>(d, ksteps, tiles_co, nwg, lds, x, w, y, partial, ep, s);
+    }
     switch (mode) {
         case kModePlain: return pointwise_rows_launch_one<PP, KMAX, kModePlain>(d, ksteps, tiles_co, nwg, lds, x, w, y, partial, ep, s);
         case kModeStats: return pointwise_rows_launch_one<PP, KMAX, kModeStats>(d, ksteps, tiles_co, nwg, lds, x, w, y, partial, ep, s);
@@ -1332,6 +1448,10 @@
 template <int KMAX>
 int pointwise_direct_launch_mode(int mode, const ConvDims& d, int ksteps, unsigned gx, int* parts, const void* x, const void* w,
                                  void* y, float* partial, const EpiArgs& ep, hipStream_t s) {
+    if (ep.grad.z) {
+        if (ep.act == STP3_ACT_RELU) return pointwise_direct_launch_one<KMAX, kModePlainGradRelu>(d, ksteps, gx, parts, x, w, y, partial, ep, s);
+        return pointwise_direct_launch_one<KMAX, kModePlainGrad>(d, ksteps, gx, parts, x, w, y, partial, ep, s);
+    }
     switch (mode) {
         case kModePlain: return pointwise_direct_launch_one<KMAX, kModePlain>(d, ksteps, gx, parts, x, w, y, partial, ep, s);
         case kModeStats: return pointwise_direct_launch_one<KMAX, kModeStats>(d, ksteps, gx, parts, x, w, y, partial, ep, s);
@@ -1360,19 +1480,24 @@
         const int pp = rows_small ? d.Cout / 8 : (d.Cout % 128 == 0 ? 16 : 8), nt = (pp + 3) / 4;
         const int tiles_co = d.Cout / (pp * 8);
         if (ep.dx && !(rows_small && mode == kModeBwdApply && d.Cin <= 32)) return STP3_EUNSUP;
-        const size_t lds = (size_t)nt * 32 * (ksteps * 16 + 8) * 2 + (size_t)4 * 32 * (nt * 32 + 8) * 2 +
-                           (ep.dx ? (size_t)32 * (nt * 32 + 8) * 2 : 0);
+        size_t lds = (size_t)nt * 32 * (ksteps * 16 + 8) * 2 + (size_t)4 * 32 * (nt * 32 + 8) * 2 +
+                     (ep.dx ? (size_t)32 * (nt * 32 + 8) * 2 : 0);
+        EpiArgs epl = ep;
+        if (ep.grad.z) {
+            epl.pre_off = (int)((lds + 15) / 16 * 16);
+            lds = (size_t)epl.pre_off + (size_t)ksteps * 16 * 16;
+        }
         unsigned per_cu = (unsigned)((160 * 1024) / lds);
         if (per_cu > 3) per_cu = 3;
         unsigned groups = (256 * per_cu + tiles_co - 1) / tiles_co;
         if (groups > gx) groups = gx;
         parts = (int)groups;
         const unsigned nwg = groups * (unsigned)tiles_co;
-        if (pp == 18) rc = pointwise_rows_launch_mode<18, 2>(mode, d, ksteps, tiles_co, nwg, lds, x, w, y, partial, ep, s);
-        else if (pp == 24) rc = pointwise_rows_launch_mode<24, 2>(mode, d, ksteps, tiles_co, nwg, lds, x, w, y, partial, ep, s);
-        else if (pp == 8) rc = pointwise_rows_launch_mode<8, 8>(mode, d, ksteps, tiles_co, nwg, lds, x, w, y, partial, ep, s);
-        else if (ksteps <= 4) rc = pointwise_rows_launch_mode<16, 4>(mode, d, ksteps, tiles_co, nwg, lds, x, w, y, partial, ep, s);
-        else rc = pointwise_rows_launch_mode<16, 8>(mode, d, ksteps, tiles_co, nwg, lds, x, w, y, partial, ep, s);
+        if (pp == 18) rc = pointwise_rows_launch_mode<18, 2>(mode, d, ksteps, tiles_co, nwg, lds, x, w, y, partial, epl, s);
+        else if (pp == 24) rc = pointwise_rows_launch_mode<24, 2>(mode, d, ksteps, tiles_co, nwg, lds, x, w, y, partial, epl, s);
+        else if (pp == 8) rc = pointwise_rows_launch_mode<8, 8>(mode, d, ksteps, tiles_co, nwg, lds, x, w, y, partial, epl, s);
+        else if (ksteps <= 4) rc = pointwise_rows_launch_mode<16, 4>(mode, d, ksteps, tiles_co, nwg, lds, x, w, y, partial, epl, s);
+        else rc = pointwise_rows_launch_mode<16, 8>(mode, d, ksteps, tiles_co, nwg, lds, x, w, y, partial, epl, s);
     } else {
         if (ep.dx) return STP3_EUNSUP;
         if (ksteps <= 2) rc = pointwise_direct_launch_mode<2>(mode, d, ksteps, gx, &parts, x, w, y, partial, ep, s);
@@ -1428,7 +1553,22 @@
         ep.act = act;
         return pointwise_run(d, x, w, y, sums, partial, gx, s, mode, ep);
     }
-    if (ep.pre) {
+    const bool grad = ep.grad.z != nullptr;
+    if (grad) {
+        if (mode != kModePlain || sums || ep.pre || d.out_f32 || p->KH != 1 || p->KW != 1 || p->stride != 1 || p->pad_h || p->pad_w ||
+            p->H != p->Ho || p->W != p->Wo || p->Cin > 2048)
+            return STP3_EUNSUP;
+        if (ep.grad.C != p->Cin || ep.grad.ldz % 8 || ep.grad.ldz < p->Cin || ((uintptr_t)ep.grad.z & 15)) return STP3_EUNSUP;
+        if (!((size_t)d.M * d.ldx * 2 < (1ull << 31) && (size_t)d.M * ep.grad.ldz * 2 < (1ull << 31) &&
+              (size_t)d.Cout * d.Ktot * 2 < (1ull << 31)))
+            return STP3_EUNSUP;
+        if (ep.add && (p->Cout % 8 || p->ldy % 8 || ep.ldadd % 8 || ep.ldadd < p->Cout || ((uintptr_t)ep.add & 15) || ((uintptr_t)y & 15)))
+            return STP3_EUNSUP;
+        if (!ep.add && pointwise_applies(p, y)) {
+            ep.act = act;
+            return pointwise_run(d, x, w, y, nullptr, nullptr, gx, s, mode, ep);
+        }
+    } else if (ep.pre) {
         if (mode != kModePlain || sums || ep.add || p->KH != 1 || p->KW != 1 || p->stride != 1 || p->pad_h || p->pad_w ||
             p->H != p->Ho || p->W != p->Wo || p->Cin > 4096)
             return STP3_EUNSUP;
@@ -1454,6 +1594,17 @@
     if ((int64_t)gx * tiles_co >= (1LL << 31)) return STP3_EUNSUP;
     const dim3 grid(gx * (unsigned)tiles_co);
     int rc;
+    if (grad) {
+        ep.pre_off = (int)((lds + 15) / 16 * 16);
+        lds = (size_t)ep.pre_off + (size_t)4 * steps * kBK * sizeof(float);
+        if (act == STP3_ACT_RELU)
+            rc = wide ? igemm_launch_pre<128, kPreGradRelu>(d, grid, lds, tiles_co, x, w, bias, y, ep, s)
+                      : igemm_launch_pre<64, kPreGradRelu>(d, grid, lds, tiles_co, x, w, bias, y, ep, s);
+        else
+            rc = wide ? igemm_launch_pre<128, kPreGrad>(d, grid, lds, tiles_co, x, w, bias, y, ep, s)
+                      : igemm_launch_pre<64, kPreGrad>(d, grid, lds, tiles_co, x, w, bias, y, ep, s);
+        return rc ? rc : status();
+    }
     if (ep.pre) {
         ep.pre_off = (int)((lds + 15) / 16 * 16);
         lds = (size_t)ep.pre_off + (size_t)2 * steps * kBK * sizeof(float);
@@ -1600,8 +1751,14 @@
 }
 
 static int wgrad_partials(const stp3_conv_dims* p, const void* dy, const void* x, void* workspace, size_t workspace_bytes,
-                          int* splits_out, hipStream_t s, const float* pre_coef = nullptr, int pre_act = STP3_ACT_NONE) {
+                          int* splits_out, hipStream_t s, const float* pre_coef = nullptr, int pre_act = STP3_ACT_NONE,
+                          const BnGradOperand* gop = nullptr, int gact = STP3_ACT_NONE) {
     if (!p || !dy || !x || !workspace) return STP3_EINVAL;
+    if (gop) {
+        if (gact != STP3_ACT_NONE && gact != STP3_ACT_RELU) return STP3_EINVAL;
+        if (p->KH != 1 || p->KW != 1 || p->stride != 1 || p->pad_h || p->pad_w || p->H != p->Ho || p->W != p->Wo) return STP3_EUNSUP;
+        if (gop->C != p->Cout || gop->ldz % 8 || gop->ldz < p->Cout || ((uintptr_t)gop->z & 15)) return STP3_EUNSUP;
+    }
     if (pre_coef) {
         if (pre_act != STP3_ACT_NONE && pre_act != STP3_ACT_RELU) return STP3_EINVAL;
         if (p->KH != 1 || p->KW != 1 || p->stride != 1 || p->pad_h || p->pad_w || p->H != p->Ho || p->W != p->Wo) return STP3_EUNSUP;
@@ -1627,10 +1784,10 @@
     d.out_f32 = 1; d.has_bias = 0; d.M = (int)M; d.kchunks = 0; d.Ktot = p->KH * p->KW * p->Cin;
     int rc;
     if (tco_sz == 128 && tci_sz == 128)
-        rc = wgrad_launch<128, 128>(d, tco, tci, taps, splits, ksteps, fold, dy, x, workspace, s, pre_coef, pre_act);
-    else if (tco_sz == 128) rc = wgrad_launch<128, 64>(d, tco, tci, taps, splits, ksteps, fold, dy, x, workspace, s, pre_coef, pre_act);
-    else if (tci_sz == 128) rc = wgrad_launch<64, 128>(d, tco, tci, taps, splits, ksteps, fold, dy, x, workspace, s, pre_coef, pre_act);
-    else rc = wgrad_launch<64, 64>(d, tco, tci, taps, splits, ksteps, fold, dy, x, workspace, s, pre_coef, pre_act);
+        rc = wgrad_launch<128, 128>(d, tco, tci, taps, splits, ksteps, fold, dy, x, workspace, s, pre_coef, pre_act, gop, gact);
+    else if (tco_sz == 128) rc = wgrad_launch<128, 64>(d, tco, tci, taps, splits, ksteps, fold, dy, x, workspace, s, pre_coef, pre_act, gop, gact);
+    else if (tci_sz == 128) rc = wgrad_launch<64, 128>(d, tco, tci, taps, splits, ksteps, fold, dy, x, workspace, s, pre_coef, pre_act, gop, gact);
+    else rc = wgrad_launch<64, 64>(d, tco, tci, taps, splits, ksteps, fold, dy, x, workspace, s, pre_coef, pre_act, gop, gact);
     if (rc) return rc;
     *splits_out = splits;
     return status();
@@ -1667,6 +1824,58 @@
     if (!splits) return STP3_EINVAL;
     int n = 0;
     int rc = wgrad_partials(p, dy, x, partials, partials_bytes, &n, (hipStream_t)stream, pre_coef, pre_act);
+    if (rc) return rc;
+    *splits = n;
+    return STP3_OK;
+}
+
+static int grad_operand(const stp3_bn_grad_operand* g, int32_t channels, BnGradOperand* out) {
+    if (!g || !g->z || !g->mean || !g->invstd || !g->gsums || !(g->count >= 1.0)) return STP3_EINVAL;
+    if (g->act != STP3_ACT_NONE && g->act != STP3_ACT_RELU) return STP3_EINVAL;
+    out->z = (const uint16_t*)g->z;
+    out->mean = g->mean; out->invstd = g->invstd; out->gamma = g->gamma; out->beta = g->beta; out->gsums = g->gsums;
+    out->inv_count = (float)(1.0 / g->count);
+    out->ldz = g->ldz;
+    out->C = channels;
+    return STP3_OK;
+}
+
+int stp3_conv2d_fwd_bngrad(const stp3_conv_dims* p, const void* dy, const void* w, const stp3_bn_grad_operand* g, const void* add,
+                           int32_t ldadd, void* y, void* stream) {
+    if (!p) return STP3_EINVAL;
+    EpiArgs ep = EpiArgs();
+    int rc = grad_operand(g, p->Cin, &ep.grad);
+    if (rc) return rc;
+    if (p->has_bias) return STP3_EUNSUP;
+    ep.add = (const uint16_t*)add;
+    ep.ldadd = ldadd;
+    return igemm_run(p, dy, w, nullptr, y, nullptr, nullptr, 0, stream, kModePlain, g->act, ep);
+}
+
+int stp3_conv2d_wgrad_bngrad(const stp3_conv_dims* p, const void* dy, const void* x, const stp3_bn_grad_operand* g, float* dw,
+                             void* workspace, size_t workspace_bytes, void* stream) {
+    if (!dw || !p) return STP3_EINVAL;
+    BnGradOperand gop;
+    int rc = grad_operand(g, p->Cout, &gop);
+    if (rc) return rc;
+    hipStream_t s = (hipStream_t)stream;
+    int splits = 0;
+    rc = wgrad_partials(p, dy, x, workspace, workspace_bytes, &splits, s, nullptr, STP3_ACT_NONE, &gop, g->act);
+    if (rc) return rc;
+    const size_t wsize = (size_t)p->Cout * p->KH * p->KW * p->Cin;
+    hipLaunchKernelGGL(conv2d_wgrad_reduce_kernel, dim3((unsigned)((wsize + 63) / 64)), dim3(256), 0, s, splits, wsize,
+                       (const float*)workspace, dw);
+    return status();
+}
+
+int stp3_conv2d_wgrad_bngrad_partials(const stp3_conv_dims* p, const void* dy, const void* x, const stp3_bn_grad_operand* g,
+                                      void* partials, size_t partials_bytes, int32_t* splits, void* stream) {
+    if (!splits || !p) return STP3_EINVAL;
+    BnGradOperand gop;
+    int rc = grad_operand(g, p->Cout, &gop);
+    if (rc) return rc;
+    int n = 0;
+    rc = wgrad_partials(p, dy, x, partials, partials_bytes, &n, (hipStream_t)stream, nullptr, STP3_ACT_NONE, &gop, g->act);
     if (rc) return rc;
     *splits = n;
     return STP3_OK;
diff --git a/st-p3_amd/stp3_amd/_lib.py b/st-p3_amd/stp3_amd/_lib.py
--- a/st-p3_amd/stp3_amd/_lib.py
+++ b/st-p3_amd/stp3_amd/_lib.py
@@ -41,6 +41,12 @@
 class WgradJob(ctypes.Structure):
     _fields_ = [('partials', ctypes.c_void_p), ('dw', ctypes.c_void_p), ('numel', ctypes.c_int64), ('splits', ctypes.c_int32),
                 ('reserved', ctypes.c_int32)]
+
+
+class BnGradOperand(ctypes.Structure):
+    _fields_ = [('z', ctypes.c_void_p), ('mean', ctypes.c_void_p), ('invstd', ctypes.c_void_p), ('gamma', ctypes.c_void_p),
+                ('beta', ctypes.c_void_p), ('gsums', ctypes.c_void_p), ('count', ctypes.c_double), ('ldz', ctypes.c_int32),
+                ('act', ctypes.c_int32)]
 
 
 class LayerNormDims(ctypes.Structure):
@@ -291,6 +297,12 @@
     'stp3_conv2d_fwd_pre': (c_int, [ctypes.POINTER(ConvDims), c_void_p, c_void_p, c_void_p, c_void_p, c_int32, c_void_p, c_void_p]),
     'stp3_conv2d_wgrad_pre': (c_int, [ctypes.POINTER(ConvDims), c_void_p, c_void_p, c_void_p, c_int32, c_void_p, c_void_p, c_size_t,
                                       c_void_p]),
+    'stp3_conv2d_fwd_bngrad': (c_int, [ctypes.POINTER(ConvDims), c_void_p, c_void_p, ctypes.POINTER(BnGradOperand), c_void_p, c_int32,
+                                       c_void_p, c_void_p]),
+    'stp3_conv2d_wgrad_bngrad': (c_int, [ctypes.POINTER(ConvDims), c_void_p, c_void_p, ctypes.POINTER(BnGradOperand), c_void_p,
+                                         c_void_p, c_size_t, c_void_p]),
+    'stp3_conv2d_wgrad_bngrad_partials': (c_int, [ctypes.POINTER(ConvDims), c_void_p, c_void_p, ctypes.POINTER(BnGradOperand),
+                                                  c_void_p, c_size_t, ctypes.POINTER(c_int32), c_void_p]),
     'stp3_conv2d_wgrad_reduce_batch': (c_int, [c_int32, ctypes.POINTER(WgradJob), c_void_p]),
     'stp3_conv2d_prep_weights': (c_int, [c_void_p, c_int32, ctypes.c_int64, c_void_p]),
     'stp3_conv2d_scatter_weight_grads': (c_int, [c_void_p, c_int32, ctypes.c_int64, c_void_p]),
diff --git a/st-p3_amd/stp3_amd/ops.py b/st-p3_amd/stp3_amd/ops.py
--- a/st-p3_amd/stp3_amd/ops.py
+++ b/st-p3_amd/stp3_amd/ops.py
@@ -1082,7 +1082,15 @@
         return g
 
 
-def _conv2d_launch(x, wb, bias, stride, pad, dil, out_dtype, sums_ptr=None, out_hw=None, add=None, out_slot=None):
+class BnGradFold:
+
+    def __init__(self, z, ldz, stat, mean_off, invstd_off, gamma, beta, gsums, count, act):
+        self.keep = (z, stat, gamma, beta, gsums)
+        self.operand = _lib.BnGradOperand(z.data_ptr(), stat.data_ptr() + mean_off, stat.data_ptr() + invstd_off, _opt_ptr(gamma),
+                                          _opt_ptr(beta), gsums.data_ptr(), float(count), int(ldz), int(act))
+
+
+def _conv2d_launch(x, wb, bias, stride, pad, dil, out_dtype, sums_ptr=None, out_hw=None, add=None, out_slot=None, grad=None):
     n, cin, h, w = x.shape
     cout, _, kh, kw = wb.shape
     x, ldx = _rows_view(x)
@@ -1104,6 +1112,20 @@
         nbytes = ctypes.c_size_t()
         check(lib.stp3_conv2d_fwd_workspace(ctypes.byref(dims), ctypes.byref(nbytes)), 'stp3_conv2d_fwd_workspace')
         ws_ptr, ws_bytes = scratch.get('conv_stat', nbytes.value, x.device, floor=8 << 20).data_ptr(), nbytes.value
+    if grad is not None:
+        assert sums_ptr is None and out_slot is None and bias is None and out_dtype == torch.bfloat16
+        later = None
+        add_ptr, ldadd = None, 0
+        if add is not None:
+            add, ldadd = _rows_view(add)
+            if (add.dtype == torch.bfloat16 and tuple(add.shape) == tuple(y.shape) and cout % 8 == 0 and ldadd % 8 == 0
+                    and add.data_ptr() % 16 == 0):
+                add_ptr = _ptr(add)
+            else:
+                later, ldadd = add, 0
+        check(lib.stp3_conv2d_fwd_bngrad(ctypes.byref(dims), _ptr(x), _ptr(wb), ctypes.byref(grad.operand), add_ptr, ldadd, _ptr(y),
+                                         _stream()), 'stp3_conv2d_fwd_bngrad')
+        return y if later is None else y + later.to(y.dtype)
     if add is not None:
         assert sums_ptr is None
         add, ldadd = _rows_view(add)
@@ -1123,7 +1145,8 @@
 DIRECT_BUCKET_GRADS = True
 
 
-def _conv2d_wgrad(dy, x, wshape, stride, pad, dil, leaf=None, pre=None):
+def _conv2d_wgrad(dy, x, wshape, stride, pad, dil, leaf=None, pre=None, grad=None):
+    assert pre is None or grad is None
     cout, cin, kh, kw = wshape
     pre_ptr, pre_act = (None, 0) if pre is None else (pre[0].data_ptr(), int(pre[1]))
     n, _, h, w = x.shape
@@ -1160,12 +1183,21 @@
         slot = arena.take(nbytes.value)
         if slot is not None:
             splits = ctypes.c_int32()
-            check(lib.stp3_conv2d_wgrad_partials(ctypes.byref(dims), _ptr(dy), _ptr(x), pre_ptr, pre_act, slot,
-                                                 ctypes.c_size_t(nbytes.value), ctypes.byref(splits), _stream()),
-                  'stp3_conv2d_wgrad_partials')
+            if grad is not None:
+                check(lib.stp3_conv2d_wgrad_bngrad_partials(ctypes.byref(dims), _ptr(dy), _ptr(x), ctypes.byref(grad.operand), slot,
+                                                            ctypes.c_size_t(nbytes.value), ctypes.byref(splits), _stream()),
+                      'stp3_conv2d_wgrad_bngrad_partials')
+            else:
+                check(lib.stp3_conv2d_wgrad_partials(ctypes.byref(dims), _ptr(dy), _ptr(x), pre_ptr, pre_act, slot,
+                                                     ctypes.c_size_t(nbytes.value), ctypes.byref(splits), _stream()),
+                      'stp3_conv2d_wgrad_partials')
             arena.jobs.append((slot, dw.data_ptr(), cout * cin * kh * kw, splits.value))
             return dw
     ws = scratch.get('conv_wgrad', nbytes.value, x.device, floor=64 << 20)
+    if grad is not None:
+        check(lib.stp3_conv2d_wgrad_bngrad(ctypes.byref(dims), _ptr(dy), _ptr(x), ctypes.byref(grad.operand), _ptr(dw), _ptr(ws),
+                                           ctypes.c_size_t(nbytes.value), _stream()), 'stp3_conv2d_wgrad_bngrad')
+        return dw
     if pre is not None:
         check(lib.stp3_conv2d_wgrad_pre(ctypes.byref(dims), _ptr(dy), _ptr(x), pre_ptr, pre_act, _ptr(dw), _ptr(ws),
                                         ctypes.c_size_t(nbytes.value), _stream()), 'stp3_conv2d_wgrad_pre')
@@ -1704,8 +1736,9 @@
     return dx
 
 
-def conv2d_data_grad(dy, wb, weight_ref, x_shape, stride, pad, dil, out_dtype=torch.bfloat16, add=None):
+def conv2d_data_grad(dy, wb, weight_ref, x_shape, stride, pad, dil, out_dtype=torch.bfloat16, add=None, grad=None):
     cout, cin, kh, kw = wb.shape
+    assert grad is None or (kh == kw == 1 and stride == 1 and tuple(pad) == (0, 0))
     bpad = (dil[0] * (kh - 1) - pad[0], dil[1] * (kw - 1) - pad[1])
     phase_cache = None
     asm = getattr(weight_ref, '_stp3_assembled', None) if weight_ref is not None else None
@@ -1734,7 +1767,7 @@
             uw = w + 2 * pad[1] - dil[1] * (kw - 1)
             g = torch.empty((n, cout, uh, uw), dtype=dy.dtype, device=dy.device, memory_format=torch.channels_last).zero_()
             g[:, :, ::stride, ::stride][:, :, :ho, :wo] = dy
-        return _conv2d_launch(g, wt, None, 1, bpad, dil, out_dtype, add=add)
+        return _conv2d_launch(g, wt, None, 1, bpad, dil, out_dtype, add=add, grad=grad)
     return dx if add is None else dx + add.to(dx.dtype)
 
 
diff --git a/st-p3_amd/stp3_amd/ops_fused.py b/st-p3_amd/stp3_amd/ops_fused.py
--- a/st-p3_amd/stp3_amd/ops_fused.py
+++ b/st-p3_amd/stp3_amd/ops_fused.py
@@ -11,6 +11,26 @@
 
 def conv2d_v2(x, wb, bias, stride, pad, dil, sums_ptr=None):
     return ops._conv2d_launch(x, wb, bias, stride, pad, dil, torch.bfloat16, sums_ptr=sums_ptr)
+
+
+GRAD_FOLD = True
+GRAD_FOLD_MIN_ELEMENTS = 1 << 24
+GRAD_FOLD_MIN_CHANNELS = 64
+
+
+def grad_fold_applies(wshape, n, rows, ldy, ldz, stride, pad, dil, act, res_mode, has_cbias, has_oscale, exchange, dy):
+    cout, cin, kh, kw = wshape
+    if not GRAD_FOLD or exchange or ops.replicas(None)[1]:
+        return False
+    if (kh, kw) != (1, 1) or stride != 1 or tuple(pad) != (0, 0) or tuple(dil) != (1, 1) or cout % 8 or cin % 8 or cout > 2048:
+        return False
+    if act not in (ops.ACT_NONE, ops.ACT_RELU) or res_mode == ops.RES_BEFORE_ACT or has_cbias or has_oscale:
+        return False
+    if ldy % 8 or ldz % 8 or dy.data_ptr() % 16 or dy.dtype != torch.bfloat16:
+        return False
+    if n * rows * max(ldy, ldz, cin) * 2 >= (1 << 31):
+        return False
+    return n * rows * cout >= GRAD_FOLD_MIN_ELEMENTS and min(cin, cout) >= GRAD_FOLD_MIN_CHANNELS
 
 
 class _ConvBnAct(torch.autograd.Function):
@@ -94,7 +114,9 @@
         sumbuf = torch.empty((n + 1) * 3 * c, dtype=torch.float32, device=dev)
         sums_off = n * 3 * c
         mean_p, invstd_p = stat.data_ptr() + 8 * c, stat.data_ptr() + 12 * c
-        dconv = torch.empty_like(yc)
+        fold = grad_fold_applies(wb.shape, n, rows, c if dims.res_mode == ops.RES_AFTER_ACT else dims.ldy, c, stride, pad, dil,
+                                 dims.act, dims.res_mode, has_cbias, osc is not None, exchange, dy)
+        dconv = None if fold else torch.empty_like(yc)
         dres = None
         if dims.res_mode == ops.RES_BEFORE_ACT and ctx.needs_input_grad[5]:
             dres = torch.empty_like(yc)
@@ -115,9 +137,14 @@
         if exchange:
             gsums = lsums.clone()
             yield gsums
-        check(lib.stp3_bn_apply_bwd(ctypes.byref(dims), dy.data_ptr(), yc.data_ptr(), None, ops._opt_ptr(res), ops._opt_ptr(osc), mean_p,
-                                    invstd_p, ops._opt_ptr(g32), ops._opt_ptr(b32), gsums.data_ptr(), count,
-                                    dconv.data_ptr(), ops._opt_ptr(dres), stream), 'stp3_bn_apply_bwd')
+        gop = None
+        if fold:
+            gop = ops.BnGradFold(yc, c, stat, 8 * c, 12 * c, g32, b32, gsums, count, dims.act)
+            dconv = dy
+        else:
+            check(lib.stp3_bn_apply_bwd(ctypes.byref(dims), dy.data_ptr(), yc.data_ptr(), None, ops._opt_ptr(res), ops._opt_ptr(osc),
+                                        mean_p, invstd_p, ops._opt_ptr(g32), ops._opt_ptr(b32), gsums.data_ptr(), count,
+                                        dconv.data_ptr(), ops._opt_ptr(dres), stream), 'stp3_bn_apply_bwd')
         dgamma = lsums[1].to(gdt) if gdt is not None and ctx.needs_input_grad[3] else None
         dbeta = lsums[0].to(bdt) if bdt is not None and ctx.needs_input_grad[4] else None
         if dims.res_mode == ops.RES_AFTER_ACT and ctx.needs_input_grad[5]:
@@ -133,13 +160,13 @@
         need_dx = ctx.needs_input_grad[0]
         hip_dx = need_dx and cout % 8 == 0 and bpad[0] >= 0 and bpad[1] >= 0
         if hip_dx:
-            dx = ops.conv2d_data_grad(dconv, wb, ctx.weight_ref, x.shape, stride, pad, dil, add=skip_grad)
+            dx = ops.conv2d_data_grad(dconv, wb, ctx.weight_ref, x.shape, stride, pad, dil, add=skip_grad, grad=gop)
             skip_grad = None
         need_dw = ctx.needs_input_grad[1]
         need_db = has_cbias and ctx.needs_input_grad[2]
         hip_dw = need_dw and cin % 8 == 0 and cout % 8 == 0
         if hip_dw:
-            dw = ops._conv2d_wgrad(dconv, x, (cout, cin, kh, kw), stride, pad, dil, leaf=ctx.weight_ref).to(wdt)
+            dw = ops._conv2d_wgrad(dconv, x, (cout, cin, kh, kw), stride, pad, dil, leaf=ctx.weight_ref, grad=gop).to(wdt)
             if need_db:
                 dcb = ops.channel_sums(dconv).to(cbdt)
         mask = [need_dx and not hip_dx, need_dw and not hip_dw, need_db and not hip_dw]
@@ -375,13 +402,15 @@
         if ctx.needs_input_grad[1]:
             dw2 = ops._conv2d_wgrad(dy, zbuf, (cout_true + cpad, ctot, 1, 1), 1, (0, 0), (1, 1), leaf=ref2,
                                     pre=(table, act))[:cout_true].to(w2dt)
-        dzbuf = torch.empty_like(zbuf)
+        folds = [grad_fold_applies(saved[4 + 5 * k].shape, n, ho * wo, ctot, ctot, cfg[2], cfg[3], cfg[4], act, ops.RES_NONE, cfg[5],
+                                   False, False, da) and da[:, cfg[0]:].data_ptr() % 16 == 0 for k, cfg in enumerate(cfgs)]
+        dzbuf = None if all(folds) else torch.empty_like(zbuf)
         grads = []
         for k, (c0, c, stride, pad, dil, has_cbias, wdt, cbdt, gdt, bdt) in enumerate(cfgs):
             x, wb, stat, g32, b32 = saved[3 + 5 * k:8 + 5 * k]
             base = 4 + _N_PRODUCER_ARGS * k
             need = ctx.needs_input_grad[base:base + 5]
-            dak, zk, dconv = da[:, c0:c0 + c], zbuf[:, c0:c0 + c], dzbuf[:, c0:c0 + c]
+            dak, zk, dconv = da[:, c0:c0 + c], zbuf[:, c0:c0 + c], None if folds[k] else dzbuf[:, c0:c0 + c]
             dims = _lib.BnDims(n, ho * wo, c, ctot, ctot, c, _lib.DTYPE_BF16, act, ops.RES_NONE, 0, 0)
             ws, ws_bytes = ops._bn_workspace(n, c, dev)
             sumbuf = torch.empty((n + 1) * 3 * c, dtype=torch.float32, device=dev)
@@ -391,18 +420,23 @@
                                          ops._opt_ptr(g32), ops._opt_ptr(b32), ws.data_ptr(), ws_bytes, sumbuf.data_ptr(),
                                          sumbuf.data_ptr() + 4 * sums_off, stream), 'stp3_bn_bwd_reduce')
             lsums = sumbuf[sums_off:].view(3, c)
-            check(lib.stp3_bn_apply_bwd(ctypes.byref(dims), dak.data_ptr(), zk.data_ptr(), None, None, None, mean_p, invstd_p,
-                                        ops._opt_ptr(g32), ops._opt_ptr(b32), lsums.data_ptr(), count, dconv.data_ptr(), None,
-                                        stream), 'stp3_bn_apply_bwd')
+            gop = None
+            if folds[k]:
+                gop = ops.BnGradFold(zk, ctot, stat, 16 * c, 20 * c, g32, b32, lsums, count, act)
+                dconv = dak
+            else:
+                check(lib.stp3_bn_apply_bwd(ctypes.byref(dims), dak.data_ptr(), zk.data_ptr(), None, None, None, mean_p, invstd_p,
+                                            ops._opt_ptr(g32), ops._opt_ptr(b32), lsums.data_ptr(), count, dconv.data_ptr(), None,
+                                            stream), 'stp3_bn_apply_bwd')
             dgamma = lsums[1].to(gdt) if gdt is not None and need[3] else None
             dbeta = lsums[0].to(bdt) if bdt is not None and need[4] else None
             cout, cin, kh, kw = wb.shape
             ref = ctx.weight_refs[1 + k]
             dx = dw = dcb = None
             if need[0]:
-                dx = ops.conv2d_data_grad(dconv, wb, ref, x.shape, stride, pad, dil)
+                dx = ops.conv2d_data_grad(dconv, wb, ref, x.shape, stride, pad, dil, grad=gop)
             if need[1]:
-                dw = ops._conv2d_wgrad(dconv, x, (cout, cin, kh, kw), stride, pad, dil, leaf=ref).to(wdt)
+                dw = ops._conv2d_wgrad(dconv, x, (cout, cin, kh, kw), stride, pad, dil, leaf=ref, grad=gop).to(wdt)
             if has_cbias and need[2]:
                 dcb = ops.channel_sums(dconv).to(cbdt)
             grads += [dx, dw, dcb, dgamma, dbeta] + [None] * (_N_PRODUCER_ARGS - 5)
diff --git a/st-p3_amd/stp3_amd/profiling.py b/st-p3_amd/stp3_amd/profiling.py
--- a/st-p3_amd/stp3_amd/profiling.py
+++ b/st-p3_amd/stp3_amd/profiling.py
@@ -35,7 +35,8 @@
 
 
 LABEL = {'stp3_conv2d_fwd': _conv_label, 'stp3_conv2d_fwd_add': _conv_label, 'stp3_conv2d_wgrad': _conv_label, 'stp3_conv2d_wgrad_partials': _conv_label,
-         'stp3_conv2d_fwd_pre': _conv_label, 'stp3_conv2d_wgrad_pre': _conv_label}
+         'stp3_conv2d_fwd_pre': _conv_label, 'stp3_conv2d_wgrad_pre': _conv_label, 'stp3_conv2d_fwd_bngrad': _conv_label,
+         'stp3_conv2d_wgrad_bngrad': _conv_label, 'stp3_conv2d_wgrad_bngrad_partials': _conv_label}
 
 
 def _bn_bytes(tensors):
@@ -71,6 +72,9 @@
     'stp3_conv2d_wgrad': ('conv_wgrad', _conv_flops),
     'stp3_conv2d_wgrad_pre': ('conv_wgrad', _conv_flops),
     'stp3_conv2d_wgrad_partials': ('conv_wgrad', _conv_flops),
+    'stp3_conv2d_fwd_bngrad': ('conv_fwd_dgrad', _conv_flops),
+    'stp3_conv2d_wgrad_bngrad': ('conv_wgrad', _conv_flops),
+    'stp3_conv2d_wgrad_bngrad_partials': ('conv_wgrad', _conv_flops),
     'stp3_conv2d_wgrad_reduce_batch': ('conv_wgrad', lambda args: 0.0),
     'stp3_bn_stats': ('batchnorm', _bn_bytes(1)),
     'stp3_bn_apply_fwd': ('batchnorm', _bn_bytes(2)),
```
